# YxZhxn/Ray3D

Hardware: AMD Instinct MI355X
Metric: lifted poses/sec (17-joint, 243-frame window) (higher is better)
Workload: dtype f32; 1 GPU; BASELINE configs[1]: synthetic 17-joint 243-frame windows, batch 256 per GPU, forward-only pos+trj (C=256, latent 256, stage 3, camera embedding); batch_per_gpu=256, receptive_field=243, joints=17, parallelism=dp1 (independent window batches, no data-path collective), clock_settle_steps=60, world_size_observed=1

## Files before the change

### include/ray3d_hip.h

```cpp
#ifndef RAY3D_HIP_H
#define RAY3D_HIP_H

#include <stddef.h>
#include <stdint.h>

#ifdef __cplusplus
extern "C" {
#endif

#define R3D_OK 0
#define R3D_ERR_ARG (-1)
#define R3D_ERR_KEY (-2)
#define R3D_ERR_SHAPE (-3)
#define R3D_ERR_STATE (-4)
#define R3D_ERR_HIP (-5)
#define R3D_ERR_WORKSPACE (-6)
#define R3D_ERR_ABORTED (-7)

#define R3D_KIND_POS 0
#define R3D_KIND_TRJ 1

#define R3D_ABI_VERSION 6

typedef struct {
// ... 39 lines not shown
    int64_t window_stride;
    const float *param_dev;
    int64_t param_stride;
    const double *cam_dev;
    int64_t cam_stride;
} r3d_input;

size_t r3d_workspace_bytes(const r3d_model *pos, const r3d_model *trj, int64_t B);

size_t r3d_input_workspace_bytes(const r3d_model *pos, const r3d_model *trj, const r3d_input *in, int64_t B);

int r3d_prepare(r3d_model *pos, r3d_model *trj, int64_t B);
int r3d_release(r3d_model *pos, r3d_model *trj, int64_t B);

int r3d_forward(r3d_model *m, const r3d_input *in, int64_t B, float *out_dev,
                void *workspace_dev, size_t workspace_bytes, void *hip_stream);

int r3d_forward_pair(r3d_model *pos, r3d_model *trj, const r3d_input *in, int64_t B,
                     float *out_dev, float *out_trj_dev, void *workspace_dev,
                     size_t workspace_bytes, void *hip_stream);


int r3d_status(r3d_model *m, void *hip_stream);

#define R3D_OPT_STAGED 1
#define R3D_OPT_SPIN_TIMEOUT_MS 2
#define R3D_OPT_CU_LIMIT 3
#define R3D_OPT_LANES 4
int r3d_set_option(r3d_model *m, int32_t option, int64_t value);

int r3d_lane_stream(r3d_model *m, int32_t lane, void **stream);
int r3d_lanes_join(r3d_model *m, void *stream);


typedef struct {
    char kernel[48];
    int32_t stage;
    int32_t blocks;
    float ms;
    double flops;
    double bytes;
} r3d_launch_record;
int r3d_profile_enable(r3d_model *m, int on);
int r3d_profile_read(r3d_model *m, r3d_launch_record *records, int capacity);

int r3d_last_clock(r3d_model *m, void *hip_stream, double *ghz);


#define R3D_METRIC_MPJPE 0
#define R3D_METRIC_PMPJPE 1
#define R3D_METRIC_NMPJPE 2
#define R3D_METRIC_VELOCITY 3
#define R3D_METRIC_ROOT 4
#define R3D_METRIC_COUNT 5
#define R3D_METRIC_MAX_BLOCKS 128
#define R3D_METRIC_OUT_DOUBLES (R3D_METRIC_COUNT * (1 + R3D_METRIC_MAX_BLOCKS))
int r3d_clip_metrics(const float *pred_dev, const float *gt_dev, int64_t n_frames, int32_t num_joints,
                     const double *rn2w, const double *tn2w, double *out_dev, void *stream);

#define R3D_DETAIL_THRESHOLDS 31
#define R3D_DETAIL_JOINT_ROWS 3
#define R3D_DETAIL_MAX_JOINTS 17
#define R3D_DETAIL_DOUBLES (R3D_DETAIL_JOINT_ROWS * R3D_DETAIL_MAX_JOINTS + R3D_DETAIL_THRESHOLDS)
#define R3D_DETAIL_OUT_DOUBLES (R3D_DETAIL_DOUBLES * (1 + R3D_METRIC_MAX_BLOCKS))
int r3d_clip_metrics_detail(const float *pred_dev, const float *gt_dev, int64_t n_frames, int32_t num_joints,
                            const double *rn2w, const double *tn2w, double *out_dev, double *frame_dev, double *detail_dev,
                            void *stream);


typedef struct {
    int64_t first_frame;
    int64_t n_frames;
    double  rn2w[9];
    double  tn2w[3];
} r3d_clip_desc;
#define R3D_CLIPS_MAX 65535
size_t r3d_clips_metrics_scratch_bytes(int32_t num_clips, int64_t max_frames, int detail);
int r3d_clips_metrics(const float *pred_dev, const float *gt_dev, int64_t total_frames, int32_t num_joints,
                      const r3d_clip_desc *clips_dev, int32_t num_clips, int64_t max_frames,
                      double *rows_dev, int64_t row_stride,
                      double *detail_dev, int64_t detail_stride,
                      double *frame_dev,
                      void *scratch_dev, size_t scratch_bytes, void *stream);


typedef struct {
    int64_t first_frame;
    int64_t n_frames;
    int64_t out_first;
    int32_t pad_front;
    int32_t pad_back;
    double  cam[16];
} r3d_clip_input_desc;
#define R3D_ENCODE_RAY 0
#define R3D_ENCODE_INTRINSIC 1
#define R3D_ENCODE_SCREEN 2
#define R3D_ENCODE_MAX_POINTS 2147483391
int r3d_clips_encode(const float *px_dev, int64_t total_frames, int32_t num_joints, int32_t encoding,
                     const r3d_clip_input_desc *clips_dev, int32_t num_clips, int64_t max_rows,
                     float *x_dev, int64_t out_rows,
                     float *x_mirror_dev, const int32_t *mirror_perm,
                     int32_t *status_dev, void *stream);


#define R3D_VALID_POS_IS_SUM 1
#define R3D_VALID_GT_ROOT_RELATIVE 2
#define R3D_VALID_LOSS 0
#define R3D_VALID_POS 1
#define R3D_VALID_TRJ_W 2
#define R3D_VALID_TRJ_WSUM 3
#define R3D_VALID_TRJ_DSUM 4
#define R3D_VALID_BONE_LEN 5
#define R3D_VALID_BONE_DIR 6
#define R3D_VALID_COUNT 7
#define R3D_VALID_MAX_BONES 16
#define R3D_VALID_BONE_ROWS 4
#define R3D_VALID_DOUBLES (R3D_VALID_COUNT + R3D_VALID_BONE_ROWS * R3D_VALID_MAX_BONES)
#define R3D_VALID_OUT_DOUBLES (R3D_VALID_DOUBLES * (1 + R3D_METRIC_MAX_BLOCKS))
int r3d_clip_valid_losses(const float *pos_dev, const float *trj_dev, const float *gt_dev, int64_t n_frames,
                          int32_t num_joints, const int32_t *parents, int32_t flags,
                          double *out_dev, double *frame_dev, void *stream);

size_t r3d_clips_valid_scratch_bytes(int32_t num_clips, int64_t max_frames);
int r3d_clips_valid_losses(const float *pos_dev, const float *trj_dev, const float *gt_dev,
                           int64_t total_frames, int32_t num_joints,
                           const int32_t *parents, int32_t flags,
                           const r3d_clip_desc *clips_dev, int32_t num_clips, int64_t max_frames,
                           double *rows_dev, int64_t row_stride,
                           double *frame_dev,
                           void *scratch_dev, size_t scratch_bytes, void *stream);


int r3d_clips_poses(const float *raw_dev, const float *raw_mirror_dev, int64_t raw_rows, int32_t num_joints,
                    const int32_t *mirror_perm,
                    const r3d_clip_desc *clips_dev, const int64_t *raw_first_dev, int32_t num_clips, int64_t max_frames,
                    float *pred_dev, double *world_dev, int64_t total_frames,
                    int32_t *status_dev, void *stream);

const char *r3d_last_error(void);
const char *r3d_version(void);
int r3d_abi_version(void);
int r3d_precision(const r3d_model *m);

#ifdef R3D_TEST_HOOKS

int r3d_debug_schedule_check(int nprob, const int *M, const int *N, const int *nk, const int *max_ks,
                             const int *max_units, int nwg, int enc, int *out_grid, int *out_tiles,
                             double *out_imbalance);

int r3d_debug_plan_check(r3d_model *pos, r3d_model *trj, int64_t batch, int nwg, int *launches, int *spilled);

int r3d_debug_forward_check(r3d_model *pos, r3d_model *trj, int64_t batch, int nwg, int *tiles, int *counters);

typedef struct r3d_census_row {
    int32_t launch;
    int32_t blocks;
    int32_t tiles;
    char kernel[48];
    char tile_kind[48];
} r3d_census_row;
int r3d_debug_forward_census(r3d_model *pos, r3d_model *trj, int64_t batch, int nwg, int32_t uv, int64_t cam_stride,
                             int64_t window_stride, int32_t staged, int32_t captured, r3d_census_row *rows, int32_t cap);
int r3d_debug_census_domain(r3d_census_row *rows, int32_t cap);

int r3d_debug_undistort_host(const double *row16, const double *uv, int64_t n, double *out_uv, double *out_rays);

int r3d_debug_encode_px_host(const double *row16, const double *uv, int64_t n, int32_t encoding, double *out2);

int r3d_debug_valid_losses_host(const float *pos, const float *trj, const float *gt, int64_t n_frames, int32_t num_joints,
                                const int32_t *parents, int32_t flags, double *out, double *frame);
int r3d_debug_clips_encode_host(const float *px, int64_t total_frames, int32_t num_joints, int32_t encoding,
                                const r3d_clip_input_desc *clips, int32_t num_clips, int64_t max_rows, float *x, int64_t out_rows,
                                float *x_mirror, const int32_t *mirror_perm, int32_t *status);
int r3d_debug_clips_valid_losses_host(const float *pos, const float *trj, const float *gt, int64_t total_frames, int32_t num_joints,
                                      const int32_t *parents, int32_t flags, const r3d_clip_desc *clips, int32_t num_clips,
                                      int64_t max_frames, double *rows, int64_t row_stride, double *frame);
int r3d_debug_clips_poses_host(const float *raw, const float *raw_mirror, int64_t raw_rows, int32_t num_joints,
                               const int32_t *mirror_perm, const r3d_clip_desc *clips, const int64_t *raw_first, int32_t num_clips,
                               int64_t max_frames, float *pred, double *world, int64_t total_frames, int32_t *status);
#endif

#ifdef __cplusplus
}
#endif
#endif
```

### ray3d_amd/_capi.py

```python
from __future__ import annotations

import ctypes as C
import os
from typing import List, Optional

_HERE = os.path.dirname(os.path.abspath(__file__))
LIB_PATH = os.path.join(_HERE, "libray3d_hip.so")
HOOKS_LIB_PATH = os.environ.get("R3D_HOOKS_LIB") or os.path.join(_HERE, "libray3d_hip_hooks.so")

R3D_KIND_POS, R3D_KIND_TRJ = 0, 1
R3D_INPUT_RAYS, R3D_INPUT_UV, R3D_INPUT_UV_DIST = 0, 1, 2
R3D_INPUT_PX_INTRINSIC, R3D_INPUT_PX_SCREEN = 3, 4
PX_MODES = (R3D_INPUT_UV_DIST, R3D_INPUT_PX_INTRINSIC, R3D_INPUT_PX_SCREEN)
R3D_ERR_ARG, R3D_ERR_WORKSPACE = -1, -6
R3D_ERR_ABORTED = -7
R3D_OPT_STAGED, R3D_OPT_SPIN_TIMEOUT_MS, R3D_OPT_CU_LIMIT, R3D_OPT_LANES = 1, 2, 3, 4

EXPORTS = (
    "r3d_create", "r3d_destroy", "r3d_num_weights", "r3d_weight_key", "r3d_weight_shape",
    "r3d_set_weight", "r3d_finalize", "r3d_workspace_bytes", "r3d_forward", "r3d_forward_pair",
    "r3d_profile_enable", "r3d_profile_read", "r3d_clip_metrics", "r3d_clip_metrics_detail", "r3d_clip_valid_losses", "r3d_last_error", "r3d_version",
    "r3d_prepare", "r3d_release", "r3d_abi_version", "r3d_precision", "r3d_status", "r3d_set_option", "r3d_last_clock",
    "r3d_lane_stream", "r3d_lanes_join", "r3d_input_workspace_bytes", "r3d_clips_metrics", "r3d_clips_metrics_scratch_bytes",
    "r3d_clips_encode", "r3d_clips_valid_losses", "r3d_clips_valid_scratch_bytes", "r3d_clips_poses",
)
HOOK_EXPORTS = ("r3d_debug_schedule_check", "r3d_debug_plan_check", "r3d_debug_forward_check",
                "r3d_debug_forward_census", "r3d_debug_census_domain",
                "r3d_debug_undistort_host", "r3d_debug_encode_px_host", "r3d_debug_valid_losses_host",
                "r3d_debug_clips_encode_host", "r3d_debug_clips_valid_losses_host", "r3d_debug_clips_poses_host")
ABI_VERSION = 6
METRIC_NAMES = ("mpjpe", "p_mpjpe", "n_mpjpe", "velocity", "root")
METRIC_OUT_DOUBLES = 5 * (1 + 128)
DETAIL_THRESHOLDS, DETAIL_JOINT_ROWS, DETAIL_MAX_JOINTS = 31, 3, 17
DETAIL_DOUBLES = DETAIL_JOINT_ROWS * DETAIL_MAX_JOINTS + DETAIL_THRESHOLDS
DETAIL_OUT_DOUBLES = DETAIL_DOUBLES * (1 + 128)
R3D_VALID_POS_IS_SUM, R3D_VALID_GT_ROOT_RELATIVE = 1, 2
VALID_NAMES = ("loss", "pos", "trj_w", "trj_wsum", "trj_dsum", "bone_len", "bone_dir")
VALID_COUNT, VALID_MAX_BONES, VALID_BONE_ROWS = 7, 16, 4
VALID_DOUBLES = VALID_COUNT + VALID_BONE_ROWS * VALID_MAX_BONES
VALID_OUT_DOUBLES = VALID_DOUBLES * (1 + 128)
METRIC_COUNT, METRIC_MAX_BLOCKS, METRIC_THREADS = 5, 128, 256
CLIPS_MAX = 65535
R3D_ENCODE_RAY, R3D_ENCODE_INTRINSIC, R3D_ENCODE_SCREEN = 0, 1, 2
ENCODE_FLOATS = {R3D_ENCODE_RAY: 3, R3D_ENCODE_INTRINSIC: 2, R3D_ENCODE_SCREEN: 2}
ENCODE_MAX_POINTS = 2 ** 31 - 257
CLIP_INPUT_DESC_BYTES = 160


class Config(C.Structure):
    _fields_ = [(n, C.c_int32) for n in ("struct_size", "kind", "num_joints", "in_features", "num_levels",
                                         "channels", "latent", "stage", "extrinsic_dim",
                                         "embed_dim", "causal", "dense", "bf16x3")]


class Input(C.Structure):
    _fields_ = [("mode", C.c_int32), ("x_dev", C.c_void_p), ("window_stride", C.c_int64),
                ("param_dev", C.c_void_p), ("param_stride", C.c_int64),
                ("cam_dev", C.c_void_p), ("cam_stride", C.c_int64)]


class ClipDesc(C.Structure):
    _fields_ = [("first_frame", C.c_int64), ("n_frames", C.c_int64), ("rn2w", C.c_double * 9), ("tn2w", C.c_double * 3)]


def clip_desc_dtype():
    import numpy as np
    return np.dtype([("first_frame", np.int64), ("n_frames", np.int64), ("rn2w", np.float64, (9,)), ("tn2w", np.float64, (3,))])


CLIP_DESC_BYTES = clip_desc_dtype().itemsize


def clip_input_desc_dtype():
    import numpy as np
    return np.dtype([("first_frame", np.int64), ("n_frames", np.int64), ("out_first", np.int64),
                     ("pad_front", np.int32), ("pad_back", np.int32), ("cam", np.float64, (16,))])


class LaunchRecord(C.Structure):
    _fields_ = [("kernel", C.c_char * 48), ("stage", C.c_int32), ("blocks", C.c_int32),
                ("ms", C.c_float), ("flops", C.c_double), ("bytes", C.c_double)]


class CensusRow(C.Structure):
    _fields_ = [("launch", C.c_int32), ("blocks", C.c_int32), ("tiles", C.c_int32), ("kernel", C.c_char * 48),
                ("tile_kind", C.c_char * 48)]


class Ray3DHipError(RuntimeError):
    pass


_libs = {}
_hooks = os.environ.get("R3D_USE_HOOKS_LIB", "0") not in ("", "0")


_live = {}


def use_hooks(on: bool) -> None:
    global _hooks
    if bool(on) != _hooks and _live.get(HOOKS_LIB_PATH if _hooks else LIB_PATH, 0) > 0:
        try:
            import torch
            if torch.cuda.is_available():
                torch.cuda.synchronize()
        except ImportError:
            pass
    _hooks = bool(on)


def load():
    path = HOOKS_LIB_PATH if _hooks else LIB_PATH
    if path in _libs:
        return _libs[path]
    if not os.path.exists(path):
        raise Ray3DHipError(
            "%s not found: build it with `python -c 'import __graft_entry__ as g; g.build()'` "
            "(hipcc --offload-arch=gfx950).  There is no CPU fallback." % path)
    lib = C.CDLL(path)
    vp, i64p = C.c_void_p, C.POINTER(C.c_int64)
    lib.r3d_create.argtypes = [C.POINTER(Config), C.POINTER(vp)]
    lib.r3d_destroy.argtypes = [vp]
    lib.r3d_num_weights.argtypes = [vp]
    lib.r3d_weight_key.argtypes = [vp, C.c_int]
    lib.r3d_weight_key.restype = C.c_char_p
    lib.r3d_weight_shape.argtypes = [vp, C.c_int, i64p, C.POINTER(C.c_int)]
    lib.r3d_set_weight.argtypes = [vp, C.c_char_p, vp, i64p, C.c_int]
    lib.r3d_finalize.argtypes = [vp]
    lib.r3d_workspace_bytes.argtypes = [vp, vp, C.c_int64]
    lib.r3d_workspace_bytes.restype = C.c_size_t
    lib.r3d_input_workspace_bytes.argtypes = [vp, vp, C.POINTER(Input), C.c_int64]
    lib.r3d_input_workspace_bytes.restype = C.c_size_t
    lib.r3d_forward.argtypes = [vp, C.POINTER(Input), C.c_int64, vp, vp, C.c_size_t, vp]
    lib.r3d_forward_pair.argtypes = [vp, vp, C.POINTER(Input), C.c_int64, vp, vp, vp, C.c_size_t, vp]
    lib.r3d_prepare.argtypes = [vp, vp, C.c_int64]
    lib.r3d_release.argtypes = [vp, vp, C.c_int64]
    lib.r3d_precision.argtypes = [vp]
    lib.r3d_status.argtypes = [vp, vp]
    lib.r3d_set_option.argtypes = [vp, C.c_int32, C.c_int64]
    lib.r3d_last_clock.argtypes = [vp, vp, C.POINTER(C.c_double)]
    lib.r3d_lane_stream.argtypes = [vp, C.c_int32, C.POINTER(vp)]
    lib.r3d_lanes_join.argtypes = [vp, vp]
    lib.r3d_profile_enable.argtypes = [vp, C.c_int]
    lib.r3d_profile_read.argtypes = [vp, C.POINTER(LaunchRecord), C.c_int]
    lib.r3d_clip_metrics.argtypes = [vp, vp, C.c_int64, C.c_int32, C.POINTER(C.c_double), C.POINTER(C.c_double), vp, vp]
    lib.r3d_clip_metrics_detail.argtypes = [vp, vp, C.c_int64, C.c_int32, C.POINTER(C.c_double), C.POINTER(C.c_double), vp, vp, vp, vp]
    lib.r3d_clip_valid_losses.argtypes = [vp, vp, vp, C.c_int64, C.c_int32, C.POINTER(C.c_int32), C.c_int32, vp, vp, vp]
    lib.r3d_clips_metrics_scratch_bytes.argtypes = [C.c_int32, C.c_int64, C.c_int]
    lib.r3d_clips_metrics_scratch_bytes.restype = C.c_size_t
    lib.r3d_clips_metrics.argtypes = [vp, vp, C.c_int64, C.c_int32, vp, C.c_int32, C.c_int64, vp, C.c_int64, vp, C.c_int64, vp, vp, C.c_size_t, vp]
    lib.r3d_clips_encode.argtypes = [vp, C.c_int64, C.c_int32, C.c_int32, vp, C.c_int32, C.c_int64, vp, C.c_int64, vp,
                                     C.POINTER(C.c_int32), vp, vp]
    lib.r3d_clips_valid_scratch_bytes.argtypes = [C.c_int32, C.c_int64]
    lib.r3d_clips_valid_scratch_bytes.restype = C.c_size_t
    lib.r3d_clips_valid_losses.argtypes = [vp, vp, vp, C.c_int64, C.c_int32, C.POINTER(C.c_int32), C.c_int32, vp, C.c_int32, C.c_int64,
                                           vp, C.c_int64, vp, vp, C.c_size_t, vp]
    lib.r3d_clips_poses.argtypes = [vp, vp, C.c_int64, C.c_int32, C.POINTER(C.c_int32), vp, vp, C.c_int32, C.c_int64, vp, vp, C.c_int64,
                                    vp, vp]
    lib.r3d_last_error.restype = C.c_char_p
    lib.r3d_version.restype = C.c_char_p
    if _hooks:
        lib.r3d_debug_forward_census.argtypes = [vp, vp, C.c_int64, C.c_int, C.c_int32, C.c_int64, C.c_int64, C.c_int32, C.c_int32,
                                                 C.POINTER(CensusRow), C.c_int32]
        lib.r3d_debug_census_domain.argtypes = [C.POINTER(CensusRow), C.c_int32]
        lib.r3d_debug_clips_poses_host.argtypes = [vp, vp, C.c_int64, C.c_int32, C.POINTER(C.c_int32), vp, vp, C.c_int32, C.c_int64, vp, vp,
                                                   C.c_int64, vp]
        lib.r3d_debug_clips_valid_losses_host.argtypes = [vp, vp, vp, C.c_int64, C.c_int32, C.POINTER(C.c_int32), C.c_int32, vp, C.c_int32,
                                                          C.c_int64, vp, C.c_int64, vp]
        lib.r3d_debug_undistort_host.argtypes = [vp, vp, C.c_int64, vp, vp]
        lib.r3d_debug_encode_px_host.argtypes = [vp, vp, C.c_int64, C.c_int32, vp]
        lib.r3d_debug_valid_losses_host.argtypes = [vp, vp, vp, C.c_int64, C.c_int32, C.POINTER(C.c_int32), C.c_int32, vp, vp]
        lib.r3d_debug_clips_encode_host.argtypes = [vp, C.c_int64, C.c_int32, C.c_int32, vp, C.c_int32, C.c_int64, vp, C.c_int64, vp,
                                                    C.POINTER(C.c_int32), vp]
    for name in EXPORTS + (HOOK_EXPORTS if _hooks else ()):
        fn = getattr(lib, name)
        if fn.restype is C.c_int or fn.restype is None:
            fn.restype = C.c_int
    if lib.r3d_abi_version() != ABI_VERSION:
        raise Ray3DHipError("%s has ABI version %d, this binding was written for %d: rebuild the library"
# ... 247 lines not shown
```

### ray3d_amd/csrc/r3d_forward.cpp

```cpp
#include <algorithm>
#include <cstring>
#include <mutex>

#include "r3d_internal.hpp"
#include "r3d_undistort.hpp"

namespace r3d {

static void output_slots(int J, const int *first, int *slot) {
    int s = 0;
    auto put = [&](int part, int idx) {
        for (int f = 0; f < 3; ++f) slot[first[part] + idx * 3 + f] = s * 3 + f;
        ++s;
    };
    enum { T = 0, LA = 1, RA = 2, LL = 3, RL = 4 };
    if (J == 17) {
        put(T, 0);
        for (int i = 0; i < 3; ++i) put(LL, i);
        for (int i = 0; i < 3; ++i) put(RL, i);
        for (int i = 1; i < 5; ++i) put(T, i);
        for (int i = 0; i < 3; ++i) put(RA, i);
        for (int i = 0; i < 3; ++i) put(LA, i);
    } else if (J == 15) {
        put(T, 0); put(T, 1);
// ... 492 lines not shown
    bool bound = false;
    char *ctrl = nullptr;
    size_t bank_bytes = 0;
    GemmProb *tables = nullptr;
    int bank = 0;
    unsigned *cnt = nullptr;
    BoundKey key;
};

void resolve_single(const Call &c, Single &s) {
    const Schedule::Fwd &fw = c.sched->fwd;
    const r3d_input *in = c.in;
    if (hipStreamIsCapturing(c.stream, &s.cap) != hipSuccess) { (void)hipGetLastError(); s.cap = hipStreamCaptureStatusActive; }
    s.own = s.cap == hipStreamCaptureStatusNone && fw.d_ctrl != nullptr;
    s.ctrl = s.own ? fw.d_ctrl : reinterpret_cast<char *>(c.ws) + workspace_act_bytes(c.pl, c.B);
    s.bank_bytes = ((size_t)(fw.ncnt + 4) * sizeof(unsigned) + 255) / 256 * 256;
    s.tables = reinterpret_cast<GemmProb *>(s.ctrl + (s.own ? 2 : 1) * s.bank_bytes);
    s.poll = s.own && fw.d_act != nullptr;
    s.key.variant = c.variant;
    s.key.base[BIND_WS] = c.ws;
    s.key.base[BIND_ARENA0] = c.bases.arena[0];
    s.key.base[BIND_ARENA1] = c.bases.arena[1];
    s.key.base[BIND_IARENA0] = c.bases.iarena[0];
    s.key.base[BIND_IARENA1] = c.bases.iarena[1];
    s.key.base[BIND_X] = in->x_dev;
    s.key.base[BIND_PARAM] = in->param_dev;
    s.key.base[BIND_CAM] = in->cam_dev;
    s.key.enc_ws = in->window_stride * c.JF;
    s.key.cam_stride = in->cam_stride;
    s.key.enc_bytes = (unsigned)((size_t)c.frames * c.JF * sizeof(float));
    s.key.param_stride = (int)in->param_stride;
    const Schedule::Fwd::Bound &bd = fw.bound;
    s.bound = s.own && bd.valid && bd.key == s.key;
    s.bank = s.bound ? bd.bank ^ 1 : 0;
    s.cnt = reinterpret_cast<unsigned *>(s.ctrl + (s.own ? s.bank : 0) * s.bank_bytes);
}

int bind_if_needed(Call &c, const Single &s) {
    if (s.bound) return R3D_OK;
    const Schedule::Fwd &fw = c.sched->fwd;
    BindArgs ba;
    memset(&ba, 0, sizeof ba);
    ba.rel = fw.d_rel[c.variant];
    ba.tags = fw.d_tags[c.variant];
    ba.out = s.tables;
    ba.nprob = fw.nprob;
    for (int k = 0; k < BIND_NBASE; ++k) ba.base[k] = s.key.base[k];
    ba.enc_ws = s.key.enc_ws;
    ba.cam_stride = s.key.cam_stride;
    ba.enc_bytes = s.key.enc_bytes;
    ba.param_stride = s.key.param_stride;
    ba.cnt = reinterpret_cast<unsigned *>(s.ctrl);
    ba.ncnt = s.own ? (int)(2 * s.bank_bytes / sizeof(unsigned)) - 4 : fw.ncnt;
    if (s.poll) {
        ba.base[BIND_WS] = fw.d_act;
        ba.arm = fw.d_act;
        ba.canon = 1;
        ba.arm_vec4 = (long long)(2 * fw.act_bytes / 16);
    }
    hipError_t e;
    if (const int rc = c.begin(bind_kernel_name(), 1, 0.0, 0.0); rc != R3D_OK) return rc;
    if ((e = launch_bind(ba, c.stream)) != hipSuccess) return hip_fail(e, "launch r3d_bind_f32");
    if (s.poll) {
        BindArgs b1 = ba;
        b1.base[BIND_WS] = fw.d_act + fw.act_bytes;
        b1.out = s.tables + fw.nprob;
        b1.ncnt = -4;
        b1.arm = nullptr;
        if ((e = launch_bind(b1, c.stream)) != hipSuccess) return hip_fail(e, "launch r3d_bind_f32");
    }
    return c.end();
}

int launch_tiles(Call &c, const Single &s, FwdArgs &fa) {
    Schedule::Fwd &fw = c.sched->fwd;
    const GemmProb *table = s.tables + (s.poll ? s.bank * fw.nprob : 0);
    if (s.poll) c.act_base = reinterpret_cast<float *>(fw.d_act + (size_t)s.bank * fw.act_bytes);
    fw.bound.valid = false;
    memset(&fa, 0, sizeof fa);
    fa.tiles = fw.d_tiles;
    fa.wg_off = fw.d_wgoff;
    fa.probs = table;
    fa.cnt = s.cnt;
    fa.cnt_next = s.own ? reinterpret_cast<unsigned *>(s.ctrl + (s.bank ^ 1) * s.bank_bytes) : nullptr;
    fa.ncnt = fw.ncnt;
    if (s.poll) {
        fa.poll = 1;
        fa.arm = fw.d_act + (size_t)(s.bank ^ 1) * fw.act_bytes;
        fa.arm_vec4 = (long long)(fw.act_bytes / 16);
    }
    fa.spin_ticks = (long long)std::max(c.a->spin_timeout_ms, 1) * 100000LL;
    if (const char *ft = hook_env("R3D_FAULT_TILE")) fa.fault_tile1 = atoi(ft) + 1;
    const bool uv_launch = c.uv && fw.uses_gather;
    const int fwd_kernel = c.shared ? FWD_KERNEL_CLIP : fw.kernel;
    if (const int rc = c.begin(forward_kernel_name(fwd_kernel, uv_launch), fw.grid, fw.flops, fw.bytes); rc != R3D_OK) return rc;
#ifdef R3D_TIMING
    timing_arm_forward(fw, fa, c.stream);
#endif
    if (const hipError_t e = launch_forward(fa, fw.grid, fwd_kernel, uv_launch, c.stream); e != hipSuccess) return hip_fail(e, "launch r3d_forward_f32");
    c.a->last_clk_dev = s.cap == hipStreamCaptureStatusNone ? s.cnt + fw.ncnt + 2 : nullptr;
    return R3D_OK;
}

int launch_in_order(Call &c, const Single &s, FwdArgs &fa) {
    Model *a = c.a;
    hipError_t e;
    std::lock_guard<std::mutex> launch_lock(g_fwd_launch_mu);
    if ((e = order_single_launch(c.stream, true, c.cu_limit > 0)) != hipSuccess) return hip_fail(e, "hipStreamWaitEvent");
    if (c.cu_limit > 0 && a->lanes <= 1 && a->last_fwd_stream && a->last_fwd_stream != c.stream) {
        if ((e = wait_behind(c.stream, (hipStream_t)a->last_fwd_stream, a->order_ev)) != hipSuccess) return hip_fail(e, "hipStreamWaitEvent");
    }
    a->last_fwd_stream = c.stream;
    if (const int rc = bind_if_needed(c, s); rc != R3D_OK) return rc;
    if (const int rc = launch_tiles(c, s, fa); rc != R3D_OK) return rc;
    if ((e = order_single_launch(c.stream, false, c.cu_limit > 0)) != hipSuccess) return hip_fail(e, "hipEventRecord");
    return R3D_OK;
}

int single_launch(Call &c) {
    Schedule::Fwd &fw = c.sched->fwd;
    Single s;
    resolve_single(c, s);
    FwdArgs fa;
    if (const int rc = launch_in_order(c, s, fa); rc != R3D_OK) return rc;
    if (s.own) {
        fw.bound.valid = true;
        fw.bound.bank = s.bank;
        fw.bound.key = s.key;
    }
#ifdef R3D_TIMING
    timing_report_forward(c.pl, fw, fa, c.B, c.stream);
#endif
    if (const int rc = c.end(); rc != R3D_OK) return rc;
    c.abort_flag = s.cnt + fw.ncnt;
    return R3D_OK;
}

int staged_level(Call &c, size_t si) {
    const Plan *pl = c.pl;
    const auto &st = (*c.sched->levels)[si];
    const StageSchedule &ss = c.sched->stages[si];
    LaunchArgs la;
    memset(&la, 0, sizeof la);
    la.tiles = c.sched->d_tiles + ss.tiles_off;
    la.wg_off = c.sched->d_wgoff + ss.wgoff_off;
    la.nprob = (int)st.size();
    la.ks = ss.ks;
    int n_enc = 0;
    for (int i = 0; i < la.nprob; ++i) {
        const ProbSpec &q = pl->probs[st[i] & ~STAGE_SPILL_IN];
        if (q.enc_lut >= 0 && q.enc_kernel) ++n_enc;
        const int rc = fill_prob(pl, q, c.B, c.a, c.bases, c.shape, la.p[i], nullptr);
        if (rc != R3D_OK) return rc;
    }
    if (n_enc != 0 && n_enc != la.nprob) { set_error("internal: launch mixes encoded and plain operands"); return R3D_ERR_STATE; }
    if ((n_enc != 0) != (ss.kind == STAGE_ENC)) { set_error("internal: schedule and plan disagree on the launch kind"); return R3D_ERR_STATE; }
    bool uv_launch = false;
    for (int i = 0; i < la.nprob; ++i) uv_launch = uv_launch || la.p[i].cam != nullptr;
    bool b3_launch = false;
    for (int i = 0; i < la.nprob; ++i) b3_launch = b3_launch || la.p[i].wb3 != nullptr;
    const char *kname = stage_kernel_name(ss.kind, uv_launch, b3_launch);
    if (const int rc = c.begin(kname, ss.nwg, ss.flops, ss.bytes); rc != R3D_OK) return rc;
#ifdef R3D_TIMING
    const bool timed = timing_arm_stage(si, la, c.stream);
#endif
    if (const hipError_t e = launch_gemm_stage(la, ss.nwg, ss.kind, uv_launch, c.stream); e != hipSuccess) return hip_fail(e, "launch r3d_gemm_f32");
#ifdef R3D_TIMING
    if (timed) timing_report_stage(si, ss, c.stream);
#endif
    return c.end();
}

int staged_levels(Call &c) {
    c.a->last_clk_dev = nullptr;
    for (size_t si = 0; si < c.sched->levels->size(); ++si)
        if (const int rc = staged_level(c, si); rc != R3D_OK) return rc;
    return R3D_OK;
}

int decoder_tail(Call &c) {
    const Model *a = c.a;
    const Plan *pl = c.pl;
    auto buf_ptr = [&](int id) -> float * { return c.act_base + (size_t)pl->buffers[id].offset_per_window * (size_t)c.B; };
    DecodeArgs da;
    memset(&da, 0, sizeof da);
    da.B = c.B;
    da.J = a->cfg.num_joints;
    da.has_pos = pl->pos_model >= 0;
    da.has_trj = pl->trj_model >= 0;
    da.out = c.out;
    da.out_trj = da.has_pos ? c.out_trj : nullptr;
    da.abort_flag = c.abort_flag;
    da.status = a->status_host;
    double dec_flops = 0;
    int first = 0;
    std::vector<Plan::Dec> order;
    for (const auto &d : pl->decs) if (pl->m[d.model]->cfg.kind == R3D_KIND_POS) order.push_back(d);
    for (const auto &d : pl->decs) if (pl->m[d.model]->cfg.kind == R3D_KIND_TRJ) order.push_back(d);
    int firsts[MAX_DEC] = {0};
    for (const auto &d : order) {
        const Model *m = pl->m[d.model];
        const Layer &L = m->layers[d.layer];
        const int sidx = da.nsrc++;
        da.h[sidx] = buf_ptr(d.hbuf);
        da.w[sidx] = m->d_arena + L.w_off;
        da.bias[sidx] = m->d_arena + L.b_off;
        da.n_out[sidx] = L.N;
        da.first[sidx] = first;
        firsts[sidx] = first;
        if (m->cfg.kind == R3D_KIND_POS) first += L.N;
        dec_flops += 2.0 * (double)c.B * L.K * L.N;
    }
    if (da.has_pos) output_slots(da.J, firsts, da.slot);
    if (const int rc = c.begin(decode_kernel_name(c.B), 0, dec_flops, (double)c.B * da.nsrc * MLP_HIDDEN * 4.0); rc != R3D_OK) return rc;
    if (const hipError_t e = launch_decode(da, c.stream); e != hipSuccess) return hip_fail(e, "launch r3d_decode_f32");
    if (const int rc = c.end(); rc != R3D_OK) return rc;
    if (c.rec.on()) c.a->nrec = (int)c.rec.n;
    return R3D_OK;
}

int relay_done(Call &c) {
    Model::Lane *relay = c.relay;
    if (!relay) return R3D_OK;
    if (const hipError_t e = hipEventRecord(relay->done, relay->stream); e != hipSuccess) return hip_fail(e, "hipEventRecord(lane)");
    if (std::find(relay->waiters.begin(), relay->waiters.end(), c.caller_stream) == relay->waiters.end()) relay->waiters.push_back(c.caller_stream);
    return R3D_OK;
}

}

int forward_run(Model *a, Model *b, const r3d_input *in, int64_t B, float *out, float *out_trj, void *ws, size_t ws_bytes,
                void *stream) {
    Call c{a, b, in, B, out, out_trj, ws, ws_bytes, stream, (hipStream_t)stream};
    int rc = check_call(c);
    if (rc == R3D_OK) rc = redirect_px(c);
    if (rc == R3D_OK) rc = pick_plan(c);
    if (rc == R3D_OK) rc = pick_lane(c);
    if (rc == R3D_OK) rc = empty_bracket(c);
    if (rc == R3D_OK) rc = px_prepass(c);
    if (rc == R3D_OK) rc = pick_schedule(c);
    if (rc == R3D_OK) rc = frame_stage(c);
    if (rc == R3D_OK) rc = c.single ? single_launch(c) : staged_levels(c);
    if (rc == R3D_OK) rc = decoder_tail(c);
    if (rc == R3D_OK) rc = relay_done(c);
    return rc;
}

}
```

### ray3d_amd/csrc/r3d_hooks.cpp

```cpp
#ifdef R3D_TEST_HOOKS
#include <algorithm>
#include <cstdio>
#include <cstring>
#include <set>
#include <utility>

#include "r3d_internal.hpp"
#include "r3d_poses.hpp"
#include "r3d_undistort.hpp"
#include "r3d_valid.hpp"

using namespace r3d;

namespace {

struct CensusProb { bool w3, lut, wb3, w2; int K; };
struct CensusKernel { const char *name; bool enc, uv, dep, b3, narrow, clip; };

std::vector<CensusKernel> census_kernels() {
    std::vector<CensusKernel> v;
    for (int uv = 0; uv < 2; ++uv) {
        const bool u = uv != 0;
        v.push_back({stage_kernel_name(STAGE_BIG, u, false), false, u, false, false, true, true});
        v.push_back({stage_kernel_name(STAGE_ENC, u, false), true, u, false, false, false, true});
// ... 118 lines not shown
            for (int g = t.z / COL_GRANULE; g < (t.z + tile_width(ks)) / COL_GRANULE && g < gcols; ++g) ++cover[pi][(size_t)u * gcols + g];
        }
    }
    for (int i = 0; i < nprob; ++i)
        for (int c : cover[i])
            if (c != 1) return -10;
    return 0;
}

int r3d_debug_plan_check(r3d_model *pos, r3d_model *trj, int64_t batch, int nwg, int *launches, int *spilled) {
    const ModelPair mp = model_pair(pos, trj);
    Model *a = mp.a, *b = mp.b;
    if (!a) return -1;
    Plan *pl = plan_get(a, b, plan_kind(batch));
    if (!pl) return -2;
    int spill_row0 = -1;
    std::vector<int4> tiles;
    std::vector<int> wgoff;
    std::vector<StageSchedule> stages;
    const std::vector<std::vector<int>> &levels = *schedule_build_host(pl, batch, nwg, spill_row0, tiles, wgoff, stages);
    if (launches) *launches = (int)stages.size();
    if (spilled) *spilled = 0;
    const int np = (int)pl->probs.size();
    std::vector<std::vector<int>> cover(np);
    std::vector<int> last_launch(np, -1), first_launch(np, 1 << 30);
    for (int i = 0; i < np; ++i) {
        const ProbSpec &q = pl->probs[i];
        const int M = (int)(batch * q.rows_per_window), N = pl->m[q.model]->layers[q.layer].N;
        cover[i].assign((size_t)((M + 31) / 32) * ((N + COL_GRANULE - 1) / COL_GRANULE), 0);
    }
    for (size_t si = 0; si < stages.size(); ++si) {
        const StageSchedule &ss = stages[si];
        const auto &st = levels[si];
        if (ss.nwg < 1 || ss.nwg > 2 * nwg) return -3;
        {
            int n_enc = 0;
            for (int e : st) n_enc += pl->probs[e & ~STAGE_SPILL_IN].enc_kernel ? 1 : 0;
            if (n_enc != 0 && n_enc != (int)st.size()) return -11;
            if ((n_enc != 0) != (ss.kind == STAGE_ENC)) return -12;
        }
        for (int t = 0; t < ss.ntiles; ++t) {
            const int4 &tl = tiles[ss.tiles_off + t];
            const int slot = tl.x & 0xff, mi = tl.x >> 8, ks = tl.w;
            if (slot >= (int)st.size() || mi < 1) return -4;
            const int id = st[slot] & ~STAGE_SPILL_IN;
            const ProbSpec &q = pl->probs[id];
            const int M = (int)(batch * q.rows_per_window), N = pl->m[q.model]->layers[q.layer].N;
            if (tl.y % 32 || tl.y < 0 || tl.y >= M || tl.z < 0 || tl.z >= N) return -5;
            if (id == pl->spill_prob) {
                const bool late = (st[slot] & STAGE_SPILL_IN) != 0;
                if (spill_row0 < 0 ? late : (late != (tl.y >= spill_row0))) return -6;
                if (late && spilled) *spilled += std::min(mi * 32, M - tl.y);
            }
            const int gcols = (N + COL_GRANULE - 1) / COL_GRANULE;
            for (int u = tl.y / 32; u < tl.y / 32 + mi; ++u) {
                if (u * 32 >= M) return -7;
                for (int g = tl.z / COL_GRANULE; g < (tl.z + tile_width(ks)) / COL_GRANULE && g < gcols; ++g) ++cover[id][(size_t)u * gcols + g];
            }
            last_launch[id] = std::max(last_launch[id], (int)si);
            first_launch[id] = std::min(first_launch[id], (int)si);
        }
    }
    for (int i = 0; i < np; ++i) {
        for (int c : cover[i])
            if (c != 1) return -8;
        for (int d : pl->probs[i].deps)
            if (last_launch[d] >= first_launch[i]) return -9;
    }
    return 0;
}

int r3d_debug_forward_check(r3d_model *pos, r3d_model *trj, int64_t batch, int nwg, int *out_tiles, int *out_counters) {
    const ModelPair mp = model_pair(pos, trj);
    Model *a = mp.a, *b = mp.b;
    if (!a) return -1;
    Plan *pl = plan_get(a, b, plan_kind(batch));
    int spill_row0 = -1;
    std::vector<int4> tiles;
    std::vector<int> wgoff;
    std::vector<StageSchedule> stages;
    const std::vector<std::vector<int>> &levels = *schedule_build_host(pl, batch, nwg, spill_row0, tiles, wgoff, stages);
    Schedule::Fwd fw;
    std::vector<int> ft, fo;
    if (!schedule_build_fwd(pl, batch, nwg, levels, stages, tiles, wgoff, fw, ft, fo)) return 1;
    if (out_tiles) *out_tiles = fw.ntiles;
    if (out_counters) *out_counters = fw.ncnt;
    const int np = (int)pl->probs.size(), TI = FWD_TILE_INT4 * 4;
    std::vector<int> gcols(np);
    for (int i = 0; i < np; ++i) gcols[i] = (pl->m[pl->probs[i].model]->layers[pl->probs[i].layer].N + COL_GRANULE - 1) / COL_GRANULE;
    std::vector<unsigned> cnt(fw.ncnt, 0);
    struct Acc { int buf, c0, c1; };
    auto reads = [&](const ProbSpec &q) {
        std::vector<Acc> v;
        for (int sgi = 0; sgi < q.nseg; ++sgi)
            if (pl->buffers[q.seg[sgi].buf].external == 0) v.push_back({q.seg[sgi].buf, q.seg[sgi].col, q.seg[sgi].col + q.seg[sgi].width});
        if (q.res_buf >= 0) v.push_back({q.res_buf, q.res_col, q.res_col + pl->m[q.model]->layers[q.layer2 >= 0 && q.layer3 < 0 ? q.layer2 : q.layer].N});
        return v;
    };
    auto writes = [&](const ProbSpec &q) {
        const int N = pl->m[q.model]->layers[q.layer3 >= 0 ? q.layer3 : q.layer2 >= 0 ? q.layer2 : q.layer].N;
        return Acc{q.c_buf, q.c_col, q.c_col + N};
    };
    auto overlap = [](const Acc &x, const Acc &y) { return x.buf == y.buf && x.c0 < y.c1 && y.c0 < x.c1; };
    auto complete = [&](int prob, int w0, int w1) {
        const ProbSpec &q = pl->probs[prob];
        const int M = (int)(batch * q.rows_per_window);
        const int a0 = w0 * q.rows_per_window, a1 = std::min(w1 * q.rows_per_window, M);
        for (int u = a0 / 32; u < (a1 + 31) / 32; ++u)
            if (cnt[fw.cnt_base[prob] + u] != (unsigned)gcols[prob]) return false;
        return true;
    };
    if (pl->kind == PLAN_SMALL) {
        for (int i = 0; i < np; ++i)
            for (int o = 0; o < i; ++o)
                if (overlap(writes(pl->probs[i]), writes(pl->probs[o]))) return -25;
        for (int i = 0; i < np; ++i)
            for (const Acc &rd : reads(pl->probs[i])) {
                std::vector<char> covered(rd.c1 - rd.c0, 0);
                bool any = false, same_rows = true;
                for (int o = 0; o < np; ++o) {
                    const Acc w = writes(pl->probs[o]);
                    if (w.buf != rd.buf) continue;
                    any = true;
                    same_rows = same_rows && pl->probs[o].rows_per_window == pl->probs[i].rows_per_window;
                    for (int c = std::max(w.c0, rd.c0); c < std::min(w.c1, rd.c1); ++c) covered[c - rd.c0] = 1;
                }
                if (!any) return -26;
                if (same_rows)
                    for (char c : covered)
                        if (!c) return -26;
            }
    }
    std::vector<int> next(fw.grid);
    for (int w = 0; w < fw.grid; ++w) next[w] = fo[w];
    int done = 0;
    for (bool progress = true; progress;) {
        progress = false;
        for (int w = 0; w < fw.grid; ++w) {
            while (next[w] < fo[w + 1]) {
                const int *d = &ft[(size_t)next[w] * TI];
                bool ready = true;
                for (int k = 0; k < d[4] && ready; ++k) {
                    const int base = d[8 + 2 * k], n = d[9 + 2 * k] & 0xffff;
                    const unsigned need = (unsigned)d[9 + 2 * k] >> 16;
                    for (int u = 0; u < n && ready; ++u) ready = cnt[base + u] >= need;
                }
                if (!ready) break;
                const int id = d[0] & 0xff, mi = d[0] >> 8;
                const ProbSpec &q = pl->probs[id];
                const int M = (int)(batch * q.rows_per_window);
                const int r1 = std::min(d[1] + mi * 32, M);
                const int w0 = d[1] / q.rows_per_window, w1 = (r1 - 1) / q.rows_per_window + 1;
                const Acc wr = writes(q);
                for (int o = 0; o < id; ++o) {
                    const ProbSpec &oq = pl->probs[o];
                    bool hazard = false;
                    for (const Acc &rd : reads(q)) hazard = hazard || overlap(rd, writes(oq));
                    for (const Acc &rd : reads(oq)) hazard = hazard || overlap(rd, wr);
                    hazard = hazard || overlap(writes(oq), wr);
                    if (hazard && !complete(o, w0, w1)) return -20;
                }
                if (d[5] != fw.cnt_base[id] + d[1] / 32 || d[5] + mi > fw.ncnt) return -21;
                for (int u = 0; u < mi; ++u) {
                    cnt[d[5] + u] += (unsigned)d[6];
                    if (cnt[d[5] + u] > (unsigned)gcols[id]) return -22;
                }
                ++next[w];
                ++done;
                progress = true;
            }
        }
    }
    if (done != fw.ntiles) return -23;
    for (int i = 0; i < np; ++i)
        for (int u = 0; u < (int)((batch * pl->probs[i].rows_per_window + 31) / 32); ++u)
            if (cnt[fw.cnt_base[i] + u] != (unsigned)gcols[i]) return -24;
    return 0;
}

int r3d_debug_forward_census(r3d_model *pos, r3d_model *trj, int64_t batch, int nwg, int32_t uv, int64_t cam_stride, int64_t window_stride,
                             int32_t staged, int32_t captured, r3d_census_row *rows, int32_t cap) {
    const ModelPair mp = model_pair(pos, trj);
    Model *a = mp.a, *b = mp.b;
    if (!a || batch <= 0 || nwg <= 0 || window_stride <= 0 || (!rows && cap > 0)) return -1;
    if (b && !same_input_shape(a, b)) return -1;
    if (uv && a->cfg.in_features != 3) return -1;
    Plan *pl = plan_get(a, b, plan_kind(batch));
    if (!pl) return -2;
    CensusSched &cs = g_census;
    if (cs.ida != a->id || cs.idb != (b ? b->id : 0) || cs.pl != pl || cs.B != batch || cs.nwg != nwg) {
        cs = CensusSched();
        cs.ida = a->id;
        cs.idb = b ? b->id : 0;
        cs.pl = pl;
        cs.B = batch;
        cs.nwg = nwg;
        cs.levels = schedule_build_host(pl, batch, nwg, cs.spill_row0, cs.tiles, cs.wgoff, cs.stages);
        if (forward_single_launch() && schedule_build_fwd(pl, batch, nwg, *cs.levels, cs.stages, cs.tiles, cs.wgoff, cs.fw, cs.ft, cs.fo)) {
            bool narrow = false, b3_tiles = false;
            cs.fw.kernel = forward_kernel_of_lists(pl, batch, cs.ft, narrow, b3_tiles);
            if (narrow && b3_tiles) cs.fw = Schedule::Fwd();
        } else {
            cs.fw = Schedule::Fwd();
        }
    }
    const std::vector<CensusKernel> kernels = census_kernels();
    const Schedule::Fwd &fw = cs.fw;
    const long long frames = (batch - 1) * window_stride + a->RF;
    const bool shared = call_shares_first_layers(pl, a, batch, uv != 0, window_stride, cam_stride, frames, pl->frame_buf >= 0);
    const int variant = (uv ? 1 : 0) + (shared ? 2 : 0);
    std::vector<GemmProb> rel;
    std::vector<unsigned char> tags;
    const bool has_table = fw.grid > 0 && forward_variant_table(pl, batch, variant, fw.nprob, rel, tags);
    const bool single = !staged && call_is_single(a, b, fw.grid, has_table, fw.kernel, shared);
    CensusOut out{rows, cap};
    if (shared) {
        std::vector<int4> ft;
        std::vector<int> fo;
        StageSchedule fs{};
        schedule_frame_stage(pl, batch, nwg, ft, fo, fs);
        const char *name = stage_kernel_name(STAGE_BIG, uv != 0, false);
        const CensusKernel *k = census_find(kernels, name);
        if (!k) return -4;
        std::map<std::string, int> hist;
        for (const int4 &t : ft) {
            const Plan::FrameProb &f = pl->frame_probs[t.x & 0xff];
            ++hist[census_tile_kind(*k, CensusProb{false, true, false, false, pl->m[f.model]->layers[f.layer].Kpad}, t.x >> 8, t.w)];
        }
        out.launch_of(name, fs.nwg, hist);
    }
    if (single) {
        (void)captured;
        out.launch_of(bind_kernel_name(), 1, {});
        const int fwd_kernel = shared ? FWD_KERNEL_CLIP : fw.kernel;
        const char *name = forward_kernel_name(fwd_kernel, uv && fw.uses_gather);
        const CensusKernel *k = census_find(kernels, name);
        if (!k) return -4;
        std::map<std::string, int> hist;
        const int TI = FWD_TILE_INT4 * 4;
        for (int t = 0; t < fw.ntiles; ++t) {
            const int *d = &cs.ft[(size_t)t * TI];
            const int id = d[0] & 0xff;
            ++hist[census_tile_kind(*k, census_prob(&tags[(size_t)id * BIND_NPTR], rel[id].K), d[0] >> 8, d[3])];
        }
        out.launch_of(name, fw.grid, hist);
    } else {
        CallShape shape;
        shape.uv = uv != 0;
        shape.shared = shared;
        shape.window_stride = window_stride;
        shape.cam_stride = cam_stride;
        shape.frames = frames;
        const Bases none;
        for (size_t si = 0; si < cs.levels->size(); ++si) {
            const auto &st = (*cs.levels)[si];
            const StageSchedule &ss = cs.stages[si];
            std::vector<CensusProb> P(st.size());
            bool uv_launch = false, b3_launch = false;
            for (size_t i = 0; i < st.size(); ++i) {
                GemmProb g;
                unsigned char tg[BIND_NPTR];
                if (fill_prob(pl, pl->probs[st[i] & ~STAGE_SPILL_IN], batch, a, none, shape, g, tg) != R3D_OK) return -3;
                P[i] = census_prob(tg, g.K);
                uv_launch = uv_launch || tg[17] != BIND_NULL;
                b3_launch = b3_launch || P[i].wb3;
            }
            const char *name = stage_kernel_name(ss.kind, uv_launch, b3_launch);
            const CensusKernel *k = census_find(kernels, name);
            if (!k) return -4;
            std::map<std::string, int> hist;
            for (int t = 0; t < ss.ntiles; ++t) {
                const int4 &tl = cs.tiles[ss.tiles_off + t];
                const int slot = tl.x & 0xff;
                if (slot >= (int)st.size()) return -5;
                ++hist[census_tile_kind(*k, P[slot], tl.x >> 8, tl.w)];
            }
            out.launch_of(name, ss.nwg, hist);
        }
    }
    out.launch_of(decode_kernel_name(batch), 0, {});
    return out.n;
}

int r3d_debug_census_domain(r3d_census_row *rows, int32_t cap) {
    if (!rows && cap > 0) return -1;
    CensusOut out{rows, cap};
    for (const char *name : launch_kernel_names()) out.row(name, 0, "", 0);
    const int codes[] = {1, 2, 4, 8, 16, NB_CODE + 4, NB_CODE + 5, NB_CODE + 6, NB_CODE + 7};
    for (const CensusKernel &k : census_kernels()) {
        std::set<std::string> kinds;
        for (int f = 0; f < 16; ++f)
            for (int K : {64, 96})
                for (int mi = 1; mi <= GEMM_SCHED_MAX_UNITS + 1; ++mi)
                    for (int ks : codes) kinds.insert(census_tile_kind(k, CensusProb{(f & 1) != 0, (f & 2) != 0, (f & 4) != 0, (f & 8) != 0, K}, mi, ks));
        for (const std::string &kind : kinds) out.row(k.name, 0, kind.c_str(), 0);
    }
    return out.n;
}

int r3d_debug_undistort_host(const double *row16, const double *uv, int64_t n, double *out_uv, double *out_rays) {
    if (!row16 || (!uv && n > 0) || n < 0) { set_error("r3d_debug_undistort_host: bad argument"); return R3D_ERR_ARG; }
    const UndistRow k = undist_row(row16);
    for (int64_t i = 0; i < n; ++i) {
        double uo, vo, r[3];
        undistort_pixel(k, uv[2 * i], uv[2 * i + 1], uo, vo);
        pixel_to_ray(k, uo, vo, r);
        if (out_uv) { out_uv[2 * i] = uo; out_uv[2 * i + 1] = vo; }
        if (out_rays) for (int c = 0; c < 3; ++c) out_rays[3 * i + c] = r[c];
    }
    return R3D_OK;
}

int r3d_debug_encode_px_host(const double *row16, const double *uv, int64_t n, int32_t encoding, double *out2) {
    if (!row16 || !out2 || (!uv && n > 0) || n < 0) { set_error("r3d_debug_encode_px_host: bad argument"); return R3D_ERR_ARG; }
    if (encoding != ENC_INTRINSIC && encoding != ENC_SCREEN) {
        set_error("r3d_debug_encode_px_host: encoding must be 1 (intrinsic) or 2 (screen), got %d", encoding);
        return R3D_ERR_ARG;
    }
    for (int64_t i = 0; i < n; ++i) encode_pixel_2d(row16, encoding, uv[2 * i], uv[2 * i + 1], out2 + 2 * i);
    return R3D_OK;
}

int r3d_debug_clips_encode_host(const float *px, int64_t total_frames, int32_t num_joints, int32_t encoding,
                                const r3d_clip_input_desc *clips, int32_t num_clips, int64_t max_rows, float *x, int64_t out_rows,
                                float *x_mirror, const int32_t *mirror_perm, int32_t *status) {
    const int rc = clips_encode_check_args("r3d_debug_clips_encode_host", px, total_frames, num_joints, encoding, clips, num_clips, max_rows,
                                           x, out_rows, x_mirror, mirror_perm, status);
    if (rc != R3D_OK) return rc;
    unsigned long long inv[2] = {0ull, 0ull};
    if (mirror_perm) mirror_pack_inverse(mirror_perm, num_joints, inv);
// ... 112 lines not shown
```

### ray3d_amd/csrc/r3d_internal.hpp

```cpp
#pragma once

#include <hip/hip_runtime.h>

#include <cstdint>
#include <cstdlib>
#include <map>
#include <mutex>
#include <string>
#include <vector>

#include "ray3d_hip.h"

namespace r3d {

constexpr int BK = 32;
constexpr int MAX_SEG = 4;
constexpr int MAX_PROB = 12;
constexpr int N_ALIGN = 256;
constexpr int MLP_HIDDEN = 1024;
constexpr int EMBED_MID = 32;
constexpr int CUR_LD = 64;


struct GemmProb {
    const float *a[MAX_SEG];
    int lda[MAX_SEG];
    int kend[MAX_SEG];
    const float *w;
    const float *bias;
    const float *res;
    float *c;
    int ldr, ldc;
    int M, N, K;
    float slope;
    const float *w2;
    const float *bias2;
    int K2;
    float slope2;
    const float *wb3;
    const float *w2b3, *w3b3;
    const float *w3;
    const float *bias3;
    int K3;
    float slope3;
    const int *lut;
    const float *x;
    long long enc_ws;
    int enc_rows;
    int enc_jf;
    int enc_cur;
    int enc_step;
    unsigned enc_bytes;
    int res_tap;
    int canon;
    const double *cam;
    long long cam_stride;
};

struct LaunchArgs {
    const int4 *tiles;
    const int *wg_off;
    int nprob;
    int ks;
    long long *dbg;
    GemmProb p[MAX_PROB];
};

constexpr int FWD_TILE_INT4 = 6;
constexpr int FWD_MAX_DEP = 8;
struct FwdArgs {
    const int4 *tiles;
    const int *wg_off;
    const GemmProb *probs;
    unsigned *cnt;
    unsigned *cnt_next;
    int ncnt;
    int poll;
    void *arm;
    long long arm_vec4;
    long long spin_ticks;
    int fault_tile1;
    long long *dbg;
};
enum { FWD_KERNEL_F32 = 0, FWD_KERNEL_B3 = 1, FWD_KERNEL_LAT = 2, FWD_KERNEL_CLIP = 3, FWD_KERNEL_COUNT = 4 };
constexpr int BIND_NPTR = 18;
enum { BIND_NULL = 0, BIND_WS, BIND_ARENA0, BIND_ARENA1, BIND_IARENA0, BIND_IARENA1, BIND_X, BIND_PARAM, BIND_CAM, BIND_NBASE };
struct BindArgs {
    const GemmProb *rel;
    const unsigned char *tags;
    GemmProb *out;
    unsigned *cnt;
    int nprob, ncnt;
    const void *base[BIND_NBASE];
    long long enc_ws, cam_stride;
    unsigned enc_bytes;
    int param_stride;
    int canon;
    void *arm;
    long long arm_vec4;
};

struct UndistArgs {
    const float *uv;
    const double *cam;
    long long cam_stride;
    float *rays;
    int npts;
    int J;
    int pts_per_window;
    int window_stride;
    int last_window;
    int encoding;
};

struct ClipsEncArgs {
    const r3d_clip_input_desc *table;
    const float *px;
    float *x;
    float *x_mirror;
    int32_t *status;
    long long total_frames, out_rows, max_rows;
    unsigned long long mirror_inv[2];
    int J;
    int encoding;
};

struct ClipsPosesArgs {
    const r3d_clip_desc *table;
    const long long *raw_first;
    const float *raw, *raw_mirror;
    float *pred;
    double *world;
    int32_t *status;
    long long raw_rows, total_frames, max_frames;
    unsigned long long mirror_perm[2];
    int J;
};

constexpr int MAX_DEC = 6;
struct DecodeArgs {
    const float *h[MAX_DEC];
    const float *w[MAX_DEC];
    const float *bias[MAX_DEC];
    int n_out[MAX_DEC];
    int first[MAX_DEC];
    int nsrc;
    int has_pos, has_trj;
    int J;
    long long B;
    float *out;
    float *out_trj;
    const unsigned *abort_flag;
    unsigned *status;
    int slot[5 * 16];
};


struct TensorSpec {
    std::string key;
    int rank;
    int64_t shape[4];
    int64_t numel() const {
        int64_t n = 1;
        for (int i = 0; i < rank; ++i) n *= shape[i];
        return n;
    }
};

inline int64_t b3_min_batch() {
    return 96;
}

inline bool env_on(const char *name) {
    const char *e = getenv(name);
    return e && atoi(e) != 0;
}
#ifdef R3D_TEST_HOOKS
inline bool hook_on(const char *name) { return env_on(name); }
inline const char *hook_env(const char *name) { return getenv(name); }
#else
inline bool hook_on(const char *) { return false; }
inline const char *hook_env(const char *) { return nullptr; }
#endif

struct Layer {
    std::string weight_key;
    std::string bias_key;
    std::string bn_prefix;
    int taps;
    int cin;
    int N, K, Npad, Kpad;
    float slope;
    std::vector<int> colmap;
    std::vector<int> colmap_neg;
    bool frag;
    size_t w_off, b_off;
    bool bf3 = false;
    bool bf3_conv = false;
    size_t wb3_off = 0;
    struct Pre { int ref_col0, ref_width, new_width, shrink_layer; };
    std::vector<Pre> pre;
    int cin_ref = 0;
    int shared_of = -1;
    int shared_split = 0;
};

struct Model {
    r3d_config cfg;
    int RF;
    std::vector<TensorSpec> specs;
    std::map<std::string, int> spec_index;
    std::vector<std::vector<float>> host_weights;
    std::vector<bool> have;
    std::vector<Layer> layers;
    std::map<std::string, int> layer_index;
    struct Branch {
        std::string prefix;
        std::vector<int> joints;
        int cin, k0, k0pad;
        size_t lut_off;
        size_t lut_uv_off;
        size_t lut_frame_off = 0, lut_frame_uv_off = 0;
        int frame_layer = -1;
    };
    std::vector<Branch> branches;
    size_t global_lut_off = 0;
    size_t global_lut_uv_off = 0;
    bool use_b3 = false;
    bool fold_shrink = false;
    std::vector<float> arena;
    std::vector<int> iarena;
    float *d_arena = nullptr;
    int *d_iarena = nullptr;
    int device = -1;
    bool finalized = false;
    bool dirty = true;
    bool opt_staged = false;
    int spin_timeout_ms = 1000;
    int cu_limit = 0;
    void *last_fwd_stream = nullptr;
    hipEvent_t order_ev = nullptr;
    int lanes = 0;
    struct Lane {
        hipStream_t stream = nullptr;
        hipEvent_t done = nullptr, in = nullptr;
        std::vector<void *> waiters;
    };
    Lane lane[4];
    int next_lane = 0;
    const unsigned *last_clk_dev = nullptr;
    unsigned *status_host = nullptr;
    bool profiling = false;
    struct Rec {
        hipEvent_t e0, e1;
        r3d_launch_record r;
    };
    std::vector<Rec> recs;
    int nrec = 0;
    uint64_t id = 0;
    ~Model();
};

struct BufferSpec {
    std::string name;
    int64_t floats_per_window;
    int external;
    int64_t offset_per_window;
};

struct ProbSpec {
    int model;
    int layer;
    int rows_per_window;
    int nseg;
    struct Seg { int buf, col, ld, width; } seg[MAX_SEG];
    int res_buf, res_col, res_ld;
    int c_buf, c_col, c_ld;
    int layer2;
    int layer3;
    int enc_lut;
    int enc_lut_uv;
    bool enc_kernel;
    int enc_rows;
    int enc_step;
    int frame_col = -1;
    std::vector<int> deps;
    int depth;
    double flops_per_window;
};

struct StageSchedule {
    int nwg;
    int ks;
    int kind;
    int ntiles;
    size_t tiles_off;
    size_t wgoff_off;
    double flops, bytes;
    double imbalance;
    double makespan;
};

struct BoundKey {
    int variant = 0;
    const void *base[BIND_NBASE] = {nullptr};
    long long enc_ws = 0, cam_stride = 0;
    unsigned enc_bytes = 0;
    int param_stride = 0;
    bool operator==(const BoundKey &o) const {
        bool same = variant == o.variant && enc_ws == o.enc_ws && cam_stride == o.cam_stride && enc_bytes == o.enc_bytes &&
                    param_stride == o.param_stride;
        for (int k = 0; same && k < BIND_NBASE; ++k) same = base[k] == o.base[k];
        return same;
    }
};

struct Schedule {
    int64_t B = 0;
    bool pinned = false;
    int spill_row0 = -1;
    const std::vector<std::vector<int>> *levels = nullptr;
    std::vector<StageSchedule> stages;
    int4 *d_tiles = nullptr;
    int *d_wgoff = nullptr;
    StageSchedule frame_stage{};
    int4 *d_frame_tiles = nullptr;
    int *d_frame_wgoff = nullptr;
    struct Fwd {
        int grid = 0, ntiles = 0, ncnt = 0, nprob = 0;
        std::vector<int> cnt_base;
        int4 *d_tiles = nullptr;
        int *d_wgoff = nullptr;
        GemmProb *d_rel[4] = {nullptr, nullptr, nullptr, nullptr};
        unsigned char *d_tags[4] = {nullptr, nullptr, nullptr, nullptr};
        std::vector<int> h_tiles, h_wgoff;
        double flops = 0, bytes = 0;
        bool uses_gather = false;
        int kernel = FWD_KERNEL_F32;
        char *d_ctrl = nullptr;
        size_t bank_bytes = 0;
        char *d_act = nullptr;
        size_t act_bytes = 0;
        struct Bound {
            bool valid = false;
            int bank = 0;
            BoundKey key;
        } bound;
    } fwd;
    ~Schedule();
};

struct Plan {
    const Model *m[2] = {nullptr, nullptr};
    std::vector<BufferSpec> buffers;
    std::vector<ProbSpec> probs;
    std::vector<std::vector<int>> stages;
    std::vector<std::vector<int>> stages_spill;
    std::vector<std::vector<int>> stages_spill_alt;
    std::vector<std::vector<int>> stages_asap;
    int spill_prob = -1;
    int kind = 0;
    int64_t floats_per_window = 0;
    int64_t tail_floats = 0;
    int frame_buf = -1, frame_ld = 0;
    struct FrameProb { int model, layer, col, lut, lut_uv; };
    std::vector<FrameProb> frame_probs;
    int emb_buf[2] = {-1, -1};
    int param_buf = -1;
    struct Dec { int model, layer, hbuf; };
    std::vector<Dec> decs;
    int pos_model = -1, trj_model = -1;
    std::map<int64_t, Schedule *> schedules;
    std::vector<int64_t> schedule_lru;
    ~Plan();
};

struct Bases {
    const char *ws = nullptr, *arena[2] = {nullptr, nullptr}, *iarena[2] = {nullptr, nullptr};
    const char *x = nullptr, *param = nullptr, *cam = nullptr;
};
struct CallShape {
    bool uv = false;
    bool shared = false;
    int64_t window_stride = 0, param_stride = 0, cam_stride = 0;
    long long frames = 0;
};

inline int frame_floats(const Model *a, bool uv) { return a->cfg.num_joints * (uv ? 2 : a->cfg.in_features); }

struct ModelPair { Model *a, *b; };
inline ModelPair model_pair(const r3d_model *pos, const r3d_model *trj) {
    Model *p = const_cast<Model *>(reinterpret_cast<const Model *>(pos)), *t = const_cast<Model *>(reinterpret_cast<const Model *>(trj));
    return {p ? p : t, p ? t : nullptr};
}

int fill_prob(const Plan *pl, const ProbSpec &q, int64_t B, const Model *a, const Bases &bs, const CallShape &cs, GemmProb &g,
              unsigned char *tags);
bool same_input_shape(const Model *a, const Model *b);
size_t workspace_bytes_pair(Model *a, Model *b, int64_t B);
int dist_check(const Model *a, const r3d_input *in, bool need_cam);
size_t dist_ray_bytes(const Model *a, const r3d_input *in, int64_t B);
struct FwdKeys { int cu_limit, nwg, lane_key0, nlanes; };
FwdKeys forward_keys(const Model *a, const Model *b);
int forward_run(Model *a, Model *b, const r3d_input *in, int64_t B, float *out, float *out_trj, void *ws, size_t ws_bytes, void *stream);
const char *stage_kernel_name(int kind, bool uv_launch, bool b3_launch);
const char *decode_kernel_name(int64_t B);
const char *bind_kernel_name();
const char *undistort_kernel_name();
std::vector<const char *> launch_kernel_names();
bool call_shares_first_layers(const Plan *pl, const Model *a, int64_t B, bool uv, int64_t window_stride, int64_t cam_stride, long long frames,
                              bool frame_tiles);
bool call_is_single(const Model *a, const Model *b, int grid, bool has_table, int kernel, bool shared);

extern std::mutex g_fwd_launch_mu;
hipError_t wait_behind(hipStream_t stream, hipStream_t other, hipEvent_t &ev);
hipError_t order_single_launch(hipStream_t stream, bool before, bool masked = false);
int lanes_create(Model *m, int n);
void lanes_destroy(Model *m);

int valid_check_args(const char *what, const float *pos, const float *trj, const float *gt, int64_t n, int32_t J,
                     const int32_t *parents, int32_t flags, const double *out);

int clips_valid_check_args(const char *what, const float *pos, const float *trj, const float *gt, int64_t total_frames, int32_t J,
                           const int32_t *parents, int32_t flags, const r3d_clip_desc *clips, int32_t num_clips, int64_t max_frames,
                           const double *rows, int64_t row_stride, const void *scratch, bool scratch_checked);

int clips_encode_check_args(const char *what, const float *px, int64_t total_frames, int32_t J, int32_t encoding,
                            const r3d_clip_input_desc *clips, int32_t num_clips, int64_t max_rows, const float *x, int64_t out_rows,
                            const float *x_mirror, const int32_t *mirror_perm, const int32_t *status);

int clips_poses_check_args(const char *what, const float *raw, const float *raw_mirror, int64_t raw_rows, int32_t J,
                           const int32_t *mirror_perm, const r3d_clip_desc *clips, const int64_t *raw_first, int32_t num_clips,
                           int64_t max_frames, const float *pred, const double *world, int64_t total_frames, const int32_t *status);

#ifdef R3D_TIMING
void timing_arm_forward(const Schedule::Fwd &fw, FwdArgs &fa, hipStream_t stream);
void timing_report_forward(const Plan *pl, const Schedule::Fwd &fw, const FwdArgs &fa, int64_t B, hipStream_t stream);
bool timing_arm_stage(size_t si, LaunchArgs &la, hipStream_t stream);
void timing_report_stage(size_t si, const StageSchedule &ss, hipStream_t stream);
#endif

void set_error(const char *fmt, ...);
const char *last_error();
int hip_fail(hipError_t e, const char *what);

Model *model_create(const r3d_config &cfg);
int model_set_weight(Model *m, const char *key, const float *host, const int64_t *shape, int rank);
int model_finalize(Model *m);
enum { PLAN_FUSED = 0, PLAN_SMALL = 1, PLAN_MEDIUM = 2, PLAN_LARGE = 3 };
int plan_kind(int64_t B);
std::vector<int64_t> plan_kind_edges();
Plan *plan_get(Model *a, Model *b, int kind);
void plans_drop(const Model *m);
bool plans_pinned(const Model *m);
constexpr int STAGE_SPILL_IN = 1 << 30;
constexpr int GEMM_SCHED_MAX_UNITS = 6;
struct SchedProb {
    int M, N, nk;
    int max_ks;
    int max_units;
    int nk2 = 0;
    int row0 = 0;
    bool gemv = false;
    bool lat = false;
    bool nb_ok = false;
};
constexpr int GEMV_ROWS = 4;
constexpr int COL_GRANULE = 32;
constexpr int NB_CODE = 64;
constexpr bool tile_is_nb(int ks) { return ks > NB_CODE; }
constexpr bool tile_is_narrow(int ks) { return ks >= 8 && ks < NB_CODE; }
constexpr int tile_width(int ks) { return ks > NB_CODE ? (ks - NB_CODE) * 32 : ks >= 8 ? 32 : 256 / ks; }
void schedule_stage(const std::vector<SchedProb> &probs, int nwg, int max_units, std::vector<int4> &tiles,
                    std::vector<int> &wgoff, StageSchedule &out, bool enc = false);
inline size_t frag_index(int o, int k, int nk) {
    const int nb = o >> 5, li = o & 31, kt = k >> 5, kin = k & 31, lh = kin >> 4, q = (kin & 15) >> 2, e = kin & 3;
    return ((((size_t)nb * nk + kt) * 4 + q) * 64 + (lh * 32 + li)) * 4 + e;
}
const std::vector<std::vector<int>> *schedule_build_host(const Plan *pl, int64_t B, int nwg, int &spill_row0, std::vector<int4> &tiles,
                                                        std::vector<int> &wgoff, std::vector<StageSchedule> &stages);
bool schedule_build_fwd(const Plan *pl, int64_t B, int nwg, const std::vector<std::vector<int>> &levels, const std::vector<StageSchedule> &stages,
                        const std::vector<int4> &tiles, const std::vector<int> &wgoff, Schedule::Fwd &fw, std::vector<int> &out_tiles,
                        std::vector<int> &out_wgoff);
Schedule *schedule_get(Plan *pl, int64_t B, int nwg, bool pin = false, int lane = 0);
void schedule_frame_stage(const Plan *pl, int64_t B, int nwg, std::vector<int4> &ft, std::vector<int> &fo, StageSchedule &ss);
bool forward_variant_table(const Plan *pl, int64_t B, int v, int nprob, std::vector<GemmProb> &rel, std::vector<unsigned char> &tags);
int forward_kernel_of_lists(const Plan *pl, int64_t B, const std::vector<int> &ft, bool &narrow, bool &b3_tiles);
inline int64_t schedule_key(int64_t B, int lane) { return B | ((int64_t)lane << 48); }
int device_cu_count();

enum { STAGE_BIG = 0, STAGE_ENC = 1 };
typedef void (*GemmKernel)(const LaunchArgs);
typedef void (*FwdKernel)(const FwdArgs);
GemmKernel gemm_kernel_f32(bool uv);
GemmKernel gemm_kernel_enc(bool uv);
GemmKernel gemm_kernel_b3(bool uv);
FwdKernel fwd_kernel_f32(bool uv);
FwdKernel fwd_kernel_b3(bool uv);
FwdKernel fwd_kernel_lat(bool uv);
FwdKernel fwd_kernel_clip(bool uv);
hipError_t launch_gemm_stage(const LaunchArgs &args, int nwg, int kind, bool uv, hipStream_t stream);
hipError_t launch_decode(const DecodeArgs &args, hipStream_t stream);
hipError_t launch_forward(const FwdArgs &args, int nwg, int kind, bool uv, hipStream_t stream);
const char *forward_kernel_name(int kind, bool uv);
int forward_resident_capacity(int kind, bool uv);
hipError_t launch_bind(const BindArgs &args, hipStream_t stream);
hipError_t launch_undistort(const UndistArgs &args, hipStream_t stream);
hipError_t launch_clips_encode(const ClipsEncArgs &args, int num_clips, hipStream_t stream);
hipError_t launch_clips_poses(const ClipsPosesArgs &args, int num_clips, hipStream_t stream);
bool forward_single_launch();
size_t fwd_ctrl_bytes(const Plan *pl, int64_t B);

inline int round_up(int v, int m) { return (v + m - 1) / m * m; }

constexpr int ENC_INVALID = (int)0x80000000u;

int launch_clip_metrics(const float *pred, const float *gt, long long n, int J, const double *Rn2w, const double *Tn2w,
                        double *out, double *frame, double *detail, hipStream_t stream);
int launch_clip_valid(const float *pos, const float *trj, const float *gt, long long n, int J, const int32_t *parents,
                      int flags, double *out, double *frame, hipStream_t stream);
size_t clips_metrics_scratch_bytes(int num_clips, long long max_frames, bool detail);
int launch_clips_metrics(const float *pred, const float *gt, long long total, int J, const r3d_clip_desc *table, int num_clips,
                         long long max_frames, double *rows, long long row_stride, double *detail, long long detail_stride,
                         double *frame, void *scratch, hipStream_t stream);
size_t clips_valid_scratch_bytes(int num_clips, long long max_frames);
int launch_clips_valid(const float *pos, const float *trj, const float *gt, long long total, int J, const int32_t *parents, int flags,
                       const r3d_clip_desc *table, int num_clips, long long max_frames, double *rows, long long row_stride,
                       double *frame, void *scratch, hipStream_t stream);

}
```

### ray3d_amd/csrc/r3d_plan.cpp

```cpp
#include <algorithm>
#include <cstdio>
#include <cstdlib>
#include <mutex>

#include "r3d_internal.hpp"

namespace r3d {

namespace {

struct Builder {
    Plan &p;
    int mi;
    const Model &m;

    int buffer(const std::string &name, int64_t floats_per_window, int external = 0) {
        BufferSpec b;
        b.name = name;
        b.floats_per_window = (floats_per_window + 15) / 16 * 16;
        b.external = external;
        b.offset_per_window = 0;
        p.buffers.push_back(b);
        return (int)p.buffers.size() - 1;
    }
// ... 169 lines not shown
            B.enc_in_gemm = small;
            B.single_assign = small;
            B.fuse_pairs = (kind == PLAN_FUSED || kind == PLAN_LARGE);
            B.fuse_top = kind == PLAN_LARGE;
        }
        const int lat = m->cfg.latent, D = m->cfg.embed_dim;
        int pe = -1;
        if (D > 0) {
            if (pl->param_buf < 0) pl->param_buf = B.buffer("param", 0, 3);
            const int eh = B.buffer("emb.h", EMBED_MID);
            pl->emb_buf[mi] = B.buffer("emb", D);
            const int E = m->cfg.extrinsic_dim;
            const int p1 = B.problem("embedder.w1", 1, {{pl->param_buf, 0, 0, E, -1}}, -1, 0, 0, eh, 0, EMBED_MID);
            pe = B.problem("embedder.w2", 1, {{eh, 0, EMBED_MID, EMBED_MID, p1}}, -1, 0, 0, pl->emb_buf[mi], 0, D);
        }
        const int g = B.buffer("global", lat);
        const int pg = B.fc_block("GlobalInfo", {}, 2, g, 0, lat, (int)m->global_lut_off, (int)m->global_lut_uv_off);
        if (m->cfg.kind == R3D_KIND_POS) {
            pl->pos_model = mi;
            const bool fold = m->fold_shrink;
            const int C = m->cfg.channels;
            const int tmp5 = fold ? -1 : B.buffer("tmp5", 5 * lat);
            int sh[5];
            for (int bi = 0; bi < 5; ++bi) sh[bi] = B.temporal_block(bi, tmp5, bi * lat, 5 * lat);
            int mix5 = -1, pf[5] = {-1, -1, -1, -1, -1};
            if (m->cfg.stage != 1) {
                mix5 = B.buffer("mix5", 5 * lat);
                for (int i = 0; i < 5; ++i) {
                    std::vector<Builder::In> ins;
                    if (fold) {
                        for (int k = 0; k < 5; ++k)
                            if (k != i) ins.push_back({B.locals[k].buf, 0, B.locals[k].ld, C, sh[k]});
                    } else {
                        if (i > 0) ins.push_back({tmp5, 0, 5 * lat, i * lat, sh[0]});
                        if (i < 4) ins.push_back({tmp5, (i + 1) * lat, 5 * lat, (4 - i) * lat, sh[4]});
                    }
                    const int first = (int)pl->probs.size();
                    pf[i] = B.fc_block("FuseBlocks." + std::to_string(i), ins, 1, mix5, i * lat, 5 * lat);
                    for (int k = 0; k < 5; ++k) pl->probs[first].deps.push_back(sh[k]);
                    for (int q = first; q < (int)pl->probs.size(); ++q) {
                        int d = 0;
                        for (int dep : pl->probs[q].deps) d = std::max(d, pl->probs[dep].depth + 1);
                        pl->probs[q].depth = d;
                    }
                }
            }
            for (int bi = 0; bi < 5; ++bi) {
                std::vector<Builder::In> ins;
                if (fold) ins.push_back({B.locals[bi].buf, 0, B.locals[bi].ld, C, sh[bi]});
                else ins.push_back({tmp5, bi * lat, 5 * lat, lat, sh[bi]});
                if (mix5 >= 0) ins.push_back({mix5, bi * lat, 5 * lat, lat, pf[bi]});
                ins.push_back({g, 0, lat, lat, pg});
                if (D > 0) ins.push_back({pl->emb_buf[mi], 0, D, D, pe});
                B.fc_block(std::string("Integration_") + (bi == 0 ? "Torso" : bi == 1 ? "LArm" : bi == 2 ? "RArm" : bi == 3 ? "LLeg" : "RLeg"),
                           ins, 1, -1, 0, 0);
            }
        } else {
            pl->trj_model = mi;
            const int local = m->fold_shrink ? -1 : B.buffer("local", lat);
            const int sh = B.temporal_block(0, local, 0, lat);
            std::vector<Builder::In> ins;
            if (m->fold_shrink) ins.push_back({B.locals[0].buf, 0, B.locals[0].ld, m->cfg.channels, sh});
            else ins.push_back({local, 0, lat, lat, sh});
            ins.push_back({g, 0, lat, lat, pg});
            if (D > 0) ins.push_back({pl->emb_buf[mi], 0, D, D, pe});
            B.fc_block("Integration", ins, 1, -1, 0, 0);
        }
    }
    std::vector<int> asap;
    for (const auto &q : pl->probs) asap.push_back(q.depth);
    auto levelise = [&](bool spill, bool pin_first, std::vector<std::vector<int>> &stages, bool early = false) -> bool {
        const int n = (int)pl->probs.size();
        for (int i = 0; i < n; ++i) pl->probs[i].depth = asap[i];
        int deepest = 0, pt = -1;
        for (const auto &q : pl->probs) deepest = std::max(deepest, q.depth);
        if (spill) {
            bool pos_fused = false;
            for (int i = 0; i < n; ++i) {
                const ProbSpec &q = pl->probs[i];
                if (q.layer3 >= 0 && pl->m[q.model]->cfg.kind == R3D_KIND_TRJ) pt = i;
                pos_fused = pos_fused || (q.layer3 >= 0 && pl->m[q.model]->cfg.kind == R3D_KIND_POS);
            }
            if (pt < 0 || !pos_fused) return false;
            for (auto &q : pl->probs)
                for (int d : q.deps)
                    if (d == pt) q.depth = std::max(q.depth, pl->probs[pt].depth + 2);
            int grown = 0;
            for (auto &q : pl->probs) {
                for (int d : q.deps) q.depth = std::max(q.depth, pl->probs[d].depth + 1);
                grown = std::max(grown, q.depth);
            }
            if (grown > deepest) return false;
        }
        std::vector<std::vector<int>> users(n);
        for (int i = 0; i < n; ++i)
            for (int d : pl->probs[i].deps) users[d].push_back(i);
        auto movable = [&](const ProbSpec &q) {
            if (early) return false;
            const std::string &key = pl->m[q.model]->layers[q.layer].weight_key;
            if (pin_first && pt >= 0 && std::find(q.deps.begin(), q.deps.end(), pt) != q.deps.end()) return false;
            if (spill && pl->m[q.model]->cfg.kind == R3D_KIND_TRJ && key.rfind("LocalLayer.", 0) == 0 && q.layer3 < 0) return true;
            return (key.rfind("GlobalInfo.", 0) == 0 && key.rfind("GlobalInfo.fc_1", 0) != 0) || key.rfind("Integration.", 0) == 0;
        };
        auto iterations = [&](const ProbSpec &q) {
            const Model *mm = pl->m[q.model];
            int it = mm->layers[q.layer].Kpad / BK;
            if (q.layer3 >= 0) it = 3 * it + mm->layers[q.layer2].Kpad / BK + mm->layers[q.layer3].Kpad / BK;
            else if (q.layer2 >= 0) it += mm->layers[q.layer2].Kpad / BK;
            return it;
        };
        std::vector<int> level_iters(deepest + 1, 0);
        for (const auto &q : pl->probs)
            if (!movable(q)) level_iters[q.depth] = std::max(level_iters[q.depth], iterations(q));
        for (int i = n - 1; i >= 0; --i) {
            ProbSpec &q = pl->probs[i];
            if (!movable(q)) continue;
            int latest = users[i].empty() ? deepest : 1 << 30;
            for (int u : users[i]) latest = std::min(latest, pl->probs[u].depth - 1);
            if (latest >= (1 << 30) || latest <= q.depth) continue;
            int pick = latest;
            for (int l = latest; l >= q.depth; --l)
                if (level_iters[l] >= iterations(q)) { pick = l; break; }
            q.depth = pick;
        }
        int maxd = 0;
        for (auto &q : pl->probs) maxd = std::max(maxd, q.depth);
        std::vector<std::vector<int>> lv(maxd + 1);
        for (int i = 0; i < n; ++i) lv[pl->probs[i].depth].push_back(i);
        if (spill) lv[pl->probs[pt].depth + 1].push_back(pt | STAGE_SPILL_IN);
        if (hook_env("R3D_PLAN_DUMP"))
            for (size_t s = 0; s < lv.size(); ++s) {
                fprintf(stderr, "[plan%s] launch %zu:", spill ? " spill" : "", s);
                for (int e : lv[s]) {
                    const ProbSpec &q = pl->probs[e & ~STAGE_SPILL_IN];
                    fprintf(stderr, " %s%s(x%d)", e & STAGE_SPILL_IN ? "+" : "", pl->m[q.model]->layers[q.layer].weight_key.c_str(), q.rows_per_window);
                }
                fprintf(stderr, "\n");
            }
        stages.clear();
        for (auto &st : lv)
            for (size_t i = 0; i < st.size(); i += MAX_PROB)
                stages.emplace_back(st.begin() + i, st.begin() + std::min(st.size(), i + MAX_PROB));
        if (spill) pl->spill_prob = pt;
        return true;
    };
    const bool can_spill = pl->m[0] && pl->m[1] && !hook_on("R3D_NO_SPILL");
    if (!(can_spill && levelise(true, false, pl->stages_spill))) pl->stages_spill.clear();
    if (!(can_spill && levelise(true, true, pl->stages_spill_alt)) || pl->stages_spill_alt == pl->stages_spill) pl->stages_spill_alt.clear();
    levelise(false, false, pl->stages);
    if (kind == PLAN_SMALL) {
        levelise(false, false, pl->stages_asap, true);
        if (pl->stages_asap == pl->stages) pl->stages_asap.clear();
    }
    {
        bool all = true;
        int col = 0;
        std::vector<Plan::FrameProb> fps;
        for (auto &q : pl->probs) {
            if (q.layer3 < 0) continue;
            const Model *mm = pl->m[q.model];
            const Model::Branch *br = nullptr;
            for (const auto &b : mm->branches)
                if ((int)b.lut_off == q.enc_lut) br = &b;
            if (!br || br->frame_layer < 0) { all = false; break; }
            q.frame_col = col;
            fps.push_back({q.model, br->frame_layer, col, (int)br->lut_frame_off, mm->cfg.in_features == 3 ? (int)br->lut_frame_uv_off : -1});
            col += (mm->layers[br->frame_layer].N + 15) / 16 * 16;
        }
        if (all && !fps.empty() && fps.size() <= (size_t)MAX_PROB) {
            Builder B{*pl, 0, *pl->m[0]};
            pl->frame_ld = col;
            pl->frame_buf = B.buffer("frames", col);
            pl->frame_probs = fps;
            int RF = 1;
            for (const Model *mm : pl->m)
                if (mm) RF = std::max(RF, mm->RF);
            pl->tail_floats = std::max<int64_t>(pl->tail_floats, (int64_t)(RF + 2) * col);
        } else {
            for (auto &q : pl->probs) q.frame_col = -1;
        }
    }
    int64_t off = 0;
    for (auto &bf : pl->buffers) {
        bf.offset_per_window = off;
        off += bf.floats_per_window;
    }
    pl->floats_per_window = off;
    return pl;
}

static std::mutex g_plans_mutex;
static std::map<std::pair<std::pair<uint64_t, uint64_t>, int>, Plan *> g_plans;

constexpr int64_t SMALL_PLAN_MAX = 48, MEDIUM_PLAN_MAX = 96, LARGE_PLAN_MIN = 1024;

std::vector<int64_t> plan_kind_edges() { return {SMALL_PLAN_MAX, MEDIUM_PLAN_MAX, LARGE_PLAN_MIN - 1}; }

int plan_kind(int64_t B) {
    if (B >= LARGE_PLAN_MIN) return PLAN_LARGE;
    if (hook_on("R3D_NO_SMALL_PLAN")) return PLAN_FUSED;
    return B <= SMALL_PLAN_MAX ? PLAN_SMALL : B <= MEDIUM_PLAN_MAX ? PLAN_MEDIUM : PLAN_FUSED;
}

Plan *plan_get(Model *a, Model *b, int kind) {
    std::lock_guard<std::mutex> lock(g_plans_mutex);
    const auto key = std::make_pair(std::make_pair(a->id, b ? b->id : (uint64_t)0), kind);
    auto it = g_plans.find(key);
    if (it != g_plans.end()) return it->second;
    Plan *p = build_plan(a, b, kind);
    g_plans[key] = p;
    return p;
}

void plans_drop(const Model *m) {
    std::lock_guard<std::mutex> lock(g_plans_mutex);
    for (auto it = g_plans.begin(); it != g_plans.end();) {
        if (it->first.first.first == m->id || it->first.first.second == m->id) {
            for (const Model *mm : it->second->m)
                if (mm) const_cast<Model *>(mm)->last_clk_dev = nullptr;
            delete it->second;
            it = g_plans.erase(it);
        } else {
            ++it;
        }
    }
}

bool plans_pinned(const Model *m) {
    std::lock_guard<std::mutex> lock(g_plans_mutex);
    for (const auto &kv : g_plans)
        if (kv.first.first.first == m->id || kv.first.first.second == m->id)
            for (const auto &sc : kv.second->schedules)
                if (sc.second && sc.second->pinned) return true;
    return false;
}

}
```

### ray3d_amd/csrc/r3d_schedule.cpp

```cpp
#include <algorithm>
#include <chrono>
#include <cmath>
#include <cstdio>
#include <cstdlib>
#include <map>

#include "r3d_internal.hpp"

namespace r3d {

Schedule::~Schedule() {
    if (d_tiles) (void)hipFree(d_tiles);
    if (d_wgoff) (void)hipFree(d_wgoff);
    if (fwd.d_tiles) (void)hipFree(fwd.d_tiles);
    if (fwd.d_wgoff) (void)hipFree(fwd.d_wgoff);
    if (fwd.d_ctrl) (void)hipFree(fwd.d_ctrl);
    if (fwd.d_act) (void)hipFree(fwd.d_act);
    for (int i = 0; i < 4; ++i) {
        if (fwd.d_rel[i]) (void)hipFree(fwd.d_rel[i]);
        if (fwd.d_tags[i]) (void)hipFree(fwd.d_tags[i]);
    }
    if (d_frame_tiles) (void)hipFree(d_frame_tiles);
    if (d_frame_wgoff) (void)hipFree(d_frame_wgoff);
}

bool forward_single_launch() {
    static const bool on = !env_on("R3D_STAGED");
    return on;
}

static void dump_fwd(const Plan *pl, int64_t B, int grid, const std::vector<int> &out_tiles, const std::vector<int> &out_wgoff) {
    const int np = (int)pl->probs.size();
    std::vector<int> M(np);
    for (int i = 0; i < np; ++i) M[i] = (int)(B * pl->probs[i].rows_per_window);
    if (const char *dump = hook_env("R3D_FWD_DUMP")) {
        if (FILE *f = fopen(dump, "w")) {
            for (int i = 0; i < np; ++i) {
                const ProbSpec &q = pl->probs[i];
                const Model *mm = pl->m[q.model];
                fprintf(f, "P %d %s rpw %d M %d N %d K %d K2 %d K3 %d deps", i, mm->layers[q.layer].weight_key.c_str(), q.rows_per_window, M[i],
                        mm->layers[q.layer].N, mm->layers[q.layer].Kpad, q.layer2 >= 0 ? mm->layers[q.layer2].Kpad : 0,
                        q.layer3 >= 0 ? mm->layers[q.layer3].Kpad : 0);
                for (int dpi : q.deps) fprintf(f, " %d", dpi);
                fprintf(f, "\n");
            }
            for (int b = 0; b < grid; ++b)
                for (int t = out_wgoff[b]; t < out_wgoff[b + 1]; ++t) {
                    const int *d = &out_tiles[(size_t)t * FWD_TILE_INT4 * 4];
                    fprintf(f, "T %d %d %d %d %d %d %d\n", b, t, d[0] & 0xff, d[0] >> 8, d[1], d[2], d[3]);
                }
            fclose(f);
        }
    }
}

static int64_t units_of(int64_t B, const ProbSpec &q) { return (B * q.rows_per_window + 31) / 32; }
static SchedProb sched_prob_of(const Plan *pl, const ProbSpec &q, int64_t B);

size_t fwd_ctrl_bytes(const Plan *pl, int64_t B) {
    int64_t ncnt = 0;
    for (const auto &q : pl->probs) ncnt += units_of(B, q);
    return ((size_t)(ncnt + 4) * sizeof(unsigned) + 255) / 256 * 256 + pl->probs.size() * sizeof(GemmProb) + 256;
}

bool schedule_build_fwd(const Plan *pl, int64_t B, int nwg, const std::vector<std::vector<int>> &levels, const std::vector<StageSchedule> &stages,
                        const std::vector<int4> &tiles, const std::vector<int> &wgoff, Schedule::Fwd &fw, std::vector<int> &out_tiles,
                        std::vector<int> &out_wgoff) {
    const int np = (int)pl->probs.size();
    if (np > 255) return false;
    for (const auto &ss : stages)
        if (ss.kind != STAGE_BIG) return false;
    for (const Model *m : pl->m)
        if (m && m->cfg.dense) return false;
    fw.nprob = np;
    fw.cnt_base.assign(np, 0);
    std::vector<int> gcols(np), M(np);
    int ncnt = 0;
    for (int i = 0; i < np; ++i) {
        const ProbSpec &q = pl->probs[i];
        fw.cnt_base[i] = ncnt;
        ncnt += (int)units_of(B, q);
        gcols[i] = (pl->m[q.model]->layers[q.layer].N + COL_GRANULE - 1) / COL_GRANULE;
        M[i] = (int)(B * q.rows_per_window);
        if (q.enc_lut >= 0) fw.uses_gather = true;
    }
    fw.ncnt = ncnt;
    std::vector<char> narrow(np, 0), quiet(np, 1);
    for (size_t si = 0; si < stages.size(); ++si)
        for (int t = 0; t < stages[si].ntiles; ++t) {
            const int4 &tl = tiles[stages[si].tiles_off + t];
            if (tile_is_narrow(tl.w)) narrow[levels[si][tl.x & 0xff] & ~STAGE_SPILL_IN] = 1;
        }
    for (int i = 0; i < np; ++i)
        for (int dp : pl->probs[i].deps)
            if (!narrow[i]) quiet[dp] = 0;
    std::vector<std::vector<int>> lists(nwg);
    fw.flops = fw.bytes = 0;
    for (size_t si = 0; si < stages.size(); ++si) {
        const StageSchedule &ss = stages[si];
        const auto &st = levels[si];
        fw.flops += ss.flops;
        fw.bytes += ss.bytes;
        if (ss.nwg > nwg) return false;
        const int n = ss.nwg, qd = n >> 3, r = n & 7;
        for (int b = 0; b < n; ++b) {
            const int xcd = b & 7, idx = b >> 3;
            const int c = (xcd < r ? xcd * (qd + 1) : r * (qd + 1) + (xcd - r) * qd) + idx;
            if (c >= n) continue;
            for (int t = wgoff[ss.wgoff_off + c]; t < wgoff[ss.wgoff_off + c + 1]; ++t) {
                const int4 &tl = tiles[ss.tiles_off + t];
                const int slot = tl.x & 0xff, mi = tl.x >> 8, ks = tl.w;
                const int id = st[slot] & ~STAGE_SPILL_IN;
                const ProbSpec &q = pl->probs[id];
                int d[FWD_TILE_INT4 * 4] = {0};
                d[0] = id | (mi << 8);
                d[1] = tl.y;
                d[2] = tl.z;
                d[3] = ks;
                d[5] = fw.cnt_base[id] + tl.y / 32;
                {
                    const int g0 = tl.z / COL_GRANULE, g1 = std::min(gcols[id], (tl.z + tile_width(ks)) / COL_GRANULE);
                    d[6] = std::max(g1 - g0, 0);
                    if (d[6] <= 0) return false;
                }
                const int r1 = std::min(tl.y + mi * 32, M[id]);
                const int w0 = tl.y / q.rows_per_window, w1 = (r1 - 1) / q.rows_per_window + 1;
                std::vector<int> deps(q.deps);
                std::sort(deps.begin(), deps.end());
                deps.erase(std::unique(deps.begin(), deps.end()), deps.end());
                int nd = 0;
                for (int dp : deps) {
                    const ProbSpec &pq = pl->probs[dp];
                    const int a0 = w0 * pq.rows_per_window, a1 = std::min(w1 * pq.rows_per_window, M[dp]);
                    if (a1 <= a0) continue;
                    const int u0 = a0 / 32, u1 = (a1 + 31) / 32;
                    if (nd == FWD_MAX_DEP || u1 - u0 > 0xffff || gcols[dp] > 0x7fff) return false;
                    d[8 + 2 * nd] = fw.cnt_base[dp] + u0;
                    d[9 + 2 * nd] = (u1 - u0) | (gcols[dp] << 16);
                    ++nd;
                }
                d[4] = nd;
                d[7] = quiet[id] ? 1 : 0;
                lists[b].insert(lists[b].end(), d, d + FWD_TILE_INT4 * 4);
            }
        }
    }
    out_tiles.clear();
    out_wgoff.assign(1, 0);
    int grid = 0;
    for (int b = 0; b < nwg; ++b) {
        out_tiles.insert(out_tiles.end(), lists[b].begin(), lists[b].end());
        out_wgoff.push_back((int)(out_tiles.size() / (FWD_TILE_INT4 * 4)));
        if (!lists[b].empty()) grid = b + 1;
    }
    out_wgoff.resize(grid + 1);
    fw.grid = grid;
    fw.ntiles = (int)(out_tiles.size() / (FWD_TILE_INT4 * 4));
    dump_fwd(pl, B, grid, out_tiles, out_wgoff);
    return grid > 0;
}

Plan::~Plan() {
    for (auto &kv : schedules) delete kv.second;
}

int device_cu_count() {
    static int cus[64] = {0};
    int dev = 0;
    if (hipGetDevice(&dev) != hipSuccess || dev < 0 || dev >= 64) return 256;
    if (!cus[dev]) {
        hipDeviceProp_t prop;
        cus[dev] = hipGetDeviceProperties(&prop, dev) == hipSuccess ? prop.multiProcessorCount : 256;
    }
    return cus[dev];
}

namespace {

struct CostModel {
    double iter = 2200.0, fixed = 2500.0, ks_iter = 2600.0, ks_fixed = 6800.0, first_extra = 5.0, first_extra_wide = 7.0, pair_scale = 1.08;
    double nb_iter_extra = 60.0, nb_fixed_extra = 1500.0;
};
const CostModel &cost_model() {
    static const CostModel c = [] {
        CostModel m;
        if (const char *e = hook_env("R3D_COST"))
            sscanf(e, "%lf,%lf,%lf,%lf,%lf,%lf,%lf,%lf,%lf", &m.iter, &m.fixed, &m.ks_iter, &m.ks_fixed, &m.first_extra, &m.first_extra_wide, &m.pair_scale,
                   &m.nb_iter_extra, &m.nb_fixed_extra);
        return m;
    }();
    return c;
}
double unit_cycles(int iters, int ks) {
    const CostModel &c = cost_model();
    if (ks > 1) return iters * c.ks_iter + c.ks_fixed;
    return iters * c.iter + c.fixed + (iters < 4 ? (4 - iters) * 1400.0 : 0.0);
}

double nb_cycles(int nk, int nb) {
    const CostModel &c = cost_model();
    return nk * (64.0 * (16 + 4 * (nb - 4)) + (c.iter - 2048.0) + c.nb_iter_extra) + c.fixed + c.nb_fixed_extra;
}

double gemv_cycles(int nk) { return 8000.0 + nk / 8.0 * 900.0; }
double lat_cycles(int nk) { return 9000.0 + nk / 8.0 * 2600.0; }

struct Run {
    int prob, col0, ks, u0, n, cap;
};

struct Seg {
    int prob, col0, units, nk, cap, max_ks;
    double c1;
    int ncols;
    bool gemv = false;
    int code = 8;
};

struct Assignment {
    std::vector<std::vector<Run>> bins;
    double worst = 0;
};

bool assign(const std::vector<Seg> &segs, int nbins, double T, int ksplit, Assignment *out) {
    std::vector<double> room(nbins, T);
    if (out) out->bins.assign(nbins, {});
    struct Left { const Seg *s; int u0; };
    std::vector<Left> left;
    int cursor = 0;
    double cursor_cost = -1;
    long long top_units = 0;
    const double top_c1 = segs.empty() ? 0.0 : segs.front().c1;
    for (const Seg &s : segs)
        if (s.c1 == top_c1) top_units += s.units;
    const int top_cap = (int)std::max<long long>(1, (top_units + nbins - 1) / nbins);
    for (const Seg &s : segs) {
        if (s.gemv) {
            const double ck = s.code == 8 ? gemv_cycles(s.nk) : lat_cycles(s.nk);
            std::vector<int> by_room(nbins);
            for (int b = 0; b < nbins; ++b) by_room[b] = b;
            std::stable_sort(by_room.begin(), by_room.end(), [&](int x, int y) { return room[x] > room[y]; });
            for (int j = 0; j * 32 < s.ncols; ++j) {
                const int best = by_room[j % nbins];
                if (room[best] + 1e-6 < ck) return false;
                room[best] -= ck;
                if (out) out->bins[best].push_back({s.prob, s.col0 + j * 32, s.code, 0, 1, 1});
            }
            continue;
        }
        if (s.c1 != cursor_cost) { cursor = 0; cursor_cost = s.c1; }
        const int spread = s.c1 == top_c1 && segs.back().c1 != top_c1 ? top_cap : 1 << 30;
        int u = 0;
        if (s.c1 * 6.0 <= T && s.c1 * s.units <= 2.0 * T && s.c1 != top_c1) {
            auto less_room = [&](int x, int y) { return room[x] != room[y] ? room[x] < room[y] : x > y; };
            std::vector<int> heap(nbins);
            for (int b = 0; b < nbins; ++b) heap[b] = b;
            std::make_heap(heap.begin(), heap.end(), less_room);
            while (u < s.units) {
                std::pop_heap(heap.begin(), heap.end(), less_room);
                const int best = heap.back();
                if (room[best] + 1e-6 < s.c1) break;
                const int take = std::min(std::min(2, (int)std::floor((room[best] + 1e-6) / s.c1)), s.units - u);
                room[best] -= take * s.c1;
                if (out) out->bins[best].push_back({s.prob, s.col0, 1, u, take, s.cap});
                u += take;
                std::push_heap(heap.begin(), heap.end(), less_room);
            }
        } else if (s.c1 <= T) {
            while (u < s.units) {
                while (cursor < nbins && room[cursor] + 1e-6 < s.c1) ++cursor;
                if (cursor == nbins) break;
                const int take = std::min(std::min((int)std::floor((room[cursor] + 1e-6) / s.c1), spread), s.units - u);
                room[cursor] -= take * s.c1;
                if (out) out->bins[cursor].push_back({s.prob, s.col0, 1, u, take, s.cap});
                u += take;
                if (take == spread) ++cursor;
            }
        }
        if (u < s.units) {
            if (s.max_ks < 2) return false;
            left.push_back({&s, u});
        }
    }
    std::stable_sort(left.begin(), left.end(), [](const Left &a, const Left &b) { return a.s->nk > b.s->nk; });
    cursor = 0;
    cursor_cost = -1;
    for (const Left &l : left) {
        const Seg &s = *l.s;
        int ks = std::min(ksplit, s.max_ks);
        while (ks > 1 && s.nk / ks < 2) ks /= 2;
        if (ks == 1) return false;
        const double ck = unit_cycles((s.nk + ks - 1) / ks, ks);
        if (ck > T) return false;
        if (ck != cursor_cost) { cursor = 0; cursor_cost = ck; }
        for (int j = 0; j < ks; ++j) {
// ... 308 lines not shown
    const auto t_begin = std::chrono::steady_clock::now();
    auto build_all = [&](const std::vector<std::vector<int>> &lv, int row0, std::vector<int4> &t, std::vector<int> &w,
                         std::vector<StageSchedule> &ss) {
        double sum = 0;
        for (const auto &st : lv) {
            StageSchedule a{};
            build_stage(pl, st, B, nwg, row0, t, w, a);
            ss.push_back(a);
            sum += a.makespan;
        }
        return sum;
    };
    if (!pl->stages_asap.empty() && B <= GEMV_ROWS) {
        build_all(pl->stages_asap, -1, tiles, wgoff, stages);
        return &pl->stages_asap;
    }
    const double c_plain = build_all(pl->stages, -1, tiles, wgoff, stages);
    double c_best = c_plain;
    std::vector<int> searched0, searched1;
    int searched_row0 = -1;
    auto try_spill = [&](const std::vector<std::vector<int>> &lv) {
        if (pl->spill_prob < 0 || lv.empty()) return;
        int s0 = -1, s1 = -1;
        for (int si = 0; si < (int)lv.size(); ++si)
            for (int e : lv[si]) {
                if (e == pl->spill_prob) s0 = si;
                if (e == (pl->spill_prob | STAGE_SPILL_IN)) s1 = si;
            }
        const ProbSpec &q = pl->probs[pl->spill_prob];
        const int M_all = (int)(B * q.rows_per_window);
        const long long own = (M_all + 31) / 32;
        long long fl_tiles = 0;
        for (int e : lv[std::max(s0, 0)])
            if (!(e & STAGE_SPILL_IN) && pl->probs[e].layer3 >= 0) fl_tiles += (B * pl->probs[e].rows_per_window + 31) / 32;
        if (!(s0 >= 0 && s1 >= 0 && fl_tiles > nwg)) return;
        const long long rem = fl_tiles % nwg;
        std::vector<long long> cands{0};
        if (rem > 0 && rem <= nwg / 2) cands.push_back(rem);
        for (long long r = 32; r <= nwg / 2; r += 32)
            if (r != rem) cands.push_back(r);
        double best = 0;
        int best_row0 = M_all;
        const bool same_pair = lv[s0] == searched0 && lv[s1] == searched1;
        if (same_pair) best_row0 = searched_row0;
        for (long long r : cands) {
            if (same_pair) break;
            if (r >= own) continue;
            const int row0 = r ? (int)((own - r) * 32) : M_all;
            std::vector<int4> t;
            std::vector<int> w;
            StageSchedule a{}, b{};
            build_stage(pl, lv[s0], B, nwg, row0, t, w, a);
            build_stage(pl, lv[s1], B, nwg, row0, t, w, b);
            const double cost = a.makespan + b.makespan;
            if (r == 0 || cost < best * 0.995) { best = cost; best_row0 = row0; }
        }
        searched0 = lv[s0];
        searched1 = lv[s1];
        searched_row0 = best_row0;
        if (best_row0 >= M_all) return;
        std::vector<int4> t;
        std::vector<int> w;
        std::vector<StageSchedule> ss;
        const double c_spill = build_all(lv, best_row0, t, w, ss);
        if (dump) fprintf(stderr, "[plan] B=%lld: %d rows late: modelled %.0f cycles, best so far %.0f\n", (long long)B, M_all - best_row0, c_spill, c_best);
        if (c_spill < c_best * 0.99) {
            c_best = c_spill;
            levels = &lv;
            spill_row0 = best_row0;
            tiles.swap(t);
            wgoff.swap(w);
            stages.swap(ss);
        }
    };
    try_spill(pl->stages_spill);
    try_spill(pl->stages_spill_alt);
    if (dump)
        fprintf(stderr, "[plan] B=%lld: schedule built in %.2f ms\n", (long long)B,
                std::chrono::duration<double, std::milli>(std::chrono::steady_clock::now() - t_begin).count());
    return levels;
}

void schedule_frame_stage(const Plan *pl, int64_t B, int nwg, std::vector<int4> &ft, std::vector<int> &fo, StageSchedule &ss) {
    const int rows = (int)(B + pl->m[0]->RF - 3);
    std::vector<SchedProb> fp;
    for (const auto &f : pl->frame_probs) {
        const Layer &L = pl->m[f.model]->layers[f.layer];
        SchedProb sp{rows, L.N, L.Kpad / BK, 1, std::max(1, std::min(3, (64 * 1024) / ((L.Kpad + 4) * 4 * 32)))};
        sp.nk2 = 2;
        fp.push_back(sp);
    }
    schedule_stage(fp, nwg, GEMM_SCHED_MAX_UNITS, ft, fo, ss, false);
}

bool forward_variant_table(const Plan *pl, int64_t B, int v, int nprob, std::vector<GemmProb> &rel, std::vector<unsigned char> &tags) {
    const Model *a = pl->m[0];
    const int uv = v & 1, shared = v >> 1;
    if (uv && a->cfg.in_features != 3) return false;
    if (shared && pl->frame_buf < 0) return false;
    rel.assign(nprob, GemmProb());
    tags.assign((size_t)nprob * BIND_NPTR, 0);
    Bases none;
    CallShape cs;
    cs.uv = uv != 0;
    cs.shared = shared != 0;
    if (shared) {
        cs.window_stride = 1;
        cs.frames = B + a->RF - 1;
    }
    for (int i = 0; i < nprob; ++i)
        if (fill_prob(pl, pl->probs[i], B, a, none, cs, rel[i], tags.data() + (size_t)i * BIND_NPTR) != R3D_OK) return false;
    return true;
}

int forward_kernel_of_lists(const Plan *pl, int64_t B, const std::vector<int> &ft, bool &narrow, bool &b3_tiles) {
    narrow = false;
    for (size_t t = 0; t * FWD_TILE_INT4 * 4 < ft.size(); ++t) narrow |= tile_is_narrow(ft[t * FWD_TILE_INT4 * 4 + 3]);
    b3_tiles = B >= b3_min_batch() && ((pl->m[0] && pl->m[0]->use_b3) || (pl->m[1] && pl->m[1]->use_b3));
    return narrow ? FWD_KERNEL_LAT : b3_tiles ? FWD_KERNEL_B3 : FWD_KERNEL_F32;
}

Schedule *schedule_get(Plan *pl, int64_t B, int nwg, bool pin, int lane) {
    const int64_t key = schedule_key(B, lane);
    auto it = pl->schedules.find(key);
    if (it != pl->schedules.end()) {
        auto pos = std::find(pl->schedule_lru.begin(), pl->schedule_lru.end(), key);
        if (pos != pl->schedule_lru.end() && pos + 1 != pl->schedule_lru.end()) std::rotate(pos, pos + 1, pl->schedule_lru.end());
        if (pin) it->second->pinned = true;
        return it->second;
    }
    {
        size_t unpinned = 0;
        for (int64_t b : pl->schedule_lru) unpinned += pl->schedules[b]->pinned ? 0 : 1;
        const size_t cap = 64 * (size_t)std::max(1, pl->m[0] ? pl->m[0]->lanes : 1);
        if (unpinned >= cap) {
            auto victim = std::find_if(pl->schedule_lru.begin(), pl->schedule_lru.end(), [&](int64_t b) { return !pl->schedules[b]->pinned; });
            if (victim != pl->schedule_lru.end() && hipDeviceSynchronize() == hipSuccess) {
                const int64_t old = *victim;
                pl->schedule_lru.erase(victim);
                for (const Model *mm : pl->m)
                    if (mm) const_cast<Model *>(mm)->last_clk_dev = nullptr;
                delete pl->schedules[old];
                pl->schedules.erase(old);
            } else {
                (void)hipGetLastError();
            }
        }
    }
    Schedule *s = new Schedule();
    s->B = B;
    std::vector<int4> tiles;
    std::vector<int> wgoff;
    s->levels = schedule_build_host(pl, B, nwg, s->spill_row0, tiles, wgoff, s->stages);
    hipError_t e;
    if ((e = hipMalloc((void **)&s->d_tiles, std::max<size_t>(tiles.size(), 1) * sizeof(int4))) != hipSuccess ||
        (e = hipMalloc((void **)&s->d_wgoff, std::max<size_t>(wgoff.size(), 1) * sizeof(int))) != hipSuccess ||
        (e = hipMemcpy(s->d_tiles, tiles.data(), tiles.size() * sizeof(int4), hipMemcpyHostToDevice)) != hipSuccess ||
        (e = hipMemcpy(s->d_wgoff, wgoff.data(), wgoff.size() * sizeof(int), hipMemcpyHostToDevice)) != hipSuccess) {
        hip_fail(e, "schedule upload");
        delete s;
        return nullptr;
    }
    if (pl->frame_buf >= 0) {
        std::vector<int4> ft;
        std::vector<int> fo;
        schedule_frame_stage(pl, B, nwg, ft, fo, s->frame_stage);
        if ((e = hipMalloc((void **)&s->d_frame_tiles, std::max<size_t>(ft.size(), 1) * sizeof(int4))) != hipSuccess ||
            (e = hipMalloc((void **)&s->d_frame_wgoff, std::max<size_t>(fo.size(), 1) * sizeof(int))) != hipSuccess ||
            (e = hipMemcpy(s->d_frame_tiles, ft.data(), ft.size() * sizeof(int4), hipMemcpyHostToDevice)) != hipSuccess ||
            (e = hipMemcpy(s->d_frame_wgoff, fo.data(), fo.size() * sizeof(int), hipMemcpyHostToDevice)) != hipSuccess) {
            hip_fail(e, "schedule upload (per-frame launch)");
            delete s;
            return nullptr;
        }
        s->frame_stage.tiles_off = s->frame_stage.wgoff_off = 0;
    }
    if (forward_single_launch()) {
        std::vector<int> ft, fo;
        Schedule::Fwd &fw = s->fwd;
        if (schedule_build_fwd(pl, B, nwg, *s->levels, s->stages, tiles, wgoff, fw, ft, fo)) {
            bool ok = (e = hipMalloc((void **)&fw.d_tiles, ft.size() * sizeof(int))) == hipSuccess &&
                      (e = hipMalloc((void **)&fw.d_wgoff, fo.size() * sizeof(int))) == hipSuccess &&
                      (e = hipMemcpy(fw.d_tiles, ft.data(), ft.size() * sizeof(int), hipMemcpyHostToDevice)) == hipSuccess &&
                      (e = hipMemcpy(fw.d_wgoff, fo.data(), fo.size() * sizeof(int), hipMemcpyHostToDevice)) == hipSuccess;
            for (int v = 0; ok && v < 4; ++v) {
                std::vector<GemmProb> rel;
                std::vector<unsigned char> tags;
                if (!forward_variant_table(pl, B, v, fw.nprob, rel, tags)) { if (v) continue; ok = false; break; }
                ok = (e = hipMalloc((void **)&fw.d_rel[v], rel.size() * sizeof(GemmProb))) == hipSuccess &&
                     (e = hipMalloc((void **)&fw.d_tags[v], tags.size())) == hipSuccess &&
                     (e = hipMemcpy(fw.d_rel[v], rel.data(), rel.size() * sizeof(GemmProb), hipMemcpyHostToDevice)) == hipSuccess &&
                     (e = hipMemcpy(fw.d_tags[v], tags.data(), tags.size(), hipMemcpyHostToDevice)) == hipSuccess;
            }
            fw.h_tiles = ft;
            fw.h_wgoff = fo;
            if (ok) {
                fw.bank_bytes = ((size_t)(fw.ncnt + 4) * sizeof(unsigned) + 255) / 256 * 256;
                ok = (e = hipMalloc((void **)&fw.d_ctrl, 2 * fw.bank_bytes + 2 * (size_t)fw.nprob * sizeof(GemmProb))) == hipSuccess;
            }
            bool narrow = false, b3_tiles = false;
            fw.kernel = forward_kernel_of_lists(pl, B, ft, narrow, b3_tiles);
            if (ok) {
                int cap = forward_resident_capacity(fw.kernel, false);
                auto also = [&](int kind, bool uvk) {
                    const int c = forward_resident_capacity(kind, uvk);
                    if (c > 0) cap = cap > 0 ? std::min(cap, c) : c;
                };
                if (fw.uses_gather && pl->m[0]->cfg.in_features == 3) also(fw.kernel, true);
                if (pl->frame_buf >= 0 && fw.kernel == FWD_KERNEL_F32) {
                    also(FWD_KERNEL_CLIP, false);
                    if (pl->m[0]->cfg.in_features == 3) also(FWD_KERNEL_CLIP, true);
                }
                const bool masked = getenv("HSA_CU_MASK") != nullptr || getenv("ROC_GLOBAL_CU_MASK") != nullptr;
                if ((narrow && b3_tiles) || (cap > 0 && fw.grid > cap) || masked) {
                    if (fw.d_tiles) (void)hipFree(fw.d_tiles);
                    if (fw.d_wgoff) (void)hipFree(fw.d_wgoff);
                    if (fw.d_ctrl) (void)hipFree(fw.d_ctrl);
                    for (int i = 0; i < 4; ++i) {
                        if (fw.d_rel[i]) (void)hipFree(fw.d_rel[i]);
                        if (fw.d_tags[i]) (void)hipFree(fw.d_tags[i]);
                    }
                    fw = Schedule::Fwd();
                    s->pinned = pin;
                    pl->schedules[key] = s;
                    pl->schedule_lru.push_back(key);
                    return s;
                }
            }
            if (ok && narrow && pl->kind == PLAN_SMALL && B <= 16) {
                fw.act_bytes = (((size_t)pl->floats_per_window * (size_t)B + (size_t)pl->tail_floats + 64) * sizeof(float) + 255) / 256 * 256;
                ok = (e = hipMalloc((void **)&fw.d_act, 2 * fw.act_bytes)) == hipSuccess;
            }
            if (!ok) {
                hip_fail(e, "schedule upload (single-launch form)");
                delete s;
                return nullptr;
            }
        } else {
            fw = Schedule::Fwd();
        }
    }
    s->pinned = pin;
    pl->schedules[key] = s;
    pl->schedule_lru.push_back(key);
    return s;
}

}
```

### ray3d_amd/csrc/r3d_tiles.hpp

```cpp
#pragma once
#include <hip/hip_runtime.h>

#include <algorithm>
#include <type_traits>

#include "r3d_internal.hpp"

namespace r3d {

#ifndef R3D_TS
#define R3D_TS 0
#endif
#ifdef R3D_TIMING
#define R3D_TSTAMP(slot) do { if (dbg && threadIdx.x == 0) dbg[slot] = wall_clock64(); } while (0)
#else
#define R3D_TSTAMP(slot) do { } while (0)
#endif

typedef float f32x16 __attribute__((ext_vector_type(16)));
typedef float f32x4 __attribute__((ext_vector_type(4)));

#define R3D_AS1 __attribute__((address_space(1)))
__device__ __forceinline__ f32x4 gload4(const float *p) { return *(const R3D_AS1 f32x4 *)p; }
__device__ __forceinline__ float gload1(const float *p) { return *(const R3D_AS1 float *)p; }
__device__ __forceinline__ void gstore1(float *p, float v) { *(R3D_AS1 float *)p = v; }
constexpr int ACT_AUX = 16;
typedef unsigned u32x4 __attribute__((ext_vector_type(4)));
typedef unsigned R3D_AS1 *gu32;
struct LateWait { int dw, ndep; gu32 cnt, abort_flag; long long spin_ticks; };
__device__ __forceinline__ void wait_deps_reg(const int dw, const int ndep, const gu32 cnt, const gu32 abort_flag, const long long spin_ticks);
__device__ __forceinline__ __amdgpu_buffer_rsrc_t act_rsrc(const float *base) {
    return __builtin_amdgcn_make_buffer_rsrc(const_cast<float *>(base), 0, 0x7fffffff, 0x00020000);
}
__device__ __forceinline__ f32x4 act_load4(__amdgpu_buffer_rsrc_t r, int byte_off) {
    return __builtin_bit_cast(f32x4, __builtin_amdgcn_raw_buffer_load_b128(r, byte_off, 0, ACT_AUX));
}
__device__ __forceinline__ float act_load1(__amdgpu_buffer_rsrc_t r, int byte_off) {
    return __builtin_bit_cast(float, __builtin_amdgcn_raw_buffer_load_b32(r, byte_off, 0, ACT_AUX));
}
__device__ __forceinline__ void act_store4(__amdgpu_buffer_rsrc_t r, int byte_off, f32x4 v) {
    __builtin_amdgcn_raw_buffer_store_b128(__builtin_bit_cast(u32x4, v), r, byte_off, 0, ACT_AUX);
}
__device__ __forceinline__ void act_store1(__amdgpu_buffer_rsrc_t r, int byte_off, float v) {
    __builtin_amdgcn_raw_buffer_store_b32(__builtin_bit_cast(unsigned, v), r, byte_off, 0, ACT_AUX);
}
__device__ __forceinline__ void tile_drain() { asm volatile("s_waitcnt vmcnt(0)" ::: "memory"); }
__device__ __forceinline__ void tile_signal(const gu32 cnt, const int sig_base, const int sig_add, const int units) {
    int t = threadIdx.x;
    asm volatile("" : "+v"(t));
    if (t < units) __hip_atomic_fetch_add(cnt + sig_base + t, (unsigned)sig_add, __ATOMIC_RELAXED, __HIP_MEMORY_SCOPE_AGENT);
}
__device__ __forceinline__ float lrelu(const float v, const float slope) { return __builtin_fmaxf(v, v * slope); }


constexpr int LDS_LD = BK + 4;
constexpr int GEMM_THREADS = 512;
constexpr int GEMM_BN = 256;
constexpr int GEMM_MAX_MI = 6;
constexpr int GEMM_STAGES = 3;
constexpr int STAGE_FLOATS = GEMM_MAX_MI * 32 * LDS_LD;
constexpr int LUT_LDS_INTS = 1152;
constexpr int RING_LDS_BYTES = GEMM_STAGES * STAGE_FLOATS * 4;
constexpr int GEMM_LDS_BYTES = 157952;
static_assert(GEMM_LDS_BYTES >= RING_LDS_BYTES, "the ring and the intermediate tile share the allocation");

typedef const LaunchArgs __attribute__((address_space(4))) *LaunchArgsPtr;
typedef const GemmProb __attribute__((address_space(4))) &ProbRef;

constexpr int EPI_LD = GEMM_BN + 4;

constexpr unsigned ACT_SENTINEL_BITS = 0x7fc5a1e7u;
__device__ __forceinline__ float act_canon(const float v) {
    return __builtin_bit_cast(unsigned, v) == ACT_SENTINEL_BITS ? __builtin_bit_cast(float, 0x7fc00000u) : v;
}

template <int MI, int KS>
__device__ __forceinline__ void store_tile(ProbRef P, const f32x16 (&acc)[MI], const int row0, const int col0, float *lds,
                                           const bool second = false) {
    constexpr int COLS = GEMM_BN / KS, WN = 8 / KS;
    constexpr int TPR = COLS / 4;
    constexpr int RPP = GEMM_THREADS / TPR;
    int tid = threadIdx.x;
    asm volatile("" : "+v"(tid));
    const int lane = tid & 63, wave = tid >> 6, li = lane & 31, lh = lane >> 5;
    const int M = P.M, N = P.N;
    const float slope = second ? P.slope2 : P.slope;
    const float *res = P.res;
    const bool canon = P.canon != 0;
    const int ldc = P.ldc, ldr = P.ldr;
    const __amdgpu_buffer_rsrc_t crs = act_rsrc(P.c + (size_t)row0 * ldc + col0);
    const __amdgpu_buffer_rsrc_t rrs = act_rsrc(res ? res + (size_t)row0 * ldr + col0 : P.c);
    const bool writer = wave < WN;
    const float bias = writer ? gload1((second ? P.bias2 : P.bias) + col0 + wave * 32 + li) : 0.0f;
    float *wr = lds + (4 * lh) * EPI_LD + wave * 32 + li;
    const int rd_row = tid / TPR, rd_c4 = (tid % TPR) * 4;
    const bool vec = (col0 + COLS <= N);
#pragma unroll
    for (int mi = 0; mi < MI; ++mi) {
        __syncthreads();
        if (writer) {
#pragma unroll
            for (int r = 0; r < 16; ++r) {
                float v = acc[mi][r] + bias;
                wr[((r & 3) + 8 * (r >> 2)) * EPI_LD] = lrelu(v, slope);
            }
        }
        __syncthreads();
#pragma unroll
        for (int j = 0; j < 32 / RPP; ++j) {
            const int lr = rd_row + RPP * j;
            const int row = row0 + mi * 32 + lr;
            if (row >= M) continue;
            f32x4 v = *reinterpret_cast<const f32x4 *>(lds + lr * EPI_LD + rd_c4);
            const int col = col0 + rd_c4;
            const int lrow = mi * 32 + lr;
            if (vec) {
                if (res) v += act_load4(rrs, (lrow * ldr + rd_c4) * 4);
                if (canon) {
#pragma unroll
                    for (int e = 0; e < 4; ++e) v[e] = act_canon(v[e]);
                }
                act_store4(crs, (lrow * ldc + rd_c4) * 4, v);
            } else {
#pragma unroll
                for (int e = 0; e < 4; ++e)
                    if (col + e < N) {
                        const float o = v[e] + (res ? act_load1(rrs, (lrow * ldr + rd_c4 + e) * 4) : 0.0f);
                        act_store1(crs, (lrow * ldc + rd_c4 + e) * 4, canon ? act_canon(o) : o);
                    }
            }
        }
    }
    __syncthreads();
}

constexpr int PAIR_LD = GEMM_BN + 4;
constexpr int PAIR_MAX_MI = 4;
template <int MI, int KS, bool PAIR = false>
__device__ __forceinline__ void gemm_tile(ProbRef P, const int row0, const int col0, float *smem, long long *dbg, const LateWait late = LateWait{0, 0, nullptr, nullptr, 0}) {
    static_assert(!PAIR || (KS == 1 && MI <= PAIR_MAX_MI), "fused pairs are whole tiles of at most 128 rows");
    constexpr int SF = STAGE_FLOATS;
    R3D_TSTAMP(0);
    static_assert(KS == 1 || (KS == 2 && MI <= 2) || (KS == 4 && MI == 1), "split-K tiles are small tiles");
    constexpr int WN = 8 / KS;
    constexpr int VR = KS * MI * 32;
    constexpr int NA = (VR + 63) / 64;
    constexpr bool PRE = MI <= 3;
    constexpr bool WD2 = MI <= 4;
    constexpr int AD = WD2 ? 5 : 4;
    int tid = threadIdx.x;
    asm volatile("" : "+v"(tid));
    const int lane = tid & 63, wave = tid >> 6;
    const int li = lane & 31, lh = lane >> 5;
    const int wn = wave % WN;
    const int wk = wave / WN;
    const int M = P.M, K = P.K;
    const int nk32 = K / BK;
    const int nk = (nk32 + KS - 1) / KS;
    const int srow = tid >> 3, a_kq = (tid & 7) * 4;

    const bool multi = P.kend[0] < K;
    int seg_ld = P.lda[0], seg_k0 = 0, seg_end = P.kend[0], seg_i = 0;
    int a_voff[NA];
    __amdgpu_buffer_rsrc_t arsrc;
    auto open_seg = [&]() {
        const float *base = P.a[seg_i] + (size_t)row0 * seg_ld;
        const long long b = ((long long)(M - 1 - row0) * seg_ld + (seg_end < K ? seg_end : K) - seg_k0) * 4;
        arsrc = __builtin_amdgcn_make_buffer_rsrc(const_cast<float *>(base), 0, b < 0x7fffffffLL ? (int)b : 0x7fffffff, 0x00020000);
#pragma unroll
        for (int i = 0; i < NA; ++i) {
            const int vr = srow + 64 * i, sub = KS == 1 ? 0 : (vr / (MI * 32) < KS ? vr / (MI * 32) : KS - 1);
            const int gr = row0 + vr - sub * (MI * 32);
            a_voff[i] = (((gr < M ? gr : M - 1) - row0) * seg_ld + a_kq + sub * BK) * 4;
        }
    };
    open_seg();
    auto prep_seg = [&](int kt) {
        if (!multi) return;
        while (kt * (BK * KS) >= seg_end) {
            ++seg_i;
            seg_k0 = seg_end;
            seg_ld = P.lda[seg_i];
            seg_end = P.kend[seg_i];
            open_seg();
        }
    };
    struct Staged {
        f32x4 a[NA];
    };
    Staged ra, ra2, ra3;
    auto issue_a = [&](int kt, Staged &R) {
        const int kb = kt * (BK * KS) - seg_k0;
#pragma unroll
        for (int i = 0; i < NA; ++i)
            R.a[i] = __builtin_bit_cast(f32x4, __builtin_amdgcn_raw_buffer_load_b128(arsrc, a_voff[i], kb * 4, ACT_AUX));
    };
    const int st_off = srow * LDS_LD + a_kq;
    auto commit_a = [&](int stage, const Staged &R) {
        float *s = stage == 0 ? smem + st_off : stage == 1 ? smem + SF + st_off : smem + 2 * SF + st_off;
        {
#pragma unroll
            for (int i = 0; i < NA; ++i) *reinterpret_cast<f32x4 *>(s + i * 64 * LDS_LD) = R.a[i];
        }
    };

    const int wave_u = __builtin_amdgcn_readfirstlane(wave);
    __amdgpu_buffer_rsrc_t wrsrc = __builtin_amdgcn_make_buffer_rsrc(
        const_cast<float *>(P.w + ((size_t)((col0 >> 5) + wave_u % WN) * nk32 + wave_u / WN) * 1024), 0,
        (nk32 - wave_u / WN) * 4096, 0x00020000);
    const int w_voff = lane * 16;
    f32x4 rb[4], rbn[4], rbn2[4];
    auto load_w = [&](int kt, f32x4 (&dst)[4]) {
#pragma unroll
        for (int q = 0; q < 4; ++q)
            dst[q] = __builtin_bit_cast(f32x4, __builtin_amdgcn_raw_buffer_load_b128(
                wrsrc, w_voff + q * 1024, kt * KS * 4096, 0));
    };

    f32x16 acc[MI];
#pragma unroll
    for (int mi = 0; mi < MI; ++mi)
#pragma unroll
        for (int r = 0; r < 16; ++r) acc[mi][r] = 0.0f;

    const int a_frag = (wk * MI * 32 + li) * LDS_LD + lh * 16;
    f32x4 av0[PRE ? MI : 1];

    const int last = nk - 1;
    load_w(0, rb);
    if (WD2) load_w(1 < last ? 1 : last, rbn);
    if (late.ndep > 0) wait_deps_reg(late.dw, late.ndep, late.cnt, late.abort_flag, late.spin_ticks);
    {
        Staged r0, r1;
        issue_a(0, r0);
        prep_seg(1 < last ? 1 : last);
        issue_a(1 < last ? 1 : last, r1);
        prep_seg(2 < last ? 2 : last);
        issue_a(2 < last ? 2 : last, ra);
        prep_seg(3 < last ? 3 : last);
        issue_a(3 < last ? 3 : last, ra2);
        prep_seg(4 < last ? 4 : last);
        if (WD2) {
            issue_a(4 < last ? 4 : last, ra3);
            prep_seg(5 < last ? 5 : last);
        }
        if (P.kend[0] < BK) {
            const int width = P.kend[0];
#pragma unroll
            for (int i = 0; i < NA; ++i)
#pragma unroll
                for (int e = 0; e < 4; ++e)
                    if (a_kq + e >= width) r0.a[i][e] = 0.0f;
        }
        commit_a(0, r0);
        commit_a(1, r1);
    }
    __syncthreads();
    if (PRE) {
#pragma unroll
        for (int mi = 0; mi < MI; ++mi) av0[mi] = *reinterpret_cast<const f32x4 *>(smem + a_frag + mi * 32 * LDS_LD);
    }
    R3D_TSTAMP(1);
    int st_cur = 0;
    auto k_tile = [&](int kt, f32x4 (&w_use)[4], f32x4 (&w_load)[4], Staged &stg) {
        const int st_next = st_cur == 2 ? 0 : st_cur + 1, st_next2 = st_next == 2 ? 0 : st_next + 1;
        const float *s = smem + st_cur * SF + a_frag;
        const bool active = KS == 1 || kt * KS + wave_u / WN < nk32;
        auto mfma_q = [&](int q) {
            if (!active) return;
            f32x4 av[MI];
#pragma unroll
            for (int mi = 0; mi < MI; ++mi) {
                if (PRE && q == 0) av[mi] = av0[mi];
                else av[mi] = *reinterpret_cast<const f32x4 *>(s + mi * 32 * LDS_LD + q * 4);
            }
#pragma unroll
            for (int kk = 0; kk < 4; ++kk)
#pragma unroll
                for (int mi = 0; mi < MI; ++mi)
                    acc[mi] = __builtin_amdgcn_mfma_f32_32x32x2f32(av[mi][kk], w_use[q][kk], acc[mi], 0, 0, 0);
        };
        constexpr bool INTERLEAVE = MI >= 3;
        if (!INTERLEAVE) {
            commit_a(st_next2, stg);
            load_w(kt + (WD2 ? 2 : 1) < last ? kt + (WD2 ? 2 : 1) : last, w_load);
            issue_a(kt + AD < last ? kt + AD : last, stg);
            prep_seg(kt + AD + 1 < last ? kt + AD + 1 : last);
        }
        mfma_q(0);
        if (INTERLEAVE) {
            commit_a(st_next2, stg);
            load_w(kt + (WD2 ? 2 : 1) < last ? kt + (WD2 ? 2 : 1) : last, w_load);
        }
        mfma_q(1);
        if (INTERLEAVE) {
            issue_a(kt + AD < last ? kt + AD : last, stg);
            prep_seg(kt + AD + 1 < last ? kt + AD + 1 : last);
        }
        mfma_q(2);
        mfma_q(3);
        if (PRE) {
            const float *sn = smem + st_next * SF + a_frag;
#pragma unroll
            for (int mi = 0; mi < MI; ++mi) av0[mi] = *reinterpret_cast<const f32x4 *>(sn + mi * 32 * LDS_LD);
        }
        __syncthreads();
        st_cur = st_next;
    };
    int kt = 0;
    if (WD2) {
        for (; kt + 2 < nk; kt += 3) {
            k_tile(kt, rb, rbn2, ra);
            k_tile(kt + 1, rbn, rb, ra2);
            k_tile(kt + 2, rbn2, rbn, ra3);
        }
        if (kt < nk) {
            k_tile(kt, rb, rbn2, ra);
            if (kt + 1 < nk) k_tile(kt + 1, rbn, rb, ra2);
        }
    } else {
        for (; kt + 1 < nk; kt += 2) {
            k_tile(kt, rb, rbn, ra);
            k_tile(kt + 1, rbn, rb, ra2);
        }
        if (kt < nk) k_tile(kt, rb, rbn, ra);
    }

    R3D_TSTAMP(2);
    if (KS > 1) {
        constexpr int PHASE_FLOATS = WN * MI * 16 * 64;
        float *red = smem + ((wn * MI) * 16) * 64 + lane;
        if (wk > 0) {
            float *mine = red + wk * PHASE_FLOATS;
#pragma unroll
            for (int mi = 0; mi < MI; ++mi)
#pragma unroll
                for (int r = 0; r < 16; ++r) mine[(mi * 16 + r) * 64] = acc[mi][r];
        }
        __syncthreads();
        if (wk == 0) {
#pragma unroll
            for (int ph = 1; ph < KS; ++ph)
#pragma unroll
                for (int mi = 0; mi < MI; ++mi)
#pragma unroll
                    for (int r = 0; r < 16; ++r) acc[mi][r] += red[ph * PHASE_FLOATS + (mi * 16 + r) * 64];
        }
    }
    R3D_TSTAMP(3);
    if constexpr (PAIR) {
        const float slope1 = P.slope;
        const float bias1 = gload1(P.bias + wave * 32 + li);
        __syncthreads();
#pragma unroll
        for (int mi = 0; mi < MI; ++mi) {
            float *wr = smem + (mi * 32 + 4 * lh) * PAIR_LD + wave * 32 + li;
#pragma unroll
            for (int r = 0; r < 16; ++r) {
                const float v = acc[mi][r] + bias1;
                wr[((r & 3) + 8 * (r >> 2)) * PAIR_LD] = lrelu(v, slope1);
            }
        }
        __syncthreads();
        const int nk2 = P.K2 / BK;
        __amdgpu_buffer_rsrc_t w2rsrc = __builtin_amdgcn_make_buffer_rsrc(
            const_cast<float *>(P.w2 + ((size_t)wave_u * nk2) * 1024), 0, nk2 * 4096, 0x00020000);
        auto load_w2 = [&](int kt, f32x4 (&dst)[4]) {
#pragma unroll
            for (int q = 0; q < 4; ++q)
                dst[q] = __builtin_bit_cast(f32x4, __builtin_amdgcn_raw_buffer_load_b128(w2rsrc, w_voff + q * 1024, kt * 4096, 0));
        };
#pragma unroll
        for (int mi = 0; mi < MI; ++mi)
#pragma unroll
            for (int r = 0; r < 16; ++r) acc[mi][r] = 0.0f;
        const float *h_frag = smem + li * PAIR_LD + lh * 16;
        const int last2 = nk2 - 1;
        auto k_tile2 = [&](int kt2, f32x4 (&w_use)[4], f32x4 (&w_load)[4]) {
            load_w2(kt2 + 2 < last2 ? kt2 + 2 : last2, w_load);
            __builtin_amdgcn_sched_barrier(0);
            const float *s = h_frag + kt2 * BK;
#pragma unroll
            for (int q = 0; q < 4; ++q) {
                f32x4 av[MI];
#pragma unroll
                for (int mi = 0; mi < MI; ++mi) av[mi] = *reinterpret_cast<const f32x4 *>(s + mi * 32 * PAIR_LD + q * 4);
#pragma unroll
                for (int kk = 0; kk < 4; ++kk)
#pragma unroll
                    for (int mi = 0; mi < MI; ++mi)
                        acc[mi] = __builtin_amdgcn_mfma_f32_32x32x2f32(av[mi][kk], w_use[q][kk], acc[mi], 0, 0, 0);
            }
        };
        load_w2(0, rb);
        load_w2(1 < last2 ? 1 : last2, rbn);
        int kt2 = 0;
        for (; kt2 + 2 < nk2; kt2 += 3) {
            k_tile2(kt2, rb, rbn2);
            k_tile2(kt2 + 1, rbn, rb);
            k_tile2(kt2 + 2, rbn2, rbn);
        }
        if (kt2 < nk2) {
            k_tile2(kt2, rb, rbn2);
            if (kt2 + 1 < nk2) k_tile2(kt2 + 1, rbn, rb);
        }
        store_tile<MI, 1>(P, acc, row0, col0, smem, true);
    } else {
        store_tile<MI, KS>(P, acc, row0, col0, smem);
    }
    R3D_TSTAMP(4);
}

template <int NB>
__device__ __forceinline__ void gemm_tile_nb(ProbRef P, const int row0, const int col0, float *smem, long long *dbg, const LateWait late = LateWait{0, 0, nullptr, nullptr, 0}) {
    static_assert(NB >= 4 && NB <= 7, "NB = 8 is gemm_tile<1, 1>");
    constexpr int SF = STAGE_FLOATS;
    constexpr int NX = NB - 4;
    constexpr int AD = 5;
    R3D_TSTAMP(0);
    int tid = threadIdx.x;
    asm volatile("" : "+v"(tid));
    const int lane = tid & 63, wave = tid >> 6;
    const int li = lane & 31, lh = lane >> 5;
    const int wave_u = __builtin_amdgcn_readfirstlane(wave);
    const bool main_w = wave_u < 4;
    const int M = P.M, K = P.K;
    const int nk = K / BK;
    const int srow = tid >> 3, a_kq = (tid & 7) * 4;
    const int xg0 = (wave_u - 4) * NX;
    int s_blk[4], s_q[4];
#pragma unroll
    for (int s = 0; s < 4; ++s) {
        const int sc = s < NX ? s : 0;
        s_blk[s] = main_w ? wave_u : (NX > 0 ? 4 + (xg0 + sc) / 4 : wave_u - 4);
        s_q[s] = main_w ? s : (NX > 0 ? (xg0 + sc) & 3 : 0);
    }
    const bool multi = P.kend[0] < K;
    int seg_ld = P.lda[0], seg_k0 = 0, seg_end = P.kend[0], seg_i = 0;
    int a_voff;
    __amdgpu_buffer_rsrc_t arsrc;
    auto open_seg = [&]() {
        const float *base = P.a[seg_i] + (size_t)row0 * seg_ld;
        const long long b = ((long long)(M - 1 - row0) * seg_ld + (seg_end < K ? seg_end : K) - seg_k0) * 4;
        arsrc = __builtin_amdgcn_make_buffer_rsrc(const_cast<float *>(base), 0, b < 0x7fffffffLL ? (int)b : 0x7fffffff, 0x00020000);
        const int gr = row0 + (srow & 31);
        a_voff = (((gr < M ? gr : M - 1) - row0) * seg_ld + a_kq) * 4;
    };
    open_seg();
    auto prep_seg = [&](int kt) {
        if (!multi) return;
        while (kt * BK >= seg_end) {
            ++seg_i;
            seg_k0 = seg_end;
            seg_ld = P.lda[seg_i];
            seg_end = P.kend[seg_i];
            open_seg();
        }
    };
    f32x4 ra, ra2, ra3;
    auto issue_a = [&](int kt, f32x4 &R) {
        R = __builtin_bit_cast(f32x4, __builtin_amdgcn_raw_buffer_load_b128(arsrc, a_voff, (kt * BK - seg_k0) * 4, ACT_AUX));
    };
    const int st_off = srow * LDS_LD + a_kq;
    auto commit_a = [&](int stage, const f32x4 &R) {
        float *sp = stage == 0 ? smem + st_off : stage == 1 ? smem + SF + st_off : smem + 2 * SF + st_off;
        *reinterpret_cast<f32x4 *>(sp) = R;
    };
    __amdgpu_buffer_rsrc_t wrsrc = __builtin_amdgcn_make_buffer_rsrc(
        const_cast<float *>(P.w + (size_t)(col0 >> 5) * nk * 1024), 0, NB * nk * 4096, 0x00020000);
    const int w_voff = lane * 16;
    int w_soff[4], a_off[4];
#pragma unroll
    for (int s = 0; s < 4; ++s) {
        w_soff[s] = __builtin_amdgcn_readfirstlane((s_blk[s] * nk) * 4096 + s_q[s] * 1024);
        a_off[s] = li * LDS_LD + lh * 16 + s_q[s] * 4;
    }
    const int last = nk - 1;
    auto k_loop = [&](auto ns_tag, auto nacc_tag, f32x16 *acc) {
        constexpr int NS = decltype(ns_tag)::value, NACC = decltype(nacc_tag)::value;
        constexpr int NSL = NS > 0 ? NS : 1;
        f32x4 rb[NSL], rbn[NSL], rbn2[NSL];
        auto load_w = [&](int kt, f32x4 (&dst)[NSL]) {
            if (NS == 0) return;
#pragma unroll
            for (int s = 0; s < NSL; ++s)
                dst[s] = __builtin_bit_cast(f32x4, __builtin_amdgcn_raw_buffer_load_b128(wrsrc, w_voff, w_soff[s] + kt * 4096, 0));
        };
        load_w(0, rb);
        load_w(1 < last ? 1 : last, rbn);
        if (late.ndep > 0) wait_deps_reg(late.dw, late.ndep, late.cnt, late.abort_flag, late.spin_ticks);
        {
            f32x4 r0, r1;
            issue_a(0, r0);
            prep_seg(1 < last ? 1 : last);
            issue_a(1 < last ? 1 : last, r1);
            prep_seg(2 < last ? 2 : last);
            issue_a(2 < last ? 2 : last, ra);
            prep_seg(3 < last ? 3 : last);
            issue_a(3 < last ? 3 : last, ra2);
            prep_seg(4 < last ? 4 : last);
            issue_a(4 < last ? 4 : last, ra3);
            prep_seg(5 < last ? 5 : last);
            commit_a(0, r0);
            commit_a(1, r1);
        }
        __syncthreads();
        f32x4 av0 = *reinterpret_cast<const f32x4 *>(smem + a_off[0]);
        R3D_TSTAMP(1);
        int st_cur = 0;
        auto k_tile = [&](int kt, f32x4 (&w_use)[NSL], f32x4 (&w_load)[NSL], f32x4 &stg) {
            const int st_next = st_cur == 2 ? 0 : st_cur + 1, st_next2 = st_next == 2 ? 0 : st_next + 1;
            const float *sp = smem + st_cur * SF;
            commit_a(st_next2, stg);
            load_w(kt + 2 < last ? kt + 2 : last, w_load);
            issue_a(kt + AD < last ? kt + AD : last, stg);
            prep_seg(kt + AD + 1 < last ? kt + AD + 1 : last);
#pragma unroll
            for (int s = 0; s < NS; ++s) {
                const f32x4 av = s == 0 ? av0 : *reinterpret_cast<const f32x4 *>(sp + a_off[s]);
#pragma unroll
                for (int kk = 0; kk < 4; ++kk)
                    acc[s % NACC] = __builtin_amdgcn_mfma_f32_32x32x2f32(av[kk], w_use[s][kk], acc[s % NACC], 0, 0, 0);
            }
            if (NS > 0) av0 = *reinterpret_cast<const f32x4 *>(smem + st_next * SF + a_off[0]);
            __syncthreads();
            st_cur = st_next;
        };
        int kt = 0;
        for (; kt + 2 < nk; kt += 3) {
            k_tile(kt, rb, rbn2, ra);
            k_tile(kt + 1, rbn, rb, ra2);
            k_tile(kt + 2, rbn2, rbn, ra3);
        }
        if (kt < nk) {
            k_tile(kt, rb, rbn2, ra);
            if (kt + 1 < nk) k_tile(kt + 1, rbn, rb, ra2);
        }
    };
    constexpr int PART = 16 * 64;
    f32x16 fin;
    if (main_w) {
        f32x16 acc[1];
#pragma unroll
        for (int r = 0; r < 16; ++r) acc[0][r] = 0.0f;
        k_loop(std::integral_constant<int, 4>{}, std::integral_constant<int, 1>{}, acc);
        fin = acc[0];
        R3D_TSTAMP(2);
        if (NX > 0) __syncthreads();
    } else {
        constexpr int NA_ = NX > 0 ? NX : 1;
        f32x16 acc[NA_];
#pragma unroll
        for (int a = 0; a < NA_; ++a)
#pragma unroll
            for (int r = 0; r < 16; ++r) acc[a][r] = 0.0f;
        k_loop(std::integral_constant<int, NX>{}, std::integral_constant<int, NA_>{}, acc);
        if (NX > 0) {
            float *red = smem + lane;
#pragma unroll
            for (int a = 0; a < NX; ++a)
#pragma unroll
                for (int r = 0; r < 16; ++r) red[(xg0 + a) * PART + r * 64] = acc[a][r];
            __syncthreads();
#pragma unroll
            for (int r = 0; r < 16; ++r) fin[r] = 0.0f;
            if (wave_u < NB) {
                const float *src = red + (wave_u - 4) * 4 * PART;
#pragma unroll
                for (int g = 0; g < 4; ++g)
#pragma unroll
                    for (int r = 0; r < 16; ++r) fin[r] += src[g * PART + r * 64];
            }
        }
    }
    R3D_TSTAMP(3);
    {
        constexpr int COLS = NB * 32, TPR = COLS / 4;
        const int N = P.N;
        const float slope = P.slope;
        const float *res = P.res;
        const int ldc = P.ldc, ldr = P.ldr;
        const __amdgpu_buffer_rsrc_t crs = act_rsrc(P.c + (size_t)row0 * ldc + col0);
        const __amdgpu_buffer_rsrc_t rrs = act_rsrc(res ? res + (size_t)row0 * ldr + col0 : P.c);
        const bool writer = wave_u < NB;
        const float bias = writer ? gload1(P.bias + col0 + wave * 32 + li) : 0.0f;
        __syncthreads();
        if (writer) {
            float *wr = smem + (4 * lh) * EPI_LD + wave * 32 + li;
#pragma unroll
            for (int r = 0; r < 16; ++r) wr[((r & 3) + 8 * (r >> 2)) * EPI_LD] = lrelu(fin[r] + bias, slope);
        }
        __syncthreads();
        const bool vec = col0 + COLS <= N;
#pragma unroll
        for (int it = 0; it < (32 * TPR + GEMM_THREADS - 1) / GEMM_THREADS; ++it) {
            const int c = tid + it * GEMM_THREADS;
            if (c >= 32 * TPR) break;
            const int lr = c / TPR, c4 = (c % TPR) * 4;
            if (row0 + lr >= M) continue;
            f32x4 v = *reinterpret_cast<const f32x4 *>(smem + lr * EPI_LD + c4);
            if (vec) {
                if (res) v += act_load4(rrs, (lr * ldr + c4) * 4);
                act_store4(crs, (lr * ldc + c4) * 4, v);
            } else {
#pragma unroll
                for (int e = 0; e < 4; ++e)
                    if (col0 + c4 + e < N) act_store1(crs, (lr * ldc + c4 + e) * 4, v[e] + (res ? act_load1(rrs, (lr * ldr + c4 + e) * 4) : 0.0f));
            }
        }
        __syncthreads();
    }
    R3D_TSTAMP(4);
}

typedef __bf16 bf16x8 __attribute__((ext_vector_type(8)));
typedef __bf16 bf16x2 __attribute__((ext_vector_type(2)));
typedef float f32x2 __attribute__((ext_vector_type(2)));
constexpr int B3_LD = 20;

__device__ __forceinline__ unsigned b3_pack(float a, float b) {
    const f32x2 v = {a, b};
    return __builtin_bit_cast(unsigned, __builtin_convertvector(v, bf16x2));
}
__device__ __forceinline__ float b3_lo(unsigned u) { return __builtin_bit_cast(float, u << 16); }
__device__ __forceinline__ float b3_hi(unsigned u) { return __builtin_bit_cast(float, u & 0xffff0000u); }

__device__ __forceinline__ void b3_split8(const f32x4 &a, const f32x4 &b, bf16x8 (&pl)[3]) {
    typedef unsigned u32x4 __attribute__((ext_vector_type(4)));
    const float x[8] = {a[0], a[1], a[2], a[3], b[0], b[1], b[2], b[3]};
    u32x4 p0, p1, p2;
#ifdef R3D_EXP_NOSPLIT_W
#pragma unroll
    for (int i = 0; i < 4; ++i) p0[i] = p1[i] = p2[i] = b3_pack(x[2 * i], x[2 * i + 1]);
    pl[0] = __builtin_bit_cast(bf16x8, p0);
    pl[1] = __builtin_bit_cast(bf16x8, p1);
    pl[2] = __builtin_bit_cast(bf16x8, p2);
    return;
#endif
#pragma unroll
    for (int i = 0; i < 4; ++i) {
        const unsigned h = b3_pack(x[2 * i], x[2 * i + 1]);
        const float r0 = x[2 * i] - b3_lo(h), r1 = x[2 * i + 1] - b3_hi(h);
        const unsigned m = b3_pack(r0, r1);
        p0[i] = h;
        p1[i] = m;
        p2[i] = b3_pack(r0 - b3_lo(m), r1 - b3_hi(m));
    }
    pl[0] = __builtin_bit_cast(bf16x8, p0);
    pl[1] = __builtin_bit_cast(bf16x8, p1);
    pl[2] = __builtin_bit_cast(bf16x8, p2);
}

typedef unsigned u32x2 __attribute__((ext_vector_type(2)));
__device__ __forceinline__ void b3_split4(const f32x4 &x, u32x2 (&pl)[3]);

template <int MI>
__device__ __forceinline__ void gemm_tile_b3(ProbRef P, const int row0, const int col0, float *smem, long long *dbg) {
    R3D_TSTAMP(0);
    constexpr int VR = MI * 32, NA = (VR + 63) / 64;
    constexpr int PLANE = VR * B3_LD, SFB = 3 * PLANE;
    static_assert(3 * SFB * 4 <= GEMM_LDS_BYTES, "three stages of three planes must fit");
    int tid = threadIdx.x;
    asm volatile("" : "+v"(tid));
    const int lane = tid & 63, wave = tid >> 6;
    const int li = lane & 31, lh = lane >> 5;
    const int M = P.M, K = P.K;
    const int nk = K / BK;
    const int srow = tid >> 3, a_kq = (tid & 7) * 4;
    const bool multi = P.kend[0] < K;
    int seg_ld = P.lda[0], seg_k0 = 0, seg_end = P.kend[0], seg_i = 0;
    int a_voff[NA];
    __amdgpu_buffer_rsrc_t arsrc;
    auto open_seg = [&]() {
        const float *base = P.a[seg_i] + (size_t)row0 * seg_ld;
        const long long b = ((long long)(M - 1 - row0) * seg_ld + (seg_end < K ? seg_end : K) - seg_k0) * 4;
        arsrc = __builtin_amdgcn_make_buffer_rsrc(const_cast<float *>(base), 0, b < 0x7fffffffLL ? (int)b : 0x7fffffff, 0x00020000);
#pragma unroll
        for (int i = 0; i < NA; ++i) {
            const int gr = row0 + srow + 64 * i;
            a_voff[i] = (((gr < M ? gr : M - 1) - row0) * seg_ld + a_kq) * 4;
        }
// ... 1531 lines not shown
            if (!dep.poll || !__any(missing) || poll_gave_up(spins, t_first, dep.abort_flag, dep.spin_ticks)) break;
        }
    }
    float eres = 0.0f;
    if (emit && P.res) {
        unsigned spins = 0;
        long long t_first = 0;
        do eres = act_ld(P.res + (size_t)er * P.ldr + ecol);
        while (dep.poll && act_missing(eres) && !poll_gave_up(spins, t_first, dep.abort_flag, dep.spin_ticks));
    }
    __syncthreads();
    float acc[GEMV_MAX_M];
#pragma unroll
    for (int r = 0; r < GEMV_MAX_M; ++r) acc[r] = 0.0f;
    for (int j0 = 0; wave_u + 8 * j0 < nk32; j0 += 4) {
        if (j0) load_round(j0);
#pragma unroll
        for (int j = 0; j < 4; ++j) {
            const int kt = wave_u + 8 * (j0 + j);
            if (kt >= nk32) break;
#pragma unroll
            for (int q = 0; q < 4; ++q)
#pragma unroll
                for (int r = 0; r < GEMV_MAX_M; ++r) {
                    const f32x4 a = *reinterpret_cast<const f32x4 *>(As + (r < M ? r : M - 1) * ldA + kt * BK + lh * 16 + q * 4);
                    acc[r] += a[0] * wf[j][q][0] + a[1] * wf[j][q][1] + a[2] * wf[j][q][2] + a[3] * wf[j][q][3];
                }
        }
    }
#pragma unroll
    for (int r = 0; r < GEMV_MAX_M; ++r) {
        acc[r] += __shfl_xor(acc[r], 32, 64);
        if (lh == 0) red[(wave * GEMV_MAX_M + r) * 32 + li] = acc[r];
    }
    __syncthreads();
    if (emit) {
        float v = 0.0f;
#pragma unroll
        for (int w = 0; w < 8; ++w) v += red[(w * GEMV_MAX_M + er) * 32 + (tid & 31)];
        v = lrelu(v + ebias, P.slope) + eres;
        act_st(P.c + (size_t)er * P.ldc + ecol, v);
    }
    __syncthreads();
}

__device__ __forceinline__ void lat_tile(ProbRef P, const int col0, float *smem, const TileDeps &dep) {
    int tid = threadIdx.x;
    asm volatile("" : "+v"(tid));
    const int lane = tid & 63, wave = tid >> 6, li = lane & 31, lh = lane >> 5;
    const int wave_u = __builtin_amdgcn_readfirstlane(wave);
    const int M = P.M, K = P.K, N = P.N, nk32 = K / BK;
    __amdgpu_buffer_rsrc_t wrsrc = __builtin_amdgcn_make_buffer_rsrc(
        const_cast<float *>(P.w + (size_t)(col0 >> 5) * nk32 * 1024), 0, nk32 * 4096, 0x00020000);
    const int e0 = P.kend[0], e1 = P.kend[1], e2 = P.kend[2];
    const int arow = li < M ? li : M - 1;
    f32x4 wf[4][4], af[4][4];
    auto load_w_round = [&](int j0) {
#pragma unroll
        for (int j = 0; j < 4; ++j)
#pragma unroll
            for (int q = 0; q < 4; ++q)
                wf[j][q] = __builtin_bit_cast(f32x4, __builtin_amdgcn_raw_buffer_load_b128(wrsrc, lane * 16 + q * 1024, (wave_u + 8 * (j0 + j)) * 4096, 0));
    };
    auto load_a_round = [&](int j0) {
#pragma unroll
        for (int j = 0; j < 4; ++j) {
            const int kt = wave_u + 8 * (j0 + j), k = kt * BK;
            const int sg = k < e0 ? 0 : k < e1 ? 1 : k < e2 ? 2 : 3;
            const int k0 = sg == 0 ? 0 : sg == 1 ? e0 : sg == 2 ? e1 : e2;
            const float *base = sg == 0 ? P.a[0] : sg == 1 ? P.a[1] : sg == 2 ? P.a[2] : P.a[3];
            const int ld = sg == 0 ? P.lda[0] : sg == 1 ? P.lda[1] : sg == 2 ? P.lda[2] : P.lda[3];
            const __amdgpu_buffer_rsrc_t ars = act_rsrc(base);
            const bool live = kt < nk32;
#pragma unroll
            for (int q = 0; q < 4; ++q)
                af[j][q] = live ? act_load4(ars, (arow * ld + (k - k0) + lh * 16 + q * 4) * 4) : f32x4{0.0f, 0.0f, 0.0f, 0.0f};
        }
    };
    f32x16 acc;
#pragma unroll
    for (int r = 0; r < 16; ++r) acc[r] = 0.0f;
    load_w_round(0);
    float ebias[2], eres[2] = {0.0f, 0.0f};
    int erow[2], ecol[2];
#pragma unroll
    for (int h = 0; h < 2; ++h) {
        const int idx = tid + h * GEMM_THREADS, r = idx >> 6, ln = idx & 63;
        erow[h] = (r & 3) + 8 * (r >> 2) + 4 * (ln >> 5);
        ecol[h] = col0 + (ln & 31);
        ebias[h] = erow[h] < M && ecol[h] < N ? gload1(P.bias + ecol[h]) : 0.0f;
    }
    if (dep.ndep > 0 && !dep.poll) wait_deps(dep.tile, dep.ndep, dep.cnt, dep.abort_flag, dep.spin_ticks);
    if (P.res) {
#pragma unroll
        for (int h = 0; h < 2; ++h)
            if (erow[h] < M && ecol[h] < N) eres[h] = act_ld(P.res + (size_t)erow[h] * P.ldr + ecol[h]);
    }
    unsigned spins = 0;
    long long t_first = 0;
    for (int j0 = 0; wave_u + 8 * j0 < nk32; j0 += 4) {
        if (j0) load_w_round(j0);
        for (;;) {
            load_a_round(j0);
            if (!dep.poll) break;
            bool missing = false;
#pragma unroll
            for (int j = 0; j < 4; ++j)
#pragma unroll
                for (int q = 0; q < 4; ++q)
#pragma unroll
                    for (int kk = 0; kk < 4; ++kk) missing |= act_missing(af[j][q][kk]);
            if (!__any(missing) || poll_gave_up(spins, t_first, dep.abort_flag, dep.spin_ticks)) break;
        }
#ifdef R3D_TIMING
        if (j0 == 0 && dep.tstamp && threadIdx.x == 0) dep.tstamp[1] = wall_clock64();
#endif
#pragma unroll
        for (int j = 0; j < 4; ++j) {
            if (wave_u + 8 * (j0 + j) >= nk32) break;
#pragma unroll
            for (int q = 0; q < 4; ++q)
#pragma unroll
                for (int kk = 0; kk < 4; ++kk)
                    acc = __builtin_amdgcn_mfma_f32_32x32x2f32(af[j][q][kk], wf[j][q][kk], acc, 0, 0, 0);
        }
    }
    float *red = smem;
#pragma unroll
    for (int r = 0; r < 16; ++r) red[(wave * 16 + r) * 64 + lane] = acc[r];
    __syncthreads();
#pragma unroll
    for (int h = 0; h < 2; ++h) {
        const int idx = tid + h * GEMM_THREADS, r = idx >> 6, ln = idx & 63;
        float v = 0.0f;
#pragma unroll
        for (int w = 0; w < 8; ++w) v += red[(w * 16 + r) * 64 + ln];
        const int row = erow[h], col = ecol[h];
        if (row < M && col < N) {
            v = lrelu(v + ebias[h], P.slope);
            if (P.res) {
                float rv = eres[h];
                unsigned rspins = 0;
                long long rt = 0;
                while (dep.poll && act_missing(rv) && !poll_gave_up(rspins, rt, dep.abort_flag, dep.spin_ticks)) rv = act_ld(P.res + (size_t)row * P.ldr + col);
                v += rv;
            }
            act_st(P.c + (size_t)row * P.ldc + col, v);
        }
    }
    __syncthreads();
}

typedef const FwdArgs __attribute__((address_space(4))) *FwdArgsPtr;
__device__ __forceinline__ void wait_deps_reg(const int dw, const int ndep, const gu32 cnt, const gu32 abort_flag, const long long spin_ticks) {
    if (threadIdx.x < 64) {
        const int lane = threadIdx.x;
        int total = 0;
        for (int d = 0; d < ndep; ++d) total += __builtin_amdgcn_readlane(dw, 9 + 2 * d) & 0xffff;
        for (int off = 0; off < total; off += 64) {
            int idx = -1, acc = 0;
            unsigned need = 0;
            for (int d = 0; d < ndep; ++d) {
                const int base = __builtin_amdgcn_readlane(dw, 8 + 2 * d), nw = __builtin_amdgcn_readlane(dw, 9 + 2 * d);
                const int n = nw & 0xffff, l = lane + off - acc;
                if (l >= 0 && l < n) { idx = base + l; need = (unsigned)nw >> 16; }
                acc += n;
            }
            long long t_first = 0;
            for (unsigned spins = 1;; ++spins) {
                const unsigned v = idx >= 0 ? __hip_atomic_load(cnt + idx, __ATOMIC_RELAXED, __HIP_MEMORY_SCOPE_AGENT) : need;
                if (__all(v >= need)) break;
                __builtin_amdgcn_s_sleep(4);
                if ((spins & 31) == 0) {
                    if (__hip_atomic_load(abort_flag, __ATOMIC_RELAXED, __HIP_MEMORY_SCOPE_AGENT) != 0) break;
                    const long long now = wall_clock64();
                    if (t_first == 0) t_first = now;
                    else if (now - t_first > spin_ticks) {
                        if (lane == 0) __hip_atomic_store(abort_flag, 1u, __ATOMIC_RELAXED, __HIP_MEMORY_SCOPE_AGENT);
                        break;
                    }
                }
            }
        }
    }
    __syncthreads();
}
__device__ __forceinline__ void wait_deps(const int4 *tile, const int ndep, const gu32 cnt, const gu32 abort_flag, const long long spin_ticks) {
    if (threadIdx.x < 64) {
        const int lane = threadIdx.x;
        const int *ti = reinterpret_cast<const int *>(tile);
        int total = 0;
        for (int d = 0; d < ndep; ++d) total += __builtin_amdgcn_readfirstlane(ti[9 + 2 * d]) & 0xffff;
        for (int off = 0; off < total; off += 64) {
            int idx = -1, acc = 0;
            unsigned need = 0;
            for (int d = 0; d < ndep; ++d) {
                const int base = __builtin_amdgcn_readfirstlane(ti[8 + 2 * d]), nw = __builtin_amdgcn_readfirstlane(ti[9 + 2 * d]);
                const int n = nw & 0xffff, l = lane + off - acc;
                if (l >= 0 && l < n) { idx = base + l; need = (unsigned)nw >> 16; }
                acc += n;
            }
            long long t_first = 0;
            for (unsigned spins = 1;; ++spins) {
                const unsigned v = idx >= 0 ? __hip_atomic_load(cnt + idx, __ATOMIC_RELAXED, __HIP_MEMORY_SCOPE_AGENT) : need;
                if (__all(v >= need)) break;
                __builtin_amdgcn_s_sleep(4);
                if ((spins & 31) == 0) {
                    if (__hip_atomic_load(abort_flag, __ATOMIC_RELAXED, __HIP_MEMORY_SCOPE_AGENT) != 0) break;
                    const long long now = wall_clock64();
                    if (t_first == 0) t_first = now;
                    else if (now - t_first > spin_ticks) {
                        if (lane == 0) __hip_atomic_store(abort_flag, 1u, __ATOMIC_RELAXED, __HIP_MEMORY_SCOPE_AGENT);
                        break;
                    }
                }
            }
        }
    }
    __syncthreads();
}

constexpr int FWD_TILE_NOSIGNAL = 1;
__device__ __forceinline__ void gemv_run(FwdArgsPtr fargs, const int4 *tl, const int TS, const int n, float *smem, const gu32 cnt,
                                         const gu32 abort_flag, int &gemv_seen, long long *dbg_arg, const int t_first_tile) {
    const long long spin_ticks = fargs->spin_ticks;
    int tid = threadIdx.x;
    asm volatile("" : "+v"(tid));
    const int lane = tid & 63, wave = tid >> 6, li = lane & 31, lh = lane >> 5;
    const int wave_u = __builtin_amdgcn_readfirstlane(wave);
    const bool poll = fargs->poll != 0;
    typedef const GemmProb __attribute__((address_space(4))) *ProbPtr;
    auto prob_of = [&](int i) -> ProbPtr {
        return (ProbPtr)fargs->probs + (__builtin_amdgcn_readfirstlane(tl[i * TS].x) & 0xff);
    };
    auto request = [&](ProbPtr P, int col0, int j0, f32x4 (&wf)[4][4]) {
        const int nk32 = P->K / BK;
        __amdgpu_buffer_rsrc_t wrsrc = __builtin_amdgcn_make_buffer_rsrc(
            const_cast<float *>(P->w + (size_t)(col0 >> 5) * nk32 * 1024), 0, nk32 * 4096, 0x00020000);
#pragma unroll
        for (int j = 0; j < 4; ++j)
#pragma unroll
            for (int q = 0; q < 4; ++q)
                wf[j][q] = __builtin_bit_cast(f32x4, __builtin_amdgcn_raw_buffer_load_b128(wrsrc, lane * 16 + q * 1024, (wave_u + 8 * (j0 + j)) * 4096, 0));
    };
    f32x4 wa[4][4], wb[4][4];
    request(prob_of(0), __builtin_amdgcn_readfirstlane(tl[0].z), 0, wa);
    auto body = [&](const int i, f32x4 (&wf)[4][4], f32x4 (&wnext)[4][4]) {
        const int4 *tile = tl + i * TS;
        ProbPtr Pp = prob_of(i);
        ProbRef P = *Pp;
        const int col0 = __builtin_amdgcn_readfirstlane(tile[0].z);
        const int4 te = tile[1];
        const int ndep = __builtin_amdgcn_readfirstlane(te.x), sig_base = __builtin_amdgcn_readfirstlane(te.y);
        const int sig_add = __builtin_amdgcn_readfirstlane(te.z), flags = __builtin_amdgcn_readfirstlane(te.w);
#ifdef R3D_TIMING
        if (dbg_arg && threadIdx.x == 0) dbg_arg[16384 + (long long)(t_first_tile + i) * 4 + 0] = wall_clock64();
#endif
        const int M = P.M, K = P.K, N = P.N, nk32 = K / BK;
        const int ldA = K + 8;
        float *As = smem, *red = smem + GEMV_MAX_M * ldA;
        const int er = tid >> 5, ecol = col0 + (tid & 31);
        const bool emit = tid < M * 32 && ecol < N;
        const float ebias = emit ? gload1(P.bias + ecol) : 0.0f;
        if (ndep > 0 && !poll) wait_deps(tile, ndep, cnt, abort_flag, spin_ticks);
        {
            const int e0 = P.kend[0], e1 = P.kend[1], e2 = P.kend[2];
            const float *a0 = P.a[0], *a1 = P.a[1], *a2 = P.a[2], *a3 = P.a[3];
            const int l0 = P.lda[0], l1 = P.lda[1], l2 = P.lda[2], l3 = P.lda[3];
            unsigned spins = 0;
            long long t_first = 0;
            for (;;) {
                bool missing = false;
                for (int r = 0; r < M; ++r)
                    for (int k = tid; k < K; k += GEMM_THREADS) {
                        const float *src = k < e0 ? a0 + (size_t)r * l0 + k : k < e1 ? a1 + (size_t)r * l1 + (k - e0)
                                         : k < e2 ? a2 + (size_t)r * l2 + (k - e1) : a3 + (size_t)r * l3 + (k - e2);
                        const float v = act_ld(src);
                        missing |= act_missing(v);
                        As[r * ldA + k] = v;
                    }
                if (!poll || !__any(missing) || poll_gave_up(spins, t_first, abort_flag, spin_ticks)) break;
            }
        }
        float eres = 0.0f;
        if (emit && P.res) {
            unsigned spins = 0;
            long long t_first = 0;
            do eres = act_ld(P.res + (size_t)er * P.ldr + ecol);
            while (poll && act_missing(eres) && !poll_gave_up(spins, t_first, abort_flag, spin_ticks));
        }
        if (i + 1 < n) request(prob_of(i + 1), __builtin_amdgcn_readfirstlane(tl[(i + 1) * TS].z), 0, wnext);
        __syncthreads();
#ifdef R3D_TIMING
        if (dbg_arg && threadIdx.x == 0) dbg_arg[16384 + (long long)(t_first_tile + i) * 4 + 1] = wall_clock64();
#endif
        float acc[GEMV_MAX_M];
#pragma unroll
        for (int r = 0; r < GEMV_MAX_M; ++r) acc[r] = 0.0f;
        for (int j0 = 0; wave_u + 8 * j0 < nk32; j0 += 4) {
            if (j0) request(Pp, col0, j0, wf);
#pragma unroll
            for (int r = 0; r < GEMV_MAX_M; ++r) {
                if (r >= M) break;
#pragma unroll
                for (int j = 0; j < 4; ++j) {
                    const int kt = wave_u + 8 * (j0 + j);
                    if (kt >= nk32) break;
#pragma unroll
                    for (int q = 0; q < 4; ++q) {
                        const f32x4 a = *reinterpret_cast<const f32x4 *>(As + r * ldA + kt * BK + lh * 16 + q * 4);
                        acc[r] += a[0] * wf[j][q][0] + a[1] * wf[j][q][1] + a[2] * wf[j][q][2] + a[3] * wf[j][q][3];
                    }
                }
            }
        }
#pragma unroll
        for (int r = 0; r < GEMV_MAX_M; ++r) {
            acc[r] += __shfl_xor(acc[r], 32, 64);
            if (lh == 0) red[(wave * GEMV_MAX_M + r) * 32 + li] = acc[r];
        }
        __syncthreads();
        const bool faulty = blockIdx.x == 0 && gemv_seen++ == fargs->fault_tile1 - 1;
        if (emit && !faulty) {
            float v = 0.0f;
#pragma unroll
            for (int w = 0; w < 8; ++w) v += red[(w * GEMV_MAX_M + er) * 32 + (tid & 31)];
            v = lrelu(v + ebias, P.slope) + eres;
            act_st(P.c + (size_t)er * P.ldc + ecol, v);
        }
        if (!(poll && (flags & FWD_TILE_NOSIGNAL))) {
            tile_drain();
            __syncthreads();
            if (!faulty) tile_signal(cnt, sig_base, sig_add, 1);
        } else {
            __syncthreads();
        }
#ifdef R3D_TIMING
        if (dbg_arg && threadIdx.x == 0) {
            dbg_arg[16384 + (long long)(t_first_tile + i) * 4 + 2] = wall_clock64();
            dbg_arg[16384 + (long long)(t_first_tile + i) * 4 + 3] = 1;
        }
#endif
    };
    int i = 0;
    for (; i + 1 < n; i += 2) {
        body(i, wa, wb);
        body(i + 1, wb, wa);
    }
    if (i < n) body(i, wa, wb);
}

template <bool ENC, bool UV, bool DEP = false, bool B3 = true, bool NARROW = true, bool CLIP = !DEP>
__device__ __forceinline__ void gemm_persistent(float *smem) {
    LaunchArgsPtr args = (LaunchArgsPtr)__builtin_amdgcn_kernarg_segment_ptr();
    FwdArgsPtr fargs = (FwdArgsPtr)__builtin_amdgcn_kernarg_segment_ptr();
    constexpr int TS = DEP ? FWD_TILE_INT4 : 1;
    int wg = blockIdx.x;
    if constexpr (!DEP) {
        const int n = gridDim.x, q = n >> 3, r = n & 7, xcd = wg & 7, idx = wg >> 3;
        wg = (xcd < r ? xcd * (q + 1) : r * (q + 1) + (xcd - r) * q) + idx;
    }
    const int4 *tiles = DEP ? fargs->tiles : args->tiles;
    const int *wg_off = DEP ? fargs->wg_off : args->wg_off;
    const gu32 cnt = DEP ? (gu32)fargs->cnt : (gu32) nullptr;
    const gu32 abort_flag = DEP ? (gu32)(fargs->cnt + fargs->ncnt) : (gu32) nullptr;
    const int t0 = __builtin_amdgcn_readfirstlane(wg_off[wg]);
    const int t1 = __builtin_amdgcn_readfirstlane(wg_off[wg + 1]);
    if constexpr (DEP) {
        unsigned *nx = fargs->cnt_next;
        if (nx != nullptr)
            for (int j = blockIdx.x * GEMM_THREADS + threadIdx.x; j < fargs->ncnt + 4; j += gridDim.x * GEMM_THREADS) nx[j] = 0u;
        typedef unsigned u32x4 __attribute__((ext_vector_type(4)));
        u32x4 *arm = NARROW ? reinterpret_cast<u32x4 *>(fargs->arm) : nullptr;
        if (arm != nullptr) {
            const u32x4 sv = {ACT_SENTINEL, ACT_SENTINEL, ACT_SENTINEL, ACT_SENTINEL};
            for (long long j = blockIdx.x * GEMM_THREADS + threadIdx.x; j < fargs->arm_vec4; j += gridDim.x * GEMM_THREADS) arm[j] = sv;
        }
    }
    if (DEP && blockIdx.x == 0 && threadIdx.x == 0) {
        fargs->cnt[fargs->ncnt + 2] = (unsigned)__builtin_readcyclecounter();
        fargs->cnt[fargs->ncnt + 3] = (unsigned)wall_clock64();
    }
    long long *dbg = nullptr;
#ifdef R3D_TIMING
    long long *dbg_arg = DEP ? fargs->dbg : args->dbg;
    long long *dbg_base = dbg_arg && wg < 16 ? dbg_arg + 6144 + wg * 64 : nullptr;
    if (dbg_arg && threadIdx.x == 0) {
        dbg_arg[1024 + wg * 4 + 0] = __builtin_readcyclecounter();
        dbg_arg[1024 + wg * 4 + 2] = wall_clock64();
    }
#endif
    int prev_pi = -1;
    int plain_seen = 0, gemv_seen = 0;
    for (int t = t0; t < t1; ++t) {
        int dw = 0;
        if constexpr (DEP) {
            int dl = threadIdx.x & 63;
            asm volatile("" : "+v"(dl));
            dw = reinterpret_cast<const int *>(tiles + t * TS)[dl < FWD_TILE_INT4 * 4 ? dl : 0];
        }
        int4 td;
        if constexpr (DEP) td = make_int4(__builtin_amdgcn_readlane(dw, 0), __builtin_amdgcn_readlane(dw, 1), __builtin_amdgcn_readlane(dw, 2), __builtin_amdgcn_readlane(dw, 3));
        else td = tiles[t * TS];
        const int pi = __builtin_amdgcn_readfirstlane(td.x & 0xff);
        const bool new_prob = pi != prev_pi;
        prev_pi = pi;
        const int mi = __builtin_amdgcn_readfirstlane(td.x >> 8);
        const int row0 = __builtin_amdgcn_readfirstlane(td.y);
        const int col0 = __builtin_amdgcn_readfirstlane(td.z);
        const int ks = __builtin_amdgcn_readfirstlane(td.w);
        int sig_base = 0, sig_add = 0, tflags = 0;
        LateWait late{0, 0, nullptr, nullptr, 0};
        TileDeps tdep{nullptr, 0, nullptr, nullptr, false, nullptr, 0};
        if constexpr (DEP) {
            const int4 te = make_int4(__builtin_amdgcn_readlane(dw, 4), __builtin_amdgcn_readlane(dw, 5), __builtin_amdgcn_readlane(dw, 6), __builtin_amdgcn_readlane(dw, 7));
            const int ndep = __builtin_amdgcn_readfirstlane(te.x);
            sig_base = __builtin_amdgcn_readfirstlane(te.y);
            sig_add = __builtin_amdgcn_readfirstlane(te.z);
            tflags = __builtin_amdgcn_readfirstlane(te.w);
#ifdef R3D_TIMING
            if (dbg_arg && threadIdx.x == 0) dbg_arg[16384 + (long long)t * 4 + 0] = wall_clock64();
#endif
#ifndef R3D_TIMING
            constexpr bool LATE = !B3 && !ENC;
#else
            constexpr bool LATE = false;
#endif
            const bool wait_here = ndep > 0 && (!NARROW || !tile_is_narrow(ks));
            if (wait_here && !LATE) wait_deps_reg(dw, ndep, cnt, abort_flag, fargs->spin_ticks);
            if (wait_here && LATE) late = LateWait{dw, ndep, cnt, abort_flag, fargs->spin_ticks};
#ifdef R3D_TIMING
            if (dbg_arg && threadIdx.x == 0) dbg_arg[16384 + (long long)t * 4 + 1] = wall_clock64();
#endif
            tdep = TileDeps{tiles + t * TS, NARROW && tile_is_narrow(ks) ? ndep : 0, cnt, abort_flag, NARROW && fargs->poll != 0, nullptr, fargs->spin_ticks};
#ifdef R3D_TIMING
            if (dbg_arg) tdep.tstamp = dbg_arg + 16384 + (long long)t * 4;
#endif
        }
        ProbRef P = DEP ? *((const GemmProb __attribute__((address_space(4))) *)fargs->probs + pi) : args->p[pi];
#ifdef R3D_TIMING
        dbg = dbg_base && t - t0 < 8 ? dbg_base + (t - t0) * 8 : nullptr;
#endif
        bool signalled = false;
        do {
        if constexpr (ENC) {
            (void)ks;
            switch (mi) {
                case 1: enc_tile<1, UV>(P, row0, col0, new_prob, smem, dbg); break;
                case 2: enc_tile<2, UV>(P, row0, col0, new_prob, smem, dbg); break;
                default: enc_tile<3, UV>(P, row0, col0, new_prob, smem, dbg); break;
            }
        } else {
            if (P.w3 != nullptr) {
                int n = 1;
                while (t + n < t1 && __builtin_amdgcn_readfirstlane(tiles[(t + n) * TS].x) == __builtin_amdgcn_readfirstlane(td.x)) ++n;
#ifdef R3D_TIMING
                long long *run_dbg = dbg_base && t - t0 < 8 ? dbg_base + (t - t0) * 8 : nullptr;
#else
                long long *run_dbg = nullptr;
#endif
                const int4 *tl = tiles + t * TS;
                if (CLIP && P.lut == nullptr) {
                  if constexpr (CLIP) {
                    if (mi >= 2) first_level_shared<2>(P, tl, TS, n, smem, cnt, run_dbg);
                    else first_level_shared<1>(P, tl, TS, n, smem, cnt, run_dbg);
                  }
                } else if (B3 && P.wb3 != nullptr) {
                  if constexpr (B3) {
                    if (P.K <= 64) {
                        if (mi >= 2) first_level_taps_b3<2, false, UV>(P, tl, TS, n, new_prob, smem, cnt, run_dbg);
                        else first_level_taps_b3<1, false, UV>(P, tl, TS, n, new_prob, smem, cnt, run_dbg);
                    } else {
                        if (mi >= 2) first_level_taps_b3<2, true, UV>(P, tl, TS, n, new_prob, smem, cnt, run_dbg);
                        else first_level_taps_b3<1, true, UV>(P, tl, TS, n, new_prob, smem, cnt, run_dbg);
                    }
                  }
                } else if (P.K <= 64) {
                    if (mi >= 2) first_level_taps<2, false, UV>(P, tl, TS, n, new_prob, smem, cnt, run_dbg);
                    else first_level_taps<1, false, UV>(P, tl, TS, n, new_prob, smem, cnt, run_dbg);
                } else {
                    if (mi >= 2) first_level_taps<2, true, UV>(P, tl, TS, n, new_prob, smem, cnt, run_dbg);
                    else first_level_taps<1, true, UV>(P, tl, TS, n, new_prob, smem, cnt, run_dbg);
                }
#ifdef R3D_TIMING
                if (DEP && dbg_arg && threadIdx.x == 0) {
                    dbg_arg[16384 + (long long)t * 4 + 2] = wall_clock64();
                    dbg_arg[16384 + (long long)t * 4 + 3] = n;
                }
#endif
                t += n - 1;
                signalled = true;
                break;
            }
            if (P.lut != nullptr) {
                switch (mi) {
                    case 1: enc_tile<1, UV>(P, row0, col0, new_prob, smem, dbg); break;
                    case 2: enc_tile<2, UV>(P, row0, col0, new_prob, smem, dbg); break;
                    default: enc_tile<3, UV>(P, row0, col0, new_prob, smem, dbg); break;
                }
                break;
            }
            if constexpr (B3) {
            if (P.wb3 != nullptr && P.w2 != nullptr) {
                if (mi >= 3) gemm_tile_b3t<3>(P, row0, smem, dbg);
                else if (mi == 2) gemm_tile_b3t<2>(P, row0, smem, dbg);
                else gemm_tile_b3t<1>(P, row0, smem, dbg);
                break;
            }
            if (P.wb3 != nullptr) {
                switch (mi) {
                    case 1: gemm_tile_b3p<1>(P, row0, col0, smem, dbg); break;
                    case 2: gemm_tile_b3<2>(P, row0, col0, smem, dbg); break;
                    case 3: gemm_tile_b3<3>(P, row0, col0, smem, dbg); break;
                    default: gemm_tile_b3<4>(P, row0, col0, smem, dbg); break;
                }
                break;
            }
            }
            if constexpr (NARROW) {
            if (ks == 8) {
                if constexpr (DEP) {
                    int n = 1;
                    while (t + n < t1 && __builtin_amdgcn_readfirstlane(tiles[(t + n) * TS].w) == 8) ++n;
#ifdef R3D_TIMING
                    long long *run_dbg_arg = dbg_arg;
#else
                    long long *run_dbg_arg = nullptr;
#endif
                    gemv_run(fargs, tiles + t * TS, TS, n, smem, cnt, abort_flag, gemv_seen, run_dbg_arg, t);
                    t += n - 1;
                    signalled = true;
                    break;
                }
                gemv_tile(P, col0, smem, tdep);
                break;
            }
            if (ks == 16) {
                lat_tile(P, col0, smem, tdep);
                break;
            }
            }
            if (ks > NB_CODE) {
                if (ks == NB_CODE + 4) gemm_tile_nb<4>(P, row0, col0, smem, dbg, late);
                else if (ks == NB_CODE + 5) gemm_tile_nb<5>(P, row0, col0, smem, dbg, late);
                else if (ks == NB_CODE + 6) gemm_tile_nb<6>(P, row0, col0, smem, dbg, late);
                else gemm_tile_nb<7>(P, row0, col0, smem, dbg, late);
                break;
            }
            if (ks > 1) {
                if (ks == 4) gemm_tile<1, 4>(P, row0, col0, smem, dbg, late);
                else if (mi == 1) gemm_tile<1, 2>(P, row0, col0, smem, dbg, late);
                else gemm_tile<2, 2>(P, row0, col0, smem, dbg, late);
                break;
            }
            if (P.w2 != nullptr) {
                switch (mi) {
                    case 1: gemm_tile<1, 1, true>(P, row0, col0, smem, dbg, late); break;
                    case 2: gemm_tile<2, 1, true>(P, row0, col0, smem, dbg, late); break;
                    case 3: gemm_tile<3, 1, true>(P, row0, col0, smem, dbg, late); break;
                    default: gemm_tile<4, 1, true>(P, row0, col0, smem, dbg, late); break;
                }
                break;
            }
            switch (mi) {
                case 1: gemm_tile<1, 1>(P, row0, col0, smem, dbg, late); break;
                case 2: gemm_tile<2, 1>(P, row0, col0, smem, dbg, late); break;
                case 3: gemm_tile<3, 1>(P, row0, col0, smem, dbg, late); break;
                case 4: gemm_tile<4, 1>(P, row0, col0, smem, dbg, late); break;
                case 5: gemm_tile<5, 1>(P, row0, col0, smem, dbg, late); break;
                default: gemm_tile<6, 1>(P, row0, col0, smem, dbg, late); break;
            }
        }
        } while (false);
        if constexpr (DEP) {
            if (NARROW && !signalled && fargs->poll != 0 && (tflags & FWD_TILE_NOSIGNAL)) {
                signalled = true;
#ifdef R3D_TIMING
                if (dbg_arg && threadIdx.x == 0) {
                    dbg_arg[16384 + (long long)t * 4 + 2] = wall_clock64();
                    dbg_arg[16384 + (long long)t * 4 + 3] = 1;
                }
#endif
            }
            if (!signalled) {
                tile_drain();
                __syncthreads();
                if (!(blockIdx.x == 0 && plain_seen++ == fargs->fault_tile1 - 1)) tile_signal(cnt, sig_base, sig_add, mi);
#ifdef R3D_TIMING
                if (dbg_arg && threadIdx.x == 0) {
                    dbg_arg[16384 + (long long)t * 4 + 2] = wall_clock64();
                    dbg_arg[16384 + (long long)t * 4 + 3] = 1;
                }
// ... 27 lines not shown
```

Baseline: 456,600 poses/s.

## Add workgroup affinity placement, rotated K order and split dependency waits to fused forward

Adds a schedule pass that places each chunk of a big GEMM stage on the workgroup that produced its input tile, instead of the fixed XCD round-robin order. It also lets tiles start their K loop at their own column so already-local data is consumed first; this rotation only turns on when the R3D_ROT hook is set. Multi-segment tiles now wait only on the early dependencies before starting, and wait for the rest after a few K iterations. The goal is to hide inter-tile dependency spin time and reuse cache locality, at the cost of more scheduling complexity and possible load imbalance from the changed placement.

Result: no change. 454,900 poses/s (-0.4%).

```diff
diff --git a/include/ray3d_hip.h b/include/ray3d_hip.h
--- a/include/ray3d_hip.h
+++ b/include/ray3d_hip.h
@@ -215,6 +215,9 @@
 
 int r3d_debug_forward_check(r3d_model *pos, r3d_model *trj, int64_t batch, int nwg, int *tiles, int *counters);
 
+int r3d_debug_forward_tiles(r3d_model *pos, r3d_model *trj, int64_t batch, int nwg, int32_t *tiles, int cap_tiles,
+                            int32_t *wg_off, int cap_wg, int32_t *rot_src, int cap_prob, int *grid);
+
 typedef struct r3d_census_row {
     int32_t launch;
     int32_t blocks;
diff --git a/ray3d_amd/_capi.py b/ray3d_amd/_capi.py
--- a/ray3d_amd/_capi.py
+++ b/ray3d_amd/_capi.py
@@ -25,7 +25,7 @@
     "r3d_clips_encode", "r3d_clips_valid_losses", "r3d_clips_valid_scratch_bytes", "r3d_clips_poses",
 )
 HOOK_EXPORTS = ("r3d_debug_schedule_check", "r3d_debug_plan_check", "r3d_debug_forward_check",
-                "r3d_debug_forward_census", "r3d_debug_census_domain",
+                "r3d_debug_forward_tiles", "r3d_debug_forward_census", "r3d_debug_census_domain",
                 "r3d_debug_undistort_host", "r3d_debug_encode_px_host", "r3d_debug_valid_losses_host",
                 "r3d_debug_clips_encode_host", "r3d_debug_clips_valid_losses_host", "r3d_debug_clips_poses_host")
 ABI_VERSION = 6
diff --git a/ray3d_amd/csrc/r3d_forward.cpp b/ray3d_amd/csrc/r3d_forward.cpp
--- a/ray3d_amd/csrc/r3d_forward.cpp
+++ b/ray3d_amd/csrc/r3d_forward.cpp
@@ -668,6 +668,7 @@
         if (q.enc_lut >= 0 && q.enc_kernel) ++n_enc;
         const int rc = fill_prob(pl, q, c.B, c.a, c.bases, c.shape, la.p[i], nullptr);
         if (rc != R3D_OK) return rc;
+        la.p[i].rot = c.sched->rot_prob[st[i] & ~STAGE_SPILL_IN];
     }
     if (n_enc != 0 && n_enc != la.nprob) { set_error("internal: launch mixes encoded and plain operands"); return R3D_ERR_STATE; }
     if ((n_enc != 0) != (ss.kind == STAGE_ENC)) { set_error("internal: schedule and plan disagree on the launch kind"); return R3D_ERR_STATE; }
diff --git a/ray3d_amd/csrc/r3d_hooks.cpp b/ray3d_amd/csrc/r3d_hooks.cpp
--- a/ray3d_amd/csrc/r3d_hooks.cpp
+++ b/ray3d_amd/csrc/r3d_hooks.cpp
@@ -294,6 +294,38 @@
                 const int r1 = std::min(d[1] + mi * 32, M);
                 const int w0 = d[1] / q.rows_per_window, w1 = (r1 - 1) / q.rows_per_window + 1;
                 const Acc wr = writes(q);
+                {
+                    const int rot = fwd_tile_rot(d[7]), n_early = fwd_tile_n_early(d[7]), late_at = fwd_tile_late_at(d[7]);
+                    const int nk = pl->m[q.model]->layers[q.layer].Kpad / BK, ks = d[3];
+                    const bool rot_kind = mi == 1 && (ks == 1 || tile_is_nb(ks)) && q.enc_lut < 0 && q.layer2 < 0;
+                    if ((rot || n_early || late_at) && !rot_kind) return -27;
+                    if (late_at > FWD_LATE_MAX || n_early > d[4] || (late_at == 0 && n_early != 0) || (late_at > 0 && (nk < 8 || n_early >= d[4]))) return -27;
+                    const int reach = late_at > 0 ? late_at - 1 + FWD_A_AHEAD : 0;
+                    if (rot || (late_at > 0 && q.nseg == 1)) {
+                        if (q.nseg != 1 || q.rot_src < 0 || rot * BK != d[2] || rot >= nk || n_early != 0) return -28;
+                        if (reach * BK > tile_width(ks)) return -28;
+                        bool own = false;
+                        for (int t = fo[w]; t < next[w] && !own; ++t) {
+                            const int *o = &ft[(size_t)t * TI];
+                            own = (o[0] & 0xff) == q.rot_src && o[0] >> 8 == 1 && o[1] == d[1] && o[2] == d[2] && o[3] == ks;
+                        }
+                        if (!own) return -29;
+                    } else if (late_at > 0) {
+                        if (q.nseg < 2 || n_early < 1 || reach * BK > q.seg[0].width) return -30;
+                        const Acc rd{q.seg[0].buf, q.seg[0].col, q.seg[0].col + q.seg[0].width};
+                        for (int o = 0; o < id; ++o) {
+                            const ProbSpec &oq = pl->probs[o];
+                            if (pl->buffers[rd.buf].external != 0 || !overlap(rd, writes(oq))) continue;
+                            const int oM = (int)(batch * oq.rows_per_window);
+                            const int a0 = w0 * oq.rows_per_window, a1 = std::min(w1 * oq.rows_per_window, oM);
+                            const int c0 = fw.cnt_base[o] + a0 / 32, c1 = fw.cnt_base[o] + (a1 + 31) / 32;
+                            bool covered = a1 <= a0;
+                            for (int k = 0; k < n_early && !covered; ++k)
+                                covered = d[8 + 2 * k] <= c0 && c1 <= d[8 + 2 * k] + (d[9 + 2 * k] & 0xffff) && ((unsigned)d[9 + 2 * k] >> 16) == (unsigned)gcols[o];
+                            if (!covered) return -31;
+                        }
+                    }
+                }
                 for (int o = 0; o < id; ++o) {
                     const ProbSpec &oq = pl->probs[o];
                     bool hazard = false;
@@ -318,6 +350,29 @@
         for (int u = 0; u < (int)((batch * pl->probs[i].rows_per_window + 31) / 32); ++u)
             if (cnt[fw.cnt_base[i] + u] != (unsigned)gcols[i]) return -24;
     return 0;
+}
+
+int r3d_debug_forward_tiles(r3d_model *pos, r3d_model *trj, int64_t batch, int nwg, int32_t *tiles_out, int cap_tiles, int32_t *wg_off,
+                            int cap_wg, int32_t *rot_src, int cap_prob, int *grid) {
+    const ModelPair mp = model_pair(pos, trj);
+    if (!mp.a || !tiles_out || !wg_off) return -1;
+    Plan *pl = plan_get(mp.a, mp.b, plan_kind(batch));
+    if (!pl) return -2;
+    int spill_row0 = -1;
+    std::vector<int4> tiles;
+    std::vector<int> wgoff;
+    std::vector<StageSchedule> stages;
+    const std::vector<std::vector<int>> &levels = *schedule_build_host(pl, batch, nwg, spill_row0, tiles, wgoff, stages);
+    Schedule::Fwd fw;
+    std::vector<int> ft, fo;
+    if (!schedule_build_fwd(pl, batch, nwg, levels, stages, tiles, wgoff, fw, ft, fo)) return 0;
+    if (fw.ntiles > cap_tiles || fw.grid > cap_wg) return -3;
+    std::copy(ft.begin(), ft.end(), tiles_out);
+    std::copy(fo.begin(), fo.begin() + fw.grid + 1, wg_off);
+    if (rot_src)
+        for (int i = 0; i < (int)pl->probs.size() && i < cap_prob; ++i) rot_src[i] = pl->probs[i].rot_src;
+    if (grid) *grid = fw.grid;
+    return fw.ntiles;
 }
 
 int r3d_debug_forward_census(r3d_model *pos, r3d_model *trj, int64_t batch, int nwg, int32_t uv, int64_t cam_stride, int64_t window_stride,
diff --git a/ray3d_amd/csrc/r3d_internal.hpp b/ray3d_amd/csrc/r3d_internal.hpp
--- a/ray3d_amd/csrc/r3d_internal.hpp
+++ b/ray3d_amd/csrc/r3d_internal.hpp
@@ -53,6 +53,7 @@
     unsigned enc_bytes;
     int res_tap;
     int canon;
+    int rot;
     const double *cam;
     long long cam_stride;
 };
@@ -68,6 +69,12 @@
 
 constexpr int FWD_TILE_INT4 = 6;
 constexpr int FWD_MAX_DEP = 8;
+constexpr int FWD_A_AHEAD = 5;
+constexpr int FWD_LATE_MAX = 4;
+__host__ __device__ constexpr int fwd_tile_rot(int f) { return (f >> 8) & 0xff; }
+__host__ __device__ constexpr int fwd_tile_n_early(int f) { return (f >> 16) & 0xf; }
+__host__ __device__ constexpr int fwd_tile_late_at(int f) { return (f >> 20) & 0xf; }
+constexpr int fwd_tile_flags(int nosignal, int rot, int n_early, int late_at) { return nosignal | rot << 8 | n_early << 16 | late_at << 20; }
 struct FwdArgs {
     const int4 *tiles;
     const int *wg_off;
@@ -285,6 +292,7 @@
     int enc_step;
     int frame_col = -1;
     std::vector<int> deps;
+    int rot_src = -1;
     int depth;
     double flops_per_window;
 };
@@ -321,6 +329,7 @@
     int spill_row0 = -1;
     const std::vector<std::vector<int>> *levels = nullptr;
     std::vector<StageSchedule> stages;
+    std::vector<char> rot_prob;
     int4 *d_tiles = nullptr;
     int *d_wgoff = nullptr;
     StageSchedule frame_stage{};
@@ -485,6 +494,12 @@
 Schedule *schedule_get(Plan *pl, int64_t B, int nwg, bool pin = false, int lane = 0);
 void schedule_frame_stage(const Plan *pl, int64_t B, int nwg, std::vector<int4> &ft, std::vector<int> &fo, StageSchedule &ss);
 bool forward_variant_table(const Plan *pl, int64_t B, int v, int nprob, std::vector<GemmProb> &rel, std::vector<unsigned char> &tags);
+struct Affinity {
+    std::vector<char> rot_prob;
+    std::vector<std::vector<int>> wg_of_chunk;
+};
+void schedule_affinity(const Plan *pl, int64_t B, int nwg, const std::vector<std::vector<int>> &levels, const std::vector<StageSchedule> &stages,
+                       const std::vector<int4> &tiles, const std::vector<int> &wgoff, Affinity &out);
 int forward_kernel_of_lists(const Plan *pl, int64_t B, const std::vector<int> &ft, bool &narrow, bool &b3_tiles);
 inline int64_t schedule_key(int64_t B, int lane) { return B | ((int64_t)lane << 48); }
 int device_cu_count();
diff --git a/ray3d_amd/csrc/r3d_plan.cpp b/ray3d_amd/csrc/r3d_plan.cpp
--- a/ray3d_amd/csrc/r3d_plan.cpp
+++ b/ray3d_amd/csrc/r3d_plan.cpp
@@ -345,6 +345,19 @@
         levelise(false, false, pl->stages_asap, true);
         if (pl->stages_asap == pl->stages) pl->stages_asap.clear();
     }
+    for (size_t i = 0; i < pl->probs.size(); ++i) {
+        ProbSpec &q = pl->probs[i];
+        const Layer &L = pl->m[q.model]->layers[q.layer];
+        q.rot_src = -1;
+        if (q.nseg != 1 || q.enc_lut >= 0 || q.layer2 >= 0 || q.seg[0].width != L.Kpad || L.N != L.Kpad || L.Kpad % BK) continue;
+        if (pl->buffers[q.seg[0].buf].external != 0) continue;
+        for (int d : q.deps) {
+            const ProbSpec &o = pl->probs[d];
+            const Layer &Lo = pl->m[o.model]->layers[o.layer];
+            if (o.enc_lut >= 0 || o.layer2 >= 0 || o.model != q.model || o.rows_per_window != q.rows_per_window) continue;
+            if (o.c_buf == q.seg[0].buf && o.c_col == q.seg[0].col && o.c_ld == q.seg[0].ld && Lo.N == L.N) q.rot_src = std::max(q.rot_src, d);
+        }
+    }
     {
         bool all = true;
         int col = 0;
diff --git a/ray3d_amd/csrc/r3d_schedule.cpp b/ray3d_amd/csrc/r3d_schedule.cpp
--- a/ray3d_amd/csrc/r3d_schedule.cpp
+++ b/ray3d_amd/csrc/r3d_schedule.cpp
@@ -1,4 +1,5 @@
 #include <algorithm>
+#include <array>
 #include <chrono>
 #include <cmath>
 #include <cstdio>
@@ -61,6 +62,100 @@
     int64_t ncnt = 0;
     for (const auto &q : pl->probs) ncnt += units_of(B, q);
     return ((size_t)(ncnt + 4) * sizeof(unsigned) + 255) / 256 * 256 + pl->probs.size() * sizeof(GemmProb) + 256;
+}
+
+static int xcd_chunk_of(int b, int n) {
+    const int qd = n >> 3, r = n & 7, xcd = b & 7, idx = b >> 3;
+    return (xcd < r ? xcd * (qd + 1) : r * (qd + 1) + (xcd - r) * qd) + idx;
+}
+
+static bool tile_takes_rot(int mi, int ks) { return mi == 1 && (ks == 1 || tile_is_nb(ks)); }
+
+void schedule_affinity(const Plan *pl, int64_t B, int nwg, const std::vector<std::vector<int>> &levels, const std::vector<StageSchedule> &stages,
+                       const std::vector<int4> &tiles, const std::vector<int> &wgoff, Affinity &out) {
+    const int np = (int)pl->probs.size();
+    out.rot_prob.assign(np, 0);
+    out.wg_of_chunk.assign(stages.size(), std::vector<int>());
+    const bool b3 = B >= b3_min_batch();
+    typedef std::array<int, 4> Key;
+    std::map<Key, int> where;
+    for (size_t si = 0; si < stages.size(); ++si) {
+        const StageSchedule &ss = stages[si];
+        const auto &st = levels[si];
+        const int n = ss.nwg;
+        std::vector<int> &wg = out.wg_of_chunk[si];
+        wg.assign(n, -1);
+        if (ss.kind != STAGE_BIG || n > nwg) {
+            for (int b = 0; b < n; ++b) if (xcd_chunk_of(b, n) < n) wg[xcd_chunk_of(b, n)] = b;
+            continue;
+        }
+        auto id_of = [&](const int4 &tl) { return st[tl.x & 0xff] & ~STAGE_SPILL_IN; };
+        std::vector<char> cand(np, 0);
+        bool deep = false;
+        for (int e : st) {
+            if (e & STAGE_SPILL_IN) continue;
+            const ProbSpec &q = pl->probs[e];
+            if (q.rot_src < 0 || e == pl->spill_prob || hook_on("R3D_NO_AFFINITY")) continue;
+            const Layer &L = pl->m[q.model]->layers[q.layer];
+            if ((b3 && L.bf3) || L.Kpad / BK < 8) continue;
+            cand[e] = 1;
+        }
+        for (int t = 0; t < ss.ntiles; ++t) {
+            const int4 &tl = tiles[ss.tiles_off + t];
+            const int id = id_of(tl);
+            if (cand[id] && !(tile_takes_rot(tl.x >> 8, tl.w) && where.count(Key{pl->probs[id].rot_src, tl.y, tl.z, tl.w}))) deep = true;
+        }
+        for (int c = 0; c < n && !deep; ++c) {
+            int held = 0;
+            for (int t = wgoff[ss.wgoff_off + c]; t < wgoff[ss.wgoff_off + c + 1]; ++t) held += cand[id_of(tiles[ss.tiles_off + t])] ? 1 : 0;
+            deep = held > 1;
+        }
+        if (deep) std::fill(cand.begin(), cand.end(), 0);
+        std::vector<int> wish(n);
+        for (bool again = true; again;) {
+            again = false;
+            std::map<int, int> taken;
+            std::fill(wish.begin(), wish.end(), -1);
+            for (int c = 0; c < n && !again; ++c)
+                for (int t = wgoff[ss.wgoff_off + c]; t < wgoff[ss.wgoff_off + c + 1]; ++t) {
+                    const int4 &tl = tiles[ss.tiles_off + t];
+                    const int id = id_of(tl);
+                    if (!cand[id]) continue;
+                    const int w = where[Key{pl->probs[id].rot_src, tl.y, tl.z, tl.w}];
+                    const auto other = taken.find(w);
+                    if (other != taken.end()) {
+                        cand[id] = 0;
+                        again = true;
+                        break;
+                    }
+                    wish[c] = w;
+                    taken[w] = id;
+                }
+        }
+        std::vector<char> used(nwg, 0);
+        for (int c = 0; c < n; ++c)
+            if (wish[c] >= 0) { wg[c] = wish[c]; used[wish[c]] = 1; }
+        std::vector<int> displaced;
+        for (int b = 0; b < n; ++b) {
+            const int c = xcd_chunk_of(b, n);
+            if (c >= n || wg[c] >= 0) continue;
+            if (!used[b]) { wg[c] = b; used[b] = 1; }
+            else displaced.push_back(c);
+        }
+        for (int c : displaced) {
+            int b = 0;
+            while (b < nwg && used[b]) ++b;
+            wg[c] = b;
+            used[b] = 1;
+        }
+        for (int c = 0; c < n; ++c)
+            for (int t = wgoff[ss.wgoff_off + c]; t < wgoff[ss.wgoff_off + c + 1]; ++t) {
+                const int4 &tl = tiles[ss.tiles_off + t];
+                where[Key{id_of(tl), tl.y, tl.z, tl.w}] = wg[c];
+            }
+        for (int e : st)
+            if (!(e & STAGE_SPILL_IN) && cand[e] && hook_on("R3D_ROT")) out.rot_prob[e] = 1;
+    }
 }
 
 bool schedule_build_fwd(const Plan *pl, int64_t B, int nwg, const std::vector<std::vector<int>> &levels, const std::vector<StageSchedule> &stages,
@@ -96,17 +191,22 @@
             if (!narrow[i]) quiet[dp] = 0;
     std::vector<std::vector<int>> lists(nwg);
     fw.flops = fw.bytes = 0;
+    Affinity aff;
+    schedule_affinity(pl, B, nwg, levels, stages, tiles, wgoff, aff);
+    std::vector<int> stage_of(np, -1);
+    for (size_t si = 0; si < stages.size(); ++si)
+        for (int e : levels[si]) stage_of[e & ~STAGE_SPILL_IN] = (int)si;
+    const bool b3 = B >= b3_min_batch();
     for (size_t si = 0; si < stages.size(); ++si) {
         const StageSchedule &ss = stages[si];
         const auto &st = levels[si];
         fw.flops += ss.flops;
         fw.bytes += ss.bytes;
         if (ss.nwg > nwg) return false;
-        const int n = ss.nwg, qd = n >> 3, r = n & 7;
-        for (int b = 0; b < n; ++b) {
-            const int xcd = b & 7, idx = b >> 3;
-            const int c = (xcd < r ? xcd * (qd + 1) : r * (qd + 1) + (xcd - r) * qd) + idx;
-            if (c >= n) continue;
+        const int n = ss.nwg;
+        for (int c = 0; c < n; ++c) {
+            const int b = aff.wg_of_chunk[si][c];
+            if (b < 0) continue;
             for (int t = wgoff[ss.wgoff_off + c]; t < wgoff[ss.wgoff_off + c + 1]; ++t) {
                 const int4 &tl = tiles[ss.tiles_off + t];
                 const int slot = tl.x & 0xff, mi = tl.x >> 8, ks = tl.w;
@@ -140,7 +240,45 @@
                     ++nd;
                 }
                 d[4] = nd;
-                d[7] = quiet[id] ? 1 : 0;
+                int rot = 0, n_early = 0, late_at = 0;
+                const Layer &L = pl->m[q.model]->layers[q.layer];
+                const int nk = L.Kpad / BK;
+                if (aff.rot_prob[id]) {
+                    rot = tl.z / BK;
+                    const int own = tile_width(ks) / BK;
+                    if (own >= FWD_A_AHEAD && nd > 0) late_at = std::min(own - FWD_A_AHEAD, FWD_LATE_MAX - 1) + 1;
+                } else if (q.nseg > 1 && tile_takes_rot(mi, ks) && q.enc_lut < 0 && q.layer2 < 0 && !(b3 && L.bf3) && nk >= 8 &&
+                           q.seg[0].width % BK == 0 && q.seg[0].width / BK >= FWD_A_AHEAD && !hook_on("R3D_NO_SPLIT_WAIT")) {
+                    std::vector<int> early, rest;
+                    std::vector<char> is_early(np, 0);
+                    bool old = true;
+                    for (int k = 0; k < nd; ++k) {
+                        int dp = -1;
+                        for (int o : deps)
+                            if (fw.cnt_base[o] <= d[8 + 2 * k] && d[8 + 2 * k] < fw.cnt_base[o] + (int)units_of(B, pl->probs[o])) dp = o;
+                        if (dp >= 0 && pl->probs[dp].c_buf == q.seg[0].buf) {
+                            early.push_back(k);
+                            is_early[dp] = 1;
+                            old = old && stage_of[dp] + 1 < (int)si;
+                        } else {
+                            rest.push_back(k);
+                        }
+                    }
+                    for (int o = 0; o < id; ++o) {
+                        const ProbSpec &oq = pl->probs[o];
+                        const int oN = pl->m[oq.model]->layers[oq.layer3 >= 0 ? oq.layer3 : oq.layer2 >= 0 ? oq.layer2 : oq.layer].N;
+                        if (oq.c_buf == q.seg[0].buf && oq.c_col < q.seg[0].col + q.seg[0].width && q.seg[0].col < oq.c_col + oN && !is_early[o]) old = false;
+                    }
+                    if (old && !early.empty() && !rest.empty() && pl->buffers[q.seg[0].buf].external == 0) {
+                        int e2[2 * FWD_MAX_DEP], j = 0;
+                        for (int k : early) { e2[j++] = d[8 + 2 * k]; e2[j++] = d[9 + 2 * k]; }
+                        for (int k : rest) { e2[j++] = d[8 + 2 * k]; e2[j++] = d[9 + 2 * k]; }
+                        std::copy(e2, e2 + j, d + 8);
+                        n_early = (int)early.size();
+                        late_at = std::min(q.seg[0].width / BK - FWD_A_AHEAD, FWD_LATE_MAX - 1) + 1;
+                    }
+                }
+                d[7] = fwd_tile_flags(quiet[id] ? 1 : 0, rot, n_early, late_at);
                 lists[b].insert(lists[b].end(), d, d + FWD_TILE_INT4 * 4);
             }
         }
@@ -755,6 +893,11 @@
     std::vector<int4> tiles;
     std::vector<int> wgoff;
     s->levels = schedule_build_host(pl, B, nwg, s->spill_row0, tiles, wgoff, s->stages);
+    {
+        Affinity aff;
+        schedule_affinity(pl, B, nwg, *s->levels, s->stages, tiles, wgoff, aff);
+        s->rot_prob = aff.rot_prob;
+    }
     hipError_t e;
     if ((e = hipMalloc((void **)&s->d_tiles, std::max<size_t>(tiles.size(), 1) * sizeof(int4))) != hipSuccess ||
         (e = hipMalloc((void **)&s->d_wgoff, std::max<size_t>(wgoff.size(), 1) * sizeof(int))) != hipSuccess ||
@@ -790,6 +933,7 @@
                 std::vector<GemmProb> rel;
                 std::vector<unsigned char> tags;
                 if (!forward_variant_table(pl, B, v, fw.nprob, rel, tags)) { if (v) continue; ok = false; break; }
+                for (int i = 0; i < fw.nprob; ++i) rel[i].rot = s->rot_prob[i];
                 ok = (e = hipMalloc((void **)&fw.d_rel[v], rel.size() * sizeof(GemmProb))) == hipSuccess &&
                      (e = hipMalloc((void **)&fw.d_tags[v], tags.size())) == hipSuccess &&
                      (e = hipMemcpy(fw.d_rel[v], rel.data(), rel.size() * sizeof(GemmProb), hipMemcpyHostToDevice)) == hipSuccess &&
diff --git a/ray3d_amd/csrc/r3d_tiles.hpp b/ray3d_amd/csrc/r3d_tiles.hpp
--- a/ray3d_amd/csrc/r3d_tiles.hpp
+++ b/ray3d_amd/csrc/r3d_tiles.hpp
@@ -27,8 +27,8 @@
 constexpr int ACT_AUX = 16;
 typedef unsigned u32x4 __attribute__((ext_vector_type(4)));
 typedef unsigned R3D_AS1 *gu32;
-struct LateWait { int dw, ndep; gu32 cnt, abort_flag; long long spin_ticks; };
-__device__ __forceinline__ void wait_deps_reg(const int dw, const int ndep, const gu32 cnt, const gu32 abort_flag, const long long spin_ticks);
+struct LateWait { int dw, ndep; gu32 cnt, abort_flag; long long spin_ticks; int rot, n_early, late_at; };
+__device__ __forceinline__ void wait_deps_reg(const int dw, const int ndep, const gu32 cnt, const gu32 abort_flag, const long long spin_ticks, const int first = 0);
 __device__ __forceinline__ __amdgpu_buffer_rsrc_t act_rsrc(const float *base) {
     return __builtin_amdgcn_make_buffer_rsrc(const_cast<float *>(base), 0, 0x7fffffff, 0x00020000);
 }
@@ -148,6 +148,7 @@
     constexpr bool PRE = MI <= 3;
     constexpr bool WD2 = MI <= 4;
     constexpr int AD = WD2 ? 5 : 4;
+    constexpr bool ROT = MI == 1 && KS == 1 && !PAIR;
     int tid = threadIdx.x;
     asm volatile("" : "+v"(tid));
     const int lane = tid & 63, wave = tid >> 6;
@@ -158,6 +159,12 @@
     const int nk32 = K / BK;
     const int nk = (nk32 + KS - 1) / KS;
     const int srow = tid >> 3, a_kq = (tid & 7) * 4;
+    const int rot = ROT ? late.rot : 0;
+    auto k_of = [&](int kt) {
+        if (!ROT) return kt;
+        const int m = kt + rot;
+        return m >= nk ? m - nk : m;
+    };
 
     const bool multi = P.kend[0] < K;
     int seg_ld = P.lda[0], seg_k0 = 0, seg_end = P.kend[0], seg_i = 0;
@@ -190,7 +197,7 @@
     };
     Staged ra, ra2, ra3;
     auto issue_a = [&](int kt, Staged &R) {
-        const int kb = kt * (BK * KS) - seg_k0;
+        const int kb = k_of(kt) * (BK * KS) - seg_k0;
 #pragma unroll
         for (int i = 0; i < NA; ++i)
             R.a[i] = __builtin_bit_cast(f32x4, __builtin_amdgcn_raw_buffer_load_b128(arsrc, a_voff[i], kb * 4, ACT_AUX));
@@ -214,7 +221,7 @@
 #pragma unroll
         for (int q = 0; q < 4; ++q)
             dst[q] = __builtin_bit_cast(f32x4, __builtin_amdgcn_raw_buffer_load_b128(
-                wrsrc, w_voff + q * 1024, kt * KS * 4096, 0));
+                wrsrc, w_voff + q * 1024, k_of(kt) * KS * 4096, 0));
     };
 
     f32x16 acc[MI];
@@ -229,7 +236,11 @@
     const int last = nk - 1;
     load_w(0, rb);
     if (WD2) load_w(1 < last ? 1 : last, rbn);
-    if (late.ndep > 0) wait_deps_reg(late.dw, late.ndep, late.cnt, late.abort_flag, late.spin_ticks);
+    const bool split = ROT && late.late_at > 0;
+    {
+        const int n1 = split ? late.n_early : late.ndep;
+        if (n1 > 0) wait_deps_reg(late.dw, n1, late.cnt, late.abort_flag, late.spin_ticks);
+    }
     {
         Staged r0, r1;
         issue_a(0, r0);
@@ -309,6 +320,19 @@
     };
     int kt = 0;
     if (WD2) {
+        if constexpr (ROT) {
+            if (split) {
+                auto stage2 = [&]() { wait_deps_reg(late.dw, late.ndep, late.cnt, late.abort_flag, late.spin_ticks, late.n_early); };
+                if (late.late_at == 1) stage2();
+                k_tile(0, rb, rbn2, ra);
+                if (late.late_at == 2) stage2();
+                k_tile(1, rbn, rb, ra2);
+                if (late.late_at == 3) stage2();
+                k_tile(2, rbn2, rbn, ra3);
+                if (late.late_at >= 4) stage2();
+                kt = 3;
+            }
+        }
         for (; kt + 2 < nk; kt += 3) {
             k_tile(kt, rb, rbn2, ra);
             k_tile(kt + 1, rbn, rb, ra2);
@@ -427,6 +451,11 @@
     const int M = P.M, K = P.K;
     const int nk = K / BK;
     const int srow = tid >> 3, a_kq = (tid & 7) * 4;
+    const int rot = late.rot;
+    auto k_of = [&](int kt) {
+        const int m = kt + rot;
+        return m >= nk ? m - nk : m;
+    };
     const int xg0 = (wave_u - 4) * NX;
     int s_blk[4], s_q[4];
 #pragma unroll
@@ -459,7 +488,7 @@
     };
     f32x4 ra, ra2, ra3;
     auto issue_a = [&](int kt, f32x4 &R) {
-        R = __builtin_bit_cast(f32x4, __builtin_amdgcn_raw_buffer_load_b128(arsrc, a_voff, (kt * BK - seg_k0) * 4, ACT_AUX));
+        R = __builtin_bit_cast(f32x4, __builtin_amdgcn_raw_buffer_load_b128(arsrc, a_voff, (k_of(kt) * BK - seg_k0) * 4, ACT_AUX));
     };
     const int st_off = srow * LDS_LD + a_kq;
     auto commit_a = [&](int stage, const f32x4 &R) {
@@ -484,11 +513,15 @@
             if (NS == 0) return;
 #pragma unroll
             for (int s = 0; s < NSL; ++s)
-                dst[s] = __builtin_bit_cast(f32x4, __builtin_amdgcn_raw_buffer_load_b128(wrsrc, w_voff, w_soff[s] + kt * 4096, 0));
+                dst[s] = __builtin_bit_cast(f32x4, __builtin_amdgcn_raw_buffer_load_b128(wrsrc, w_voff, w_soff[s] + k_of(kt) * 4096, 0));
         };
         load_w(0, rb);
         load_w(1 < last ? 1 : last, rbn);
-        if (late.ndep > 0) wait_deps_reg(late.dw, late.ndep, late.cnt, late.abort_flag, late.spin_ticks);
+        const bool split = late.late_at > 0;
+        {
+            const int n1 = split ? late.n_early : late.ndep;
+            if (n1 > 0) wait_deps_reg(late.dw, n1, late.cnt, late.abort_flag, late.spin_ticks);
+        }
         {
             f32x4 r0, r1;
             issue_a(0, r0);
@@ -527,6 +560,17 @@
             st_cur = st_next;
         };
         int kt = 0;
+        if (split) {
+            auto stage2 = [&]() { wait_deps_reg(late.dw, late.ndep, late.cnt, late.abort_flag, late.spin_ticks, late.n_early); };
+            if (late.late_at == 1) stage2();
+            k_tile(0, rb, rbn2, ra);
+            if (late.late_at == 2) stage2();
+            k_tile(1, rbn, rb, ra2);
+            if (late.late_at == 3) stage2();
+            k_tile(2, rbn2, rbn, ra3);
+            if (late.late_at >= 4) stage2();
+            kt = 3;
+        }
         for (; kt + 2 < nk; kt += 3) {
             k_tile(kt, rb, rbn2, ra);
             k_tile(kt + 1, rbn, rb, ra2);
@@ -2364,15 +2408,15 @@
 }
 
 typedef const FwdArgs __attribute__((address_space(4))) *FwdArgsPtr;
-__device__ __forceinline__ void wait_deps_reg(const int dw, const int ndep, const gu32 cnt, const gu32 abort_flag, const long long spin_ticks) {
+__device__ __forceinline__ void wait_deps_reg(const int dw, const int ndep, const gu32 cnt, const gu32 abort_flag, const long long spin_ticks, const int first) {
     if (threadIdx.x < 64) {
         const int lane = threadIdx.x;
         int total = 0;
-        for (int d = 0; d < ndep; ++d) total += __builtin_amdgcn_readlane(dw, 9 + 2 * d) & 0xffff;
+        for (int d = first; d < ndep; ++d) total += __builtin_amdgcn_readlane(dw, 9 + 2 * d) & 0xffff;
         for (int off = 0; off < total; off += 64) {
             int idx = -1, acc = 0;
             unsigned need = 0;
-            for (int d = 0; d < ndep; ++d) {
+            for (int d = first; d < ndep; ++d) {
                 const int base = __builtin_amdgcn_readlane(dw, 8 + 2 * d), nw = __builtin_amdgcn_readlane(dw, 9 + 2 * d);
                 const int n = nw & 0xffff, l = lane + off - acc;
                 if (l >= 0 && l < n) { idx = base + l; need = (unsigned)nw >> 16; }
@@ -2640,7 +2684,8 @@
 #endif
             const bool wait_here = ndep > 0 && (!NARROW || !tile_is_narrow(ks));
             if (wait_here && !LATE) wait_deps_reg(dw, ndep, cnt, abort_flag, fargs->spin_ticks);
-            if (wait_here && LATE) late = LateWait{dw, ndep, cnt, abort_flag, fargs->spin_ticks};
+            if (wait_here && LATE) late = LateWait{dw, ndep, cnt, abort_flag, fargs->spin_ticks, 0, fwd_tile_n_early(tflags), fwd_tile_late_at(tflags)};
+            late.rot = fwd_tile_rot(tflags);
 #ifdef R3D_TIMING
             if (dbg_arg && threadIdx.x == 0) dbg_arg[16384 + (long long)t * 4 + 1] = wall_clock64();
 #endif
@@ -2650,6 +2695,7 @@
 #endif
         }
         ProbRef P = DEP ? *((const GemmProb __attribute__((address_space(4))) *)fargs->probs + pi) : args->p[pi];
+        if constexpr (!DEP) late.rot = P.rot != 0 ? col0 >> 5 : 0;
 #ifdef R3D_TIMING
         dbg = dbg_base && t - t0 < 8 ? dbg_base + (t - t0) * 8 : nullptr;
 #endif
```
